# joshua-lintropic/pfs-neural-net

Measured on AMD Instinct MI355X. Metric: training-step edges/sec on 2394×128 bipartite batches; % HBM roofline, higher is better.
Workload: dtype f32 (split-bf16 products: bf16x6 forward, bf16x3 backward); 1 GPU; 16 complete bipartite 2394x128 graphs per GPU, 8 message-passing blocks, Fdim 10; full training step (GNN fwd + train.py loss + bwd + Adam); fibers=2394, classes=128, graphs_per_gpu=16, global_graphs=16, blocks=8, fdim=10, edges_per_gpu_step=4902912, parallelism=dp1

## Files before the change

### include/pfsgnn.h

```cpp
#ifndef PFSGNN_H
#define PFSGNN_H

#include <stddef.h>
#include <stdint.h>

#ifdef __cplusplus
extern "C" {
#endif

const char* pfsgnn_version(void);
const char* pfsgnn_last_error(void);
size_t pfsgnn_workspace_bytes(int G, int NF, int NC, int F);

#define PFSGNN_EDGE_VALU 0
#define PFSGNN_EDGE_MFMA 1
#define PFSGNN_EDGE_MFMA_F32 2
#define PFSGNN_EDGE_BF16Y 3
#define PFSGNN_EDGE_BF16 4
#define PFSGNN_EDGE_BF16_MFMA 5
#define PFSGNN_EDGE_BF16X3 6
#define PFSGNN_EDGE_BF16X6 7
int pfsgnn_set_edge_path(int path);
int pfsgnn_get_edge_path(void);
size_t pfsgnn_sync_bytes(void);
// ... 260 lines not shown
int pfsgnn_sliced_plan(const int* fib_ptr, int G, int NF, int* fib, int* base, int* len,
                       int* slot_of, long long* info, void* ws, size_t ws_bytes, void* stream);
int pfsgnn_sliced_fill(const int* src_p, const int* tgt_p, const int* user_of, const int* fib_ptr,
                       long long E, int NF, int NC, const int* slot_of, const int* base,
                       long long EP, int maxdeg, unsigned char* cls, int* pos_user, float* pco,
                       void* stream);
int pfsgnn_edges_to_slots(const float* src, long long E, long long EP, int F, const int* pos_user,
                          float* dst, void* stream);
int pfsgnn_edges_from_slots(const float* y, const float* sc, const float* sh, long long E,
                            long long EP, int F, const int* pos_user, int rowmajor, float* dst,
                            void* stream);


int pfsgnn_edge_mlp_fwd(int G, int NF, int NC, int F, const float* xe, const float* xsc,
                        const float* xsh, const float* Ps, const float* Pt, const float* W1,
                        const float* W2, const float* b2, float* y, float* mu, float* var,
                        void* ws, size_t ws_bytes, void* stream);
int pfsgnn_edge_mlp_fwd_bn(int G, int NF, int NC, int F, const float* xe, const float* xsc,
                           const float* xsh, const float* Ps, const float* Pt, const float* W1,
                           const float* W2, const float* b2, float* y, float* mu, float* var,
                           const float* gamma, const float* beta, float* rm, float* rv,
                           float momentum, float eps, float* sc, float* sh, float* inv1,
                           float* inv2, void* ws, size_t ws_bytes, void* stream);
int pfsgnn_source_fwd(int G, int NF, int NC, int F, const float* y, const float* sc,
                      const float* sh, const float* Qt, const float* Ws1, const float* Ws2,
                      const float* bs2, float* mom, float* hs, void* ws, size_t ws_bytes,
                      void* stream);
size_t pfsgnn_msg_bytes(int G, int NF, int NC, int F);
int pfsgnn_source_fwd_msg(int G, int NF, int NC, int F, const float* y, const float* sc,
                          const float* sh, const float* Qt, const float* Ws1, const float* Ws2,
                          const float* bs2, float* mom, float* hs, float* msg, void* ws,
                          size_t ws_bytes, void* stream);
int pfsgnn_target_fwd(int G, int NF, int NC, int F, const float* y, const float* sc,
                      const float* sh, const float* Rs, const float* Wt1, float* hsum,
                      const float* Wt2, const float* bt2, float bscale, float* agg,
                      unsigned char* tmask, void* ws, size_t ws_bytes, void* stream);
size_t pfsgnn_tmask_bytes(int G, int NF, int NC, int F);
int pfsgnn_target_bwd(int G, int NF, int NC, int F, const float* y, const float* sc,
                      const float* sh, const float* Rs, const float* Wt1, const float* g_hsum,
                      float* GzT, float* dWt1, float* gxe, float* g_xs,
                      const unsigned char* tmask, void* ws, size_t ws_bytes, void* stream);
int pfsgnn_target_bwd_bn(int G, int NF, int NC, int F, const float* y, const float* sc,
                         const float* sh, const float* Rs, const float* Wt1, const float* g_hsum,
                         float* GzT, float* dWt1, float* gxe, float* g_xs,
                         const unsigned char* tmask, const float* bn_Yp, const float* bn_mu,
                         const float* bn_var, float bn_eps, float* bn_part, void* ws,
                         size_t ws_bytes, void* stream);
int pfsgnn_source_bwd(int G, int NF, int NC, int F, const float* y, const float* sc,
                      const float* sh, const float* Qt, const float* Ws1, const float* Ws2,
                      const float* bs2, const float* mean, const float* coef, const float* Rs,
                      const float* Wt1, const float* g_hsum, const float* g_next,
                      const float* mu1, const float* inv1, float* g_tot, float* GzS,
                      float* dWs1, float* dWs2, float* dbs2, float* Sg, float* Sgx,
                      float* g_xt, const unsigned char* tmask, void* ws, size_t ws_bytes,
                      void* stream);
int pfsgnn_source_bwd_bn(int G, int NF, int NC, int F, const float* y, const float* sc,
                         const float* sh, const float* Qt, const float* Ws1, const float* Ws2,
                         const float* bs2, const float* mean, const float* coef, const float* Rs,
                         const float* Wt1, const float* g_hsum, const float* g_next,
                         const float* mu1, const float* inv1, const float* var1,
                         const float* gamma, long long n, float eps, float* g_tot, float* GzS,
                         float* dWs1, float* dWs2, float* dbs2, float* alpha, float* gam0,
                         float* gam1, float* dgamma, float* dbeta, float* g_xt,
                         const unsigned char* tmask, void* ws, size_t ws_bytes, void* stream);
int pfsgnn_source_bwd_msg(int G, int NF, int NC, int F, const float* y, const float* sc,
                          const float* sh, const float* Qt, const float* Ws1, const float* Ws2,
                          const float* bs2, const float* mean, const float* coef,
                          const float* Rs, const float* Wt1, const float* g_hsum,
                          const float* g_next, const float* mu1, const float* inv1,
                          float* g_tot, float* GzS, float* dWs1, float* dWs2, float* dbs2,
                          float* Sg, float* Sgx, float* g_xt, const unsigned char* tmask,
                          const float* msg, void* ws, size_t ws_bytes, void* stream);
int pfsgnn_source_bwd_bn_msg(int G, int NF, int NC, int F, const float* y, const float* sc,
                             const float* sh, const float* Qt, const float* Ws1,
                             const float* Ws2, const float* bs2, const float* mean,
                             const float* coef, const float* Rs, const float* Wt1,
                             const float* g_hsum, const float* g_next, const float* mu1,
                             const float* inv1, const float* var1, const float* gamma,
                             long long n, float eps, float* g_tot, float* GzS, float* dWs1,
                             float* dWs2, float* dbs2, float* alpha, float* gam0, float* gam1,
                             float* dgamma, float* dbeta, float* g_xt,
                             const unsigned char* tmask, const float* msg, void* ws,
                             size_t ws_bytes, void* stream);
int pfsgnn_edge_bn_grad_sums(int G, int NF, int NC, int F, const float* g, const float* y,
                             const float* mu1, const float* inv1, float* Sg, float* Sgx,
                             void* ws, size_t ws_bytes, void* stream);
int pfsgnn_edge_mlp_bwd(int G, int NF, int NC, int F, const float* g_tot, const float* alpha,
                        const float* gam0, const float* gam1, const float* y, const float* xe,
                        const float* xsc, const float* xsh, const float* Ps, const float* Pt,
                        const float* W1, const float* W2, float* dW1, float* dW2, float* db2,
                        float* gxe, float* GzEs, float* GzEt, float* g_xs, float* g_xt,
                        float* Vu, void* ws, size_t ws_bytes, void* stream);

int pfsgnn_sl_edge_mlp_fwd(const pfsgnn_sliced_t* sl, int G, int NF, int NC, int F,
                           const float* xe, const float* xsc, const float* xsh, const float* Ps,
                           const float* Pt, const float* W1, const float* W2, const float* b2,
                           float* y, float* mu, float* var, void* ws, size_t ws_bytes,
                           void* stream);
int pfsgnn_sl_edge_mlp_fwd_bn(const pfsgnn_sliced_t* sl, int G, int NF, int NC, int F,
                              const float* xe, const float* xsc, const float* xsh,
                              const float* Ps, const float* Pt, const float* W1, const float* W2,
                              const float* b2, float* y, float* mu, float* var,
                              const float* gamma, const float* beta, float* rm, float* rv,
                              float momentum, float eps, float* sc, float* sh, float* inv1,
                              float* inv2, void* ws, size_t ws_bytes, void* stream);
int pfsgnn_sl_source_fwd(const pfsgnn_sliced_t* sl, int G, int NF, int NC, int F, const float* y,
                         const float* sc, const float* sh, const float* Qt, const float* Ws1,
                         const float* Ws2, const float* bs2, float* mom, float* hs, void* ws,
                         size_t ws_bytes, void* stream);
size_t pfsgnn_sl_tmask_bytes(const pfsgnn_sliced_t* sl, int F);
int pfsgnn_sl_target_fwd(const pfsgnn_sliced_t* sl, int G, int NF, int NC, int F, const float* y,
                         const float* sc, const float* sh, const float* Rs, const float* Wt1,
                         float* hsum, const float* Wt2, const float* bt2, float bscale,
                         float* agg, unsigned char* tmask, void* ws, size_t ws_bytes,
                         void* stream);
int pfsgnn_sl_target_bwd(const pfsgnn_sliced_t* sl, int G, int NF, int NC, int F, const float* y,
                         const float* sc, const float* sh, const float* Rs, const float* Wt1,
                         const float* g_hsum, float* GzT, float* dWt1, float* gxe, float* g_xs,
                         const unsigned char* tmask, void* ws, size_t ws_bytes, void* stream);
int pfsgnn_sl_source_bwd(const pfsgnn_sliced_t* sl, int G, int NF, int NC, int F, const float* y,
                         const float* sc, const float* sh, const float* Qt, const float* Ws1,
                         const float* Ws2, const float* bs2, const float* mean,
                         const float* coef, const float* Rs, const float* Wt1,
                         const float* g_hsum, const float* g_next, const float* mu1,
                         const float* inv1, float* g_tot, float* GzS, float* dWs1, float* dWs2,
                         float* dbs2, float* Sg, float* Sgx, float* g_xt,
                         const unsigned char* tmask, void* ws, size_t ws_bytes, void* stream);
int pfsgnn_sl_source_bwd_bn(const pfsgnn_sliced_t* sl, int G, int NF, int NC, int F,
                            const float* y, const float* sc, const float* sh, const float* Qt,
                            const float* Ws1, const float* Ws2, const float* bs2,
                            const float* mean, const float* coef, const float* Rs,
                            const float* Wt1, const float* g_hsum, const float* g_next,
                            const float* mu1, const float* inv1, const float* var1,
                            const float* gamma, long long n, float eps, float* g_tot, float* GzS,
                            float* dWs1, float* dWs2, float* dbs2, float* alpha, float* gam0,
                            float* gam1, float* dgamma, float* dbeta, float* g_xt,
                            const unsigned char* tmask, void* ws, size_t ws_bytes, void* stream);
int pfsgnn_sl_edge_mlp_bwd(const pfsgnn_sliced_t* sl, int G, int NF, int NC, int F,
                           const float* g_tot, const float* alpha, const float* gam0,
                           const float* gam1, const float* y, const float* xe, const float* xsc,
                           const float* xsh, const float* Ps, const float* Pt, const float* W1,
                           const float* W2, float* dW1, float* dW2, float* db2, float* gxe,
                           float* GzEs, float* GzEt, float* g_xs, float* g_xt, float* Vu,
                           void* ws, size_t ws_bytes, void* stream);

int pfsgnn_loss_fwd(int G, int NF, int NC, int F, const float* y, const float* sc,
                    const float* sh, const float* Wd1, const float* bd1, const float* Wd2,
                    const float* bd2, const float* ci, float scale, float sharpness,
                    float noiselevel, unsigned long long seed,
                    const unsigned long long* seed_dev, float* n_prime,
                    float* fiber_time, float* tmean, float* tvar, float* tt,
                    void* ws, size_t ws_bytes, void* stream);
int pfsgnn_loss_finalize(int G, int NF, int NC, const float* n_prime, const float* fiber_time,
                         const float* tvar, const float* ci, float pclass, float pfiber,
                         float total_time, float nfields, float wutils, float wvar,
                         float* loss, float* utils, float* variance, float* Gn, float* Gf,
                         float* Gv, void* stream);
int pfsgnn_loss_bwd(int G, int NF, int NC, int F, const float* y, const float* sc,
                    const float* sh, const float* Wd1, const float* bd1, const float* Wd2,
                    const float* bd2, const float* ci, float scale, float sharpness,
                    float noiselevel, unsigned long long seed,
                    const unsigned long long* seed_dev, const float* Gn,
                    const float* Gf, const float* Gv, const float* tmean, const float* gscale,
                    float* dWd1, float* dbd1, float* dWd2, float* dbd2, float* gxe,
                    void* ws, size_t ws_bytes, void* stream);
int pfsgnn_loss_bn_parts(int G, int NF, int NC);
// ... 28 lines not shown
```

### pfs-neural-net_amd/csrc/pfsgnn_edge.hip

```cpp
#include <cmath>
#include "pfsgnn_common.h"
#include "../../include/pfsgnn.h"
#include "pfsgnn_mfma.h"

#include <algorithm>
#include <map>
#include <mutex>

#define EDGE_PROLOGUE                                                       \
  const int t = threadIdx.x, lane = t & 63;                                 \
  const int wave = __builtin_amdgcn_readfirstlane(t >> 6);                  \
  const int bx = PF_LOGICAL_BLOCK(geo);                                     \
  if (bx >= geo.nblocks) return;                                            \
  const int ks = bx % geo.KS, grp = bx / geo.KS;                            \
  const int fg = grp % geo.NFG, gg = grp / geo.NFG;                         \
  const int f = fg * 64 + lane;                                             \
  const bool fvalid = f < geo.NF;                                           \
  const long long n = (long long)gg * geo.NF + (fvalid ? f : 0);            \
  const long long nbase = (long long)gg * geo.NF + (long long)fg * 64;      \
  const int nvalid = min(64, geo.NF - fg * 64);                             \
  const int c0 = ks * geo.CPS, c1 = min(geo.NC, c0 + geo.CPS);              \
  const long long E = geo.E, NS = geo.NS, NT = geo.NT;                      \
  const uint32_t RB = (uint32_t)geo.E * 4u;       \
  (void)E; (void)NS; (void)NT; (void)n; (void)nbase; (void)nvalid; (void)RB;
// ... 1352 lines not shown
  static const bool on = [] {
    const char* e = getenv("PFSGNN_XCD_ORDER");
    return !(e && atoi(e) == 0);
  }();
  return on;
}
EdgeGeo geo_for(int G, int NF, int NC) {
  if (!use_mfma()) return make_geo(G, NF, NC);
  EdgeGeo g = geo_mfma(G, NF, NC);
  if (xcd_order()) g.xcdper = (g.nblocks + 7) / 8;
  return g;
}
pfm::SlGeo sl_of(const pfsgnn_sliced_t& s) {
  return pfm::SlGeo{s.fib, s.base, s.len, s.cls, s.pco, s.EP, s.E, s.maxdeg};
}
int sliced_max_nc(int F) {
  if (mf_bfy()) return 0;
  static std::mutex mu;
  static std::map<std::pair<int, int>, int> memo;
  std::lock_guard<std::mutex> lk(mu);
  const auto key = std::make_pair(F, g_path);
  auto it = memo.find(key);
  if (it != memo.end()) return it->second;
  const int p0 = mf_prec(0, F), p1 = mf_prec(1, F);
  const int m = std::min(pfm::sl_max_nc(F, p0), p1 == p0 ? pfm::SL_MAX_NC : pfm::sl_max_nc(F, p1));
  memo[key] = m;
  return m;
}
int check_sliced(const char* where, const pfsgnn_sliced_t* sl, int NC, int F) {
  if (!sl) return 0;
  if (sl->EP * F * 4 >= (1ll << 32)) return pf::fail(where, "edge tensor exceeds 4 GiB (split the batch)");
  if (!sl->fib || !sl->base || !sl->len || !sl->cls || !sl->pco || sl->EP <= 0 || sl->E <= 0 ||
      sl->EP < sl->E)
    return pf::fail(where, "bad sliced layout");
  if (mf_bfy()) return pf::fail(where, "sliced layout: bf16 edge-state paths are not supported");
  if (NC > sliced_max_nc(F)) return pf::fail(where, "sliced layout: too many classes per graph for the LDS (pfsgnn_sliced_max_nc)");
  return 0;
}
EdgeGeo geo_of(int G, int NF, int NC, const pfsgnn_sliced_t* sl) {
  return sl ? pfm::sl_geo(G, NF, NC, sl_of(*sl)) : geo_for(G, NF, NC);
}
int col_bpg(const EdgeGeo& geo, const pfsgnn_sliced_t* sl) {
  return sl ? geo.NFG * geo.KS : geo.NFG;
}

}

extern "C" int pfsgnn_set_edge_path(int path) {
  if (path < PFSGNN_EDGE_VALU || path > PFSGNN_EDGE_BF16X6)
    return pf::fail("pfsgnn_set_edge_path",
                    "path must be PFSGNN_EDGE_VALU, _MFMA, _MFMA_F32, _BF16Y, _BF16, _BF16_MFMA, "
                    "_BF16X3 or _BF16X6");
  g_path = path;
  return 0;
}
extern "C" int pfsgnn_get_edge_path(void) { return g_path; }

extern "C" int pfsgnn_sliced_max_nc(int F, int* nc) {
  PF_REQUIRE(nc, "pfsgnn_sliced_max_nc", "null");
  *nc = sliced_max_nc(F);
  return 0;
}

extern "C" int pfsgnn_edge_grid(int G, int NF, int NC, int* info) {
  PF_REQUIRE(G > 0 && NF > 0 && NC > 0 && info, "pfsgnn_edge_grid", "bad arguments");
  const EdgeGeo geo = geo_for(G, NF, NC);
  info[0] = geo.KS;
  info[1] = geo.CPS;
  info[2] = geo.nblocks;
  info[3] = geo.NFG;
  return 0;
}

namespace {
size_t edge_ws_floats(const EdgeGeo& geo, int G, int NC, int F) {
  const size_t nb = geo.nblocks, ks = geo.KS, NS = geo.NS;
  const size_t H = 4 * F, C = 2 * F;
  const size_t colp = (size_t)G * geo.NFG * NC;
  size_t edge = 0;
  edge = std::max(edge, nb * (1 + 2 * F) + 2 * 48 * MOM_MAXG + 256);
  edge = std::max(edge, ks * 4 * C * NS + C * NS + 1024);
  edge = std::max(edge, colp * C + 1024);
  edge = std::max(edge, nb * C * F + ks * C * NS + 1024);
  edge = std::max(edge, nb * (C * (C + 1) + C * F + 2 * F) + colp * C + 4096);
  edge = std::max(edge, nb * (F * (H + 1) + H * F) + colp * H + ks * H * NS + 4096);
  edge = std::max(edge, colp * 4 + ks * NS + nb * (F * (F + 1) + F + 1) + 4096);
  edge += (size_t)geo.NT * (H + 2 * C) + 4 * H * H + 8 * 256;
  return edge;
}
}

extern "C" size_t pfsgnn_workspace_bytes(int G, int NF, int NC, int F) {
  const EdgeGeo geo = make_geo(G, NF, NC);
  pfm::SlGeo sg{};
  sg.maxdeg = 1 << 30;
  EdgeGeo gs = pfm::sl_geo(G, NF, NC, sg);
  gs.NFG *= gs.KS;
  gs.nblocks = G * gs.NFG;
  const size_t edge = std::max(std::max(edge_ws_floats(geo, G, NC, F),
                                        edge_ws_floats(geo_mfma(G, NF, NC), G, NC, F)),
                               edge_ws_floats(gs, G, NC, F));
  size_t node = (size_t)512 * 161 * 161 + 4096;
  size_t lay = (size_t)geo.E + 1024;
  return (std::max(std::max(edge, node), lay) + 64 * 16) * sizeof(float) + 16 * 256;
}

static int edge_mlp_fwd_impl(const pfsgnn_sliced_t* sl, int G, int NF, int NC, int F,
                             const float* xe, const float* xsc, const float* xsh, const float* Ps,
                             const float* Pt, const float* W1, const float* W2, const float* b2,
                             float* y, float* mu, float* var, Bn2Args bn, void* ws,
                             size_t ws_bytes, void* stream) {
  if (int rc = check_dims("pfsgnn_edge_mlp_fwd", G, NF, NC, F)) return rc;
  if (int rc = check_sliced("pfsgnn_edge_mlp_fwd", sl, NC, F)) return rc;
  PF_REQUIRE(xe && Ps && Pt && W1 && W2 && b2 && y && mu && var, "pfsgnn_edge_mlp_fwd", "null");
  const EdgeGeo geo = geo_of(G, NF, NC, sl);
  Ws w{reinterpret_cast<char*>(ws), ws_bytes};
  hipStream_t st = as_stream(stream);
  float* part = w.take((size_t)geo.nblocks * (1 + 2 * F));
  if (sl) {
    PF_REQUIRE(part, "pfsgnn_edge_mlp_fwd", "workspace too small");
    { pf::Timer tm_("edge_mlp_fwd", st);
    float* tabs = w.take((size_t)pfm::sl_tab_floats(geo, F));
    PF_REQUIRE(tabs, "pfsgnn_edge_mlp_fwd", "workspace too small");
    if (int rc = pfm::sl_edge_mlp_fwd(geo, sl_of(*sl), F, xe, xsc, xsh, Ps, Pt, W1, W2, b2, y, part,
                                      tabs, mf_prec(0, F), st))
      return rc;
    tm_.end(); }
    hipLaunchKernelGGL(k_moments_finalize, dim3(F), dim3(256), 0, st, part, geo.nblocks, F, sl->E,
                       mu, var, bn);
    return pf::check_launch("pfsgnn_edge_mlp_fwd");
  }
  if (use_mfma()) {
    PF_REQUIRE(part, "pfsgnn_edge_mlp_fwd", "workspace too small");
    MomFin fin{};
    if (geo.nblocks <= MOM_GROUP * MOM_MAXG && F <= 16) {
      unsigned* cnt = pf::sync_slot(1 + MOM_MAXG);
      double* gp = cnt ? reinterpret_cast<double*>(w.take(2 * 48 * MOM_MAXG)) : nullptr;
      if (gp) fin = MomFin{cnt, gp, mu, var, geo.E, bn};
    }
    { pf::Timer tm_("edge_mlp_fwd", st);
    for (int rep = 0, nrep = 1 + pf::repeats("edge_mlp_fwd"); rep < nrep; ++rep) {
      MomFin fr = fin;
      if (rep + 1 < nrep) fr.bn.rm = fr.bn.rv = nullptr;
      if (int rc = pfm::edge_mlp_fwd(geo, F, xe, xsc, xsh, Ps, Pt, W1, W2, b2, y, part, fr,
                                     mf_prec(0, F), mf_bfy(), st))
        return rc;
    }
    tm_.end(); }
    if (!fin.cnt)
      hipLaunchKernelGGL(k_moments_finalize, dim3(F), dim3(256), 0, st, part, geo.nblocks, F, geo.E,
                         mu, var, bn);
    return pf::check_launch("pfsgnn_edge_mlp_fwd");
  }
  const float* PtT = class_rows(Pt, 4 * F, geo, w, st);
  const float* W2T = transposed(W2, F, 4 * F, w, st);
  PF_REQUIRE(part && PtT && W2T, "pfsgnn_edge_mlp_fwd", "workspace too small");
  { pf::Timer tm_("edge_mlp_fwd", st);
  DISPATCH_F(F, hipLaunchKernelGGL(k_edge_mlp_fwd<FF>, dim3(edge_grid(geo)), dim3(256), 0, st, geo,
                                   xe, xsc, xsh, Ps, PtT, W1, W2T, b2, y, part));
  tm_.end(); }
  hipLaunchKernelGGL(k_moments_finalize, dim3(F), dim3(256), 0, st, part, geo.nblocks, F, geo.E,
                     mu, var, bn);
  return pf::check_launch("pfsgnn_edge_mlp_fwd");
}

extern "C" int pfsgnn_edge_mlp_fwd(int G, int NF, int NC, int F, const float* xe,
                                   const float* xsc, const float* xsh, const float* Ps,
// ... 174 lines not shown
    DISPATCH_F(F, hipLaunchKernelGGL(k_target_fwd<FF>, dim3(edge_grid(geo)), dim3(256), 0, st, geo,
                                     y, sc, sh, Rs, Wt1, part));
  }
  tm_.end();
  return 0;
}

static int target_fwd_impl(const pfsgnn_sliced_t* sl, int G, int NF, int NC, int F,
                           const float* y, const float* sc, const float* sh, const float* Rs,
                           const float* Wt1, float* hsum, const float* Wt2, const float* bt2,
                           float bscale, float* agg, unsigned char* tmask, void* ws,
                           size_t ws_bytes, void* stream) {
  if (int rc = check_dims("pfsgnn_target_fwd", G, NF, NC, F)) return rc;
  if (int rc = check_sliced("pfsgnn_target_fwd", sl, NC, F)) return rc;
  PF_REQUIRE(y && Rs && Wt1 && hsum, "pfsgnn_target_fwd", "null");
  const EdgeGeo geo = geo_of(G, NF, NC, sl);
  Ws w{reinterpret_cast<char*>(ws), ws_bytes};
  float* part = w.take((size_t)G * col_bpg(geo, sl) * NC * 2 * F);
  PF_REQUIRE(part, "pfsgnn_target_fwd", "workspace too small");
  hipStream_t st = as_stream(stream);
  if (int rc = target_fwd_edges(sl, geo, F, y, sc, sh, Rs, Wt1, part, tmask, st)) return rc;
  PF_REQUIRE(!Wt2 || agg, "pfsgnn_target_fwd", "Wt2 needs agg");
  const NodeLin La = Wt2 ? NodeLin{Wt2, 2 * F, 0, 2 * F, 0, bt2, bscale, agg, (long long)G * NC}
                         : no_lin();
  if (int rc = columns_lin(part, G, col_bpg(geo, sl), NC, 2 * F, hsum, La, no_lin(), st)) return rc;
  return pf::check_launch("pfsgnn_target_fwd");
}

extern "C" int pfsgnn_target_fwd(int G, int NF, int NC, int F, const float* y, const float* sc,
                                 const float* sh, const float* Rs, const float* Wt1, float* hsum,
                                 const float* Wt2, const float* bt2, float bscale, float* agg,
                                 unsigned char* tmask, void* ws, size_t ws_bytes, void* stream) {
  return target_fwd_impl(nullptr, G, NF, NC, F, y, sc, sh, Rs, Wt1, hsum, Wt2, bt2, bscale, agg,
                         tmask, ws, ws_bytes, stream);
}

extern "C" size_t pfsgnn_block_tail_bytes(void) { return sizeof(pfsgnn_block_tail); }

extern "C" int pfsgnn_target_block_fwd(const pfsgnn_block_tail* a, void* ws, size_t ws_bytes,
                                       void* stream) {
  const char* where = "pfsgnn_target_block_fwd";
  PF_REQUIRE(a, where, "null");
  const int G = a->G, NF = a->NF, NC = a->NC, F = a->F;
  if (int rc = check_dims(where, G, NF, NC, F)) return rc;
  PF_REQUIRE(a->y && a->Rs && a->Wt1 && a->Wt2 && a->bt2 && a->hsum && a->agg && a->xt && a->u &&
                 a->W1 && a->b1 && a->W2 && a->b2 && a->gamma && a->beta && a->Z && a->Yp &&
                 a->xt_new && a->mu && a->var && a->xs && a->gW1 && a->gb1 && a->gW2 && a->gb2 &&
                 a->means && a->gZ && a->gV && a->unew,
             where, "null");
  PF_REQUIRE(a->gH > 0 && a->gH <= 192, where, "GlobalModel width must be <= 192");
  PF_REQUIRE(!a->gw || (a->y1 && a->r1 && a->r2), where, "RMSNorm needs y1, r1, r2");
  PF_REQUIRE(!a->We || (a->be && a->Ws && a->bs && a->Pt && a->Qt), where,
             "next-block parts need be, Ws, bs, Pt, Qt");
  PF_REQUIRE((long long)G * NC > 1, where, "BatchNorm needs more than one class");
  const EdgeGeo geo = geo_of(G, NF, NC, nullptr);
  Ws w{reinterpret_cast<char*>(ws), ws_bytes};
  float* part = w.take((size_t)G * col_bpg(geo, nullptr) * NC * 2 * F);
  float* scratch = w.take(pf::tail_ws_floats(G, NC, F));
  PF_REQUIRE(part && scratch, where, "workspace too small");
  hipStream_t st = as_stream(stream);
  if (int rc = target_fwd_edges(nullptr, geo, F, a->y, a->sc, a->sh, a->Rs, a->Wt1, part, a->tmask,
                                st))
    return rc;
  if (int rc = pf::class_tail_fwd(*a, part, col_bpg(geo, nullptr), (float)NF, scratch, st)) return rc;
  return pf::check_launch(where);
}

extern "C" int pfsgnn_sl_target_fwd(const pfsgnn_sliced_t* sl, int G, int NF, int NC, int F,
                                    const float* y, const float* sc, const float* sh,
                                    const float* Rs, const float* Wt1, float* hsum,
                                    const float* Wt2, const float* bt2, float bscale, float* agg,
                                    unsigned char* tmask, void* ws, size_t ws_bytes,
                                    void* stream) {
  PF_REQUIRE(sl, "pfsgnn_sl_target_fwd", "null layout");
  return target_fwd_impl(sl, G, NF, NC, F, y, sc, sh, Rs, Wt1, hsum, Wt2, bt2, bscale, agg, tmask,
                         ws, ws_bytes, stream);
}

static int target_bwd_impl(const pfsgnn_sliced_t* sl, int G, int NF, int NC, int F,
                           const float* y, const float* sc, const float* sh, const float* Rs,
                           const float* Wt1, const float* g_hsum, float* GzT, float* dWt1,
                           float* gxe, float* g_xs, const unsigned char* tmask, void* ws,
                           size_t ws_bytes, void* stream,
                           const FiberBnSums& bs = FiberBnSums{}) {
  if (int rc = check_dims("pfsgnn_target_bwd", G, NF, NC, F)) return rc;
  if (int rc = check_sliced("pfsgnn_target_bwd", sl, NC, F)) return rc;
  PF_REQUIRE(y && Rs && Wt1 && g_hsum && GzT && dWt1, "pfsgnn_target_bwd", "null");
  const EdgeGeo geo = geo_of(G, NF, NC, sl);
  const int C = 2 * F;
  Ws w{reinterpret_cast<char*>(ws), ws_bytes};
  hipStream_t st = as_stream(stream);
  float* part = pf::defer_take((size_t)geo.nblocks * C * F);
  const bool defer = part != nullptr;
  if (!defer) part = w.take((size_t)geo.nblocks * C * F);
  float* gz = fiber_dst(geo, C, GzT, w);
  const float* ghT = (sl || use_mfma()) ? g_hsum
                                       : class_rows(g_hsum, C, geo, w, st);
  PF_REQUIRE(part && gz && ghT, "pfsgnn_target_bwd", "workspace too small");
  { pf::Timer tm_("target_bwd", st);
  if (sl) {
    float* tabs = w.take((size_t)pfm::sl_tab_floats(geo, F));
    PF_REQUIRE(tabs, "pfsgnn_target_bwd", "workspace too small");
    if (int rc = pfm::sl_target_bwd(geo, sl_of(*sl), F, y, sc, sh, Rs, Wt1, ghT, gz, gxe, part,
                                    tmask, tabs, mf_prec(1, F), st))
      return rc;
  } else if (use_mfma()) {
    for (int rep = 0, nrep = 1 + pf::repeats("target_bwd"); rep < nrep; ++rep)
      if (int rc = pfm::target_bwd(geo, F, y, sc, sh, Rs, Wt1, ghT, gz, gxe, part, tmask,
                                   mf_prec(1, F), st))
        return rc;
  } else {
  DISPATCH_F(F, hipLaunchKernelGGL(k_target_bwd<FF>, dim3(edge_grid(geo)), dim3(256), 0, st, geo, y,
                                   sc, sh, Rs, Wt1, ghT, gz, gxe, part));
  }
  tm_.end(); }
  if (int rc = fiber_finish_lin(geo, C, gz, GzT, lin_t_add(g_xs ? Wt1 : nullptr, 2 * F, 0, F, g_xs,
                                                           geo.NS),
                                no_lin(), st, bs))
    return rc;
  const RedDesc rd{part, geo.nblocks, (size_t)C * F, F, C, F, dWt1 + F, C, 1, 1.f};
  if (defer) pf::defer_push(&rd, 1);
  else launch_reduce_multi(&rd, 1, st);
  return pf::check_launch("pfsgnn_target_bwd");
}

extern "C" int pfsgnn_target_bwd(int G, int NF, int NC, int F, const float* y, const float* sc,
                                 const float* sh, const float* Rs, const float* Wt1,
                                 const float* g_hsum, float* GzT, float* dWt1, float* gxe,
                                 float* g_xs, const unsigned char* tmask, void* ws,
                                 size_t ws_bytes, void* stream) {
  return target_bwd_impl(nullptr, G, NF, NC, F, y, sc, sh, Rs, Wt1, g_hsum, GzT, dWt1, gxe, g_xs,
                         tmask, ws, ws_bytes, stream);
}

extern "C" int pfsgnn_target_bwd_bn(int G, int NF, int NC, int F, const float* y,
                                    const float* sc, const float* sh, const float* Rs,
                                    const float* Wt1, const float* g_hsum, float* GzT, float* dWt1,
                                    float* gxe, float* g_xs, const unsigned char* tmask,
                                    const float* bn_Yp, const float* bn_mu, const float* bn_var,
                                    float bn_eps, float* bn_part, void* ws, size_t ws_bytes,
                                    void* stream) {
  PF_REQUIRE(g_xs && bn_Yp && bn_mu && bn_var && bn_part, "pfsgnn_target_bwd_bn", "null");
  return target_bwd_impl(nullptr, G, NF, NC, F, y, sc, sh, Rs, Wt1, g_hsum, GzT, dWt1, gxe, g_xs,
                         tmask, ws, ws_bytes, stream,
                         FiberBnSums{bn_Yp, bn_mu, bn_var, bn_eps, bn_part});
}

extern "C" int pfsgnn_sl_target_bwd(const pfsgnn_sliced_t* sl, int G, int NF, int NC, int F,
                                    const float* y, const float* sc, const float* sh,
                                    const float* Rs, const float* Wt1, const float* g_hsum,
                                    float* GzT, float* dWt1, float* gxe, float* g_xs,
                                    const unsigned char* tmask, void* ws, size_t ws_bytes,
                                    void* stream) {
  PF_REQUIRE(sl, "pfsgnn_sl_target_bwd", "null layout");
  return target_bwd_impl(sl, G, NF, NC, F, y, sc, sh, Rs, Wt1, g_hsum, GzT, dWt1, gxe, g_xs, tmask,
                         ws, ws_bytes, stream);
}

struct Bn2Bwd {
  const float* gamma;
  const float* mu1;
  const float* var1;
  long long n;
  float eps;
  float *alpha, *gam0, *gam1, *dgamma, *dbeta;
};

__device__ __forceinline__ void bn2_coef_block(int k, const float* __restrict__ part, int nb, int F,
                                               const Bn2Bwd& bb, float* __restrict__ Sg,
                                               float* __restrict__ Sgx) {
  const int t = threadIdx.x;
  float a0 = 0.f, a1 = 0.f, a2 = 0.f, a3 = 0.f, b0 = 0.f, b1 = 0.f, b2 = 0.f, b3 = 0.f;
  int b = t;
  for (; b + 768 < nb; b += 1024) {
    const float* p = part + (size_t)b * 2 * F + k;
    const size_t st = (size_t)256 * 2 * F;
    a0 += p[0]; b0 += p[F];
    a1 += p[st]; b1 += p[st + F];
    a2 += p[2 * st]; b2 += p[2 * st + F];
    a3 += p[3 * st]; b3 += p[3 * st + F];
  }
  for (; b < nb; b += 256) {
    a0 += part[(size_t)b * 2 * F + k];
    b0 += part[(size_t)b * 2 * F + F + k];
  }
  float v[2] = {(a0 + a1) + (a2 + a3), (b0 + b1) + (b2 + b3)};
  __shared__ float scratch[8];
  block_sum<2>(v, scratch);
  if (t == 0) {
    if (Sg) { Sg[k] = v[0]; Sgx[k] = v[1]; }
    bn2_bwd_coef_one(k, v[0], v[1], bb.mu1, bb.var1, bb.gamma, bb.n, bb.eps, bb.alpha, bb.gam0,
                     bb.gam1, bb.dgamma, bb.dbeta);
  }
}
__global__ __launch_bounds__(256) void k_bn2_coef_part(const float* __restrict__ part, int nb,
                                                       int F, Bn2Bwd bb, float* __restrict__ Sg,
                                                       float* __restrict__ Sgx) {
  bn2_coef_block(blockIdx.x, part, nb, F, bb, Sg, Sgx);
}
extern "C" int pfsgnn_bn2_bwd_coef_part(const float* part, int nparts, int F, const float* gamma,
                                        const float* mu1, const float* var1, long long n,
                                        float eps, float* alpha, float* gam0, float* gam1,
                                        float* dgamma, float* dbeta, void* stream) {
  PF_REQUIRE(part && nparts > 0 && F > 0 && F <= 16 && gamma && mu1 && var1 && alpha && gam0 &&
                 gam1 && dgamma && dbeta,
             "pfsgnn_bn2_bwd_coef_part", "bad arguments");
  const Bn2Bwd bb{gamma, mu1, var1, n, eps, alpha, gam0, gam1, dgamma, dbeta};
  hipLaunchKernelGGL(k_bn2_coef_part, dim3(F), dim3(256), 0, as_stream(stream), part, nparts, F,
                     bb, nullptr, nullptr);
  return pf::check_launch("pfsgnn_bn2_bwd_coef_part");
}
template <int C>
__global__ __launch_bounds__(256) void k_bn2_coef_columns_lin(const float* __restrict__ part,
                                                              int nb, int F, Bn2Bwd bb,
                                                              float* __restrict__ Sg,
                                                              float* __restrict__ Sgx, ColRed cr) {
  __shared__ ColLinLds<C> S;
  const int bx = blockIdx.x;
  if (bx < F)
    bn2_coef_block(bx, part, nb, F, bb, Sg, Sgx);
  else
    reduce_columns_lin_block<C>(S, bx - F, cr.part, cr.G, cr.BPG, cr.NC, cr.out, cr.L0, cr.L1);
}

static int source_bwd_impl(const pfsgnn_sliced_t* sl, int G, int NF, int NC, int F,
                           const float* y, const float* sc, const float* sh, const float* Qt,
                           const float* Ws1, const float* Ws2, const float* bs2, const float* mean,
                           const float* coef, const float* Rs, const float* Wt1,
                           const float* g_hsum, const float* g_next, const float* mu1,
                           const float* inv1, float* g_tot, float* GzS, float* dWs1, float* dWs2,
                           float* dbs2, float* Sg, float* Sgx, const Bn2Bwd* bb, float* g_xt,
                           const unsigned char* tmask, void* ws, size_t ws_bytes, void* stream,
                           const float* msg = nullptr);

extern "C" int pfsgnn_source_bwd(int G, int NF, int NC, int F, const float* y, const float* sc,
                                 const float* sh, const float* Qt, const float* Ws1,
                                 const float* Ws2, const float* bs2, const float* mean,
                                 const float* coef, const float* Rs, const float* Wt1,
                                 const float* g_hsum, const float* g_next, const float* mu1,
                                 const float* inv1, float* g_tot, float* GzS, float* dWs1,
                                 float* dWs2, float* dbs2, float* Sg, float* Sgx, float* g_xt,
                                 const unsigned char* tmask, void* ws, size_t ws_bytes,
                                 void* stream) {
  return source_bwd_impl(nullptr, G, NF, NC, F, y, sc, sh, Qt, Ws1, Ws2, bs2, mean, coef, Rs, Wt1,
                         g_hsum, g_next, mu1, inv1, g_tot, GzS, dWs1, dWs2, dbs2, Sg, Sgx, nullptr,
                         g_xt, tmask, ws, ws_bytes, stream);
}

extern "C" int pfsgnn_source_bwd_bn(int G, int NF, int NC, int F, const float* y, const float* sc,
                                    const float* sh, const float* Qt, const float* Ws1,
                                    const float* Ws2, const float* bs2, const float* mean,
                                    const float* coef, const float* Rs, const float* Wt1,
                                    const float* g_hsum, const float* g_next, const float* mu1,
                                    const float* inv1, const float* var1, const float* gamma,
                                    long long n, float eps, float* g_tot, float* GzS, float* dWs1,
                                    float* dWs2, float* dbs2, float* alpha, float* gam0,
                                    float* gam1, float* dgamma, float* dbeta, float* g_xt,
                                    const unsigned char* tmask, void* ws, size_t ws_bytes,
                                    void* stream) {
  PF_REQUIRE(mu1 && inv1 && var1 && gamma && n > 0 && alpha && gam0 && gam1 && dgamma && dbeta,
             "pfsgnn_source_bwd_bn", "null");
  const Bn2Bwd bb{gamma, mu1, var1, n, eps, alpha, gam0, gam1, dgamma, dbeta};
  return source_bwd_impl(nullptr, G, NF, NC, F, y, sc, sh, Qt, Ws1, Ws2, bs2, mean, coef, Rs, Wt1,
                         g_hsum, g_next, mu1, inv1, g_tot, GzS, dWs1, dWs2, dbs2, nullptr, nullptr,
                         &bb, g_xt, tmask, ws, ws_bytes, stream);
}

extern "C" int pfsgnn_source_bwd_msg(int G, int NF, int NC, int F, const float* y,
                                     const float* sc, const float* sh, const float* Qt,
                                     const float* Ws1, const float* Ws2, const float* bs2,
                                     const float* mean, const float* coef, const float* Rs,
                                     const float* Wt1, const float* g_hsum, const float* g_next,
                                     const float* mu1, const float* inv1, float* g_tot, float* GzS,
                                     float* dWs1, float* dWs2, float* dbs2, float* Sg, float* Sgx,
                                     float* g_xt, const unsigned char* tmask, const float* msg,
                                     void* ws, size_t ws_bytes, void* stream) {
  PF_REQUIRE(msg, "pfsgnn_source_bwd_msg", "null message cache");
  return source_bwd_impl(nullptr, G, NF, NC, F, y, sc, sh, Qt, Ws1, Ws2, bs2, mean, coef, Rs, Wt1,
                         g_hsum, g_next, mu1, inv1, g_tot, GzS, dWs1, dWs2, dbs2, Sg, Sgx, nullptr,
                         g_xt, tmask, ws, ws_bytes, stream, msg);
}

extern "C" int pfsgnn_source_bwd_bn_msg(
    int G, int NF, int NC, int F, const float* y, const float* sc, const float* sh,
    const float* Qt, const float* Ws1, const float* Ws2, const float* bs2, const float* mean,
    const float* coef, const float* Rs, const float* Wt1, const float* g_hsum,
    const float* g_next, const float* mu1, const float* inv1, const float* var1,
    const float* gamma, long long n, float eps, float* g_tot, float* GzS, float* dWs1,
    float* dWs2, float* dbs2, float* alpha, float* gam0, float* gam1, float* dgamma,
    float* dbeta, float* g_xt, const unsigned char* tmask, const float* msg, void* ws,
    size_t ws_bytes, void* stream) {
  PF_REQUIRE(msg && mu1 && inv1 && var1 && gamma && n > 0 && alpha && gam0 && gam1 && dgamma &&
                 dbeta,
             "pfsgnn_source_bwd_bn_msg", "null");
  const Bn2Bwd bb{gamma, mu1, var1, n, eps, alpha, gam0, gam1, dgamma, dbeta};
  return source_bwd_impl(nullptr, G, NF, NC, F, y, sc, sh, Qt, Ws1, Ws2, bs2, mean, coef, Rs, Wt1,
                         g_hsum, g_next, mu1, inv1, g_tot, GzS, dWs1, dWs2, dbs2, nullptr, nullptr,
                         &bb, g_xt, tmask, ws, ws_bytes, stream, msg);
}

extern "C" int pfsgnn_sl_source_bwd(const pfsgnn_sliced_t* sl, int G, int NF, int NC, int F,
                                    const float* y, const float* sc, const float* sh,
                                    const float* Qt, const float* Ws1, const float* Ws2,
                                    const float* bs2, const float* mean, const float* coef,
                                    const float* Rs, const float* Wt1, const float* g_hsum,
                                    const float* g_next, const float* mu1, const float* inv1,
                                    float* g_tot, float* GzS, float* dWs1, float* dWs2,
                                    float* dbs2, float* Sg, float* Sgx, float* g_xt,
                                    const unsigned char* tmask, void* ws, size_t ws_bytes,
                                    void* stream) {
  PF_REQUIRE(sl, "pfsgnn_sl_source_bwd", "null layout");
  return source_bwd_impl(sl, G, NF, NC, F, y, sc, sh, Qt, Ws1, Ws2, bs2, mean, coef, Rs, Wt1,
                         g_hsum, g_next, mu1, inv1, g_tot, GzS, dWs1, dWs2, dbs2, Sg, Sgx, nullptr,
                         g_xt, tmask, ws, ws_bytes, stream);
}

extern "C" int pfsgnn_sl_source_bwd_bn(
    const pfsgnn_sliced_t* sl, int G, int NF, int NC, int F, const float* y, const float* sc,
    const float* sh, const float* Qt, const float* Ws1, const float* Ws2, const float* bs2,
    const float* mean, const float* coef, const float* Rs, const float* Wt1, const float* g_hsum,
    const float* g_next, const float* mu1, const float* inv1, const float* var1,
    const float* gamma, long long n, float eps, float* g_tot, float* GzS, float* dWs1,
    float* dWs2, float* dbs2, float* alpha, float* gam0, float* gam1, float* dgamma, float* dbeta,
    float* g_xt, const unsigned char* tmask, void* ws, size_t ws_bytes, void* stream) {
  PF_REQUIRE(sl && mu1 && inv1 && var1 && gamma && n > 0 && alpha && gam0 && gam1 && dgamma &&
                 dbeta,
             "pfsgnn_sl_source_bwd_bn", "null");
  const Bn2Bwd bb{gamma, mu1, var1, n, eps, alpha, gam0, gam1, dgamma, dbeta};
  return source_bwd_impl(sl, G, NF, NC, F, y, sc, sh, Qt, Ws1, Ws2, bs2, mean, coef, Rs, Wt1,
                         g_hsum, g_next, mu1, inv1, g_tot, GzS, dWs1, dWs2, dbs2, nullptr, nullptr,
                         &bb, g_xt, tmask, ws, ws_bytes, stream);
}

static int source_bwd_impl(const pfsgnn_sliced_t* sl, int G, int NF, int NC, int F,
                           const float* y, const float* sc, const float* sh, const float* Qt,
                           const float* Ws1, const float* Ws2, const float* bs2, const float* mean,
                           const float* coef, const float* Rs, const float* Wt1,
                           const float* g_hsum, const float* g_next, const float* mu1,
                           const float* inv1, float* g_tot, float* GzS, float* dWs1, float* dWs2,
                           float* dbs2, float* Sg, float* Sgx, const Bn2Bwd* bb, float* g_xt,
                           const unsigned char* tmask, void* ws, size_t ws_bytes, void* stream,
                           const float* msg) {
  if (int rc = check_dims("pfsgnn_source_bwd", G, NF, NC, F)) return rc;
  PF_REQUIRE(!msg || (!sl && msg_bytes(G, NF, NC, F) > 0), "pfsgnn_source_bwd_msg",
             "the message cache is not kept on this path (pfsgnn_msg_bytes is 0)");
  if (int rc = check_sliced("pfsgnn_source_bwd", sl, NC, F)) return rc;
  PF_REQUIRE(y && Qt && Ws1 && Ws2 && bs2 && mean && coef && g_tot && GzS && dWs1 && dWs2 && dbs2,
             "pfsgnn_source_bwd", "null");
  PF_REQUIRE((Rs == nullptr) == (Wt1 == nullptr) && (Rs == nullptr) == (g_hsum == nullptr),
             "pfsgnn_source_bwd", "Rs, Wt1, g_hsum must be given together");
  PF_REQUIRE(!mu1 || (inv1 && ((Sg && Sgx) || bb)), "pfsgnn_source_bwd",
             "mu1 needs inv1, Sg, Sgx");
  const EdgeGeo geo = geo_of(G, NF, NC, sl);
  const int C = 2 * F;
  const size_t nb = geo.nblocks;
  Ws w{reinterpret_cast<char*>(ws), ws_bytes};
  float* pW2 = pf::defer_take(nb * C * (C + 1) + nb * C * F);
  const bool defer = pW2 != nullptr;
  if (!defer) pW2 = w.take(nb * C * (C + 1) + nb * C * F);
  float* pW1 = pW2 ? pW2 + nb * C * (C + 1) : nullptr;
  float* pCol = w.take((size_t)G * col_bpg(geo, sl) * NC * C);
  float* pBN = w.take(nb * 2 * F);
  hipStream_t st = as_stream(stream);
  const bool mfma = sl || use_mfma();
  const float* QtT = mfma ? Qt : class_rows(Qt, C, geo, w, st);
  const float* ghT = mfma ? g_hsum : class_rows(g_hsum, C, geo, w, st);
  PF_REQUIRE(pW2 && pW1 && pCol && pBN && QtT && (ghT || !g_hsum), "pfsgnn_source_bwd",
             "workspace too small");
  { pf::Timer tm_("source_bwd", st);
  if (sl) {
    float* tabs = w.take((size_t)pfm::sl_tab_floats(geo, F));
    PF_REQUIRE(tabs, "pfsgnn_source_bwd", "workspace too small");
    if (int rc = pfm::sl_source_bwd(geo, sl_of(*sl), F, y, sc, sh, QtT, Ws1, Ws2, bs2, mean, coef,
                                    Rs, Wt1, ghT, g_next, mu1, inv1, g_tot, pW2, pW1, pCol, pBN,
                                    tmask, tabs, mf_prec(1, F), st))
      return rc;
  } else if (mfma) {
    for (int rep = 0, nrep = 1 + pf::repeats("source_bwd"); rep < nrep; ++rep)
      if (int rc = pfm::source_bwd(geo, F, msg, y, sc, sh, QtT, Ws1, Ws2, bs2, mean, coef, Rs, Wt1,
                                   ghT, g_next, mu1, inv1, g_tot, pW2, pW1, pCol, pBN, tmask,
                                   mf_prec(1, F), st))
        return rc;
  } else {
  DISPATCH_F(F, hipLaunchKernelGGL(k_source_bwd<FF>, dim3(edge_grid(geo)), dim3(256), 0, st, geo, y,
                                   sc, sh, QtT, Ws1, Ws2, bs2, mean, coef, Rs, Wt1, ghT, g_next,
                                   mu1, inv1, g_tot, pW2, pW1, pCol, pBN));
  }
  tm_.end(); }
  {
    RedDesc rd[5] = {{pBN, (int)nb, (size_t)2 * F, F, 1, F, Sg, F, 0, 1.f},
                     {pBN + F, (int)nb, (size_t)2 * F, F, 1, F, Sgx, F, 0, 1.f},
                     {pW2, (int)nb, (size_t)C * (C + 1), C + 1, C, C, dWs2, C, 1, 1.f},
                     {pW2 + C, (int)nb, (size_t)C * (C + 1), C + 1, C, 1, dbs2, 1, 1, 1.f},
                     {pW1, (int)nb, (size_t)C * F, F, C, F, dWs1 + F, C, 1, 1.f}};
    const bool sums = mu1 && !bb;
    const RedDesc* now = sums ? rd : rd + 2;
    int nnow = sums ? 5 : 3;
    if (defer) {
      pf::defer_push(rd + 2, 3);
      nnow -= 3;
    }
    if (nnow) launch_reduce_multi(now, nnow, st);
  }
  const NodeLin Lx = lin_t_add(g_xt ? Ws1 : nullptr, 2 * F, 0, F, g_xt, geo.NT);
  if (bb && Lx.W) {
    const ColRed cr{pCol, G, col_bpg(geo, sl), NC, GzS, Lx, no_lin()};
    const int nbc = (int)(((long long)G * NC + 3) / 4);
    DISPATCH_C(C, hipLaunchKernelGGL(k_bn2_coef_columns_lin<CC>, dim3(F + nbc), dim3(256), 0, st,
                                     pBN, (int)nb, F, *bb, Sg, Sgx, cr));
  } else {
    if (bb)
      hipLaunchKernelGGL(k_bn2_coef_part, dim3(F), dim3(256), 0, st, pBN, (int)nb, F, *bb, Sg,
                         Sgx);
    if (int rc = columns_lin(pCol, G, col_bpg(geo, sl), NC, C, GzS, Lx, no_lin(), st)) return rc;
  }
  return pf::check_launch("pfsgnn_source_bwd");
}

extern "C" int pfsgnn_edge_bn_grad_sums(int G, int NF, int NC, int F, const float* g,
                                        const float* y, const float* mu1, const float* inv1,
                                        float* Sg, float* Sgx, void* ws, size_t ws_bytes,
                                        void* stream) {
  if (int rc = check_dims("pfsgnn_edge_bn_grad_sums", G, NF, NC, F)) return rc;
  PF_REQUIRE(g && y && mu1 && inv1 && Sg && Sgx, "pfsgnn_edge_bn_grad_sums", "null");
  const EdgeGeo geo = make_geo(G, NF, NC);
  Ws w{reinterpret_cast<char*>(ws), ws_bytes};
  float* pBN = w.take((size_t)geo.nblocks * 2 * F);
  PF_REQUIRE(pBN, "pfsgnn_edge_bn_grad_sums", "workspace too small");
  hipStream_t st = as_stream(stream);
  { pf::Timer tm_("edge_bn_sums", st);
  DISPATCH_F(F, hipLaunchKernelGGL(k_edge_bn_sums<FF>, dim3(edge_grid(geo)), dim3(256), 0, st, geo, g,
                                   y, mu1, inv1, pBN));
  tm_.end(); }
  {
    RedDesc rd[2] = {{pBN, geo.nblocks, (size_t)2 * F, F, 1, F, Sg, F, 0, 1.f},
                     {pBN + F, geo.nblocks, (size_t)2 * F, F, 1, F, Sgx, F, 0, 1.f}};
    launch_reduce_multi(rd, 2, st);
  }
  return pf::check_launch("pfsgnn_edge_bn_grad_sums");
}

static int edge_mlp_bwd_impl(const pfsgnn_sliced_t* sl, int G, int NF, int NC, int F,
                             const float* g_tot, const float* alpha, const float* gam0,
                             const float* gam1, const float* y, const float* xe, const float* xsc,
                             const float* xsh, const float* Ps, const float* Pt, const float* W1,
                             const float* W2, float* dW1, float* dW2, float* db2, float* gxe,
                             float* GzEs, float* GzEt, float* g_xs, float* g_xt, float* Vu,
                             void* ws, size_t ws_bytes, void* stream) {
  if (int rc = check_dims("pfsgnn_edge_mlp_bwd", G, NF, NC, F)) return rc;
  if (int rc = check_sliced("pfsgnn_edge_mlp_bwd", sl, NC, F)) return rc;
  PF_REQUIRE(g_tot && alpha && gam0 && gam1 && y && xe && Ps && Pt && W1 && W2 && dW1 && dW2 &&
                 db2 && GzEs && GzEt,
             "pfsgnn_edge_mlp_bwd", "null");
  const EdgeGeo geo = geo_of(G, NF, NC, sl);
  const int H = 4 * F;
  const size_t nb = geo.nblocks;
  Ws w{reinterpret_cast<char*>(ws), ws_bytes};
  float* pW2 = pf::defer_take(nb * F * (H + 1) + nb * H * F);
  const bool defer = pW2 != nullptr;
  if (!defer) pW2 = w.take(nb * F * (H + 1) + nb * H * F);
  float* pW1 = pW2 ? pW2 + nb * F * (H + 1) : nullptr;
  float* pCol = w.take((size_t)G * col_bpg(geo, sl) * NC * H);
  float* gs = fiber_dst(geo, H, GzEs, w);
  hipStream_t st = as_stream(stream);
  if (sl) {
    PF_REQUIRE(pW2 && pW1 && pCol && gs, "pfsgnn_edge_mlp_bwd", "workspace too small");
    pf::Timer tm_("edge_mlp_bwd", st);
    float* tabs = w.take((size_t)pfm::sl_tab_floats(geo, F));
    PF_REQUIRE(tabs, "pfsgnn_edge_mlp_bwd", "workspace too small");
    if (int rc = pfm::sl_edge_mlp_bwd(geo, sl_of(*sl), F, g_tot, alpha, gam0, gam1, y, xe, xsc,
                                      xsh, Ps, Pt, W1, W2, gxe, gs, pW2, pW1, pCol, tabs,
                                      mf_prec(0, F), st))
      return rc;
    tm_.end();
  } else if (use_mfma()) {
    PF_REQUIRE(pW2 && pW1 && pCol && gs, "pfsgnn_edge_mlp_bwd", "workspace too small");
    pf::Timer tm_("edge_mlp_bwd", st);
    for (int rep = 0, nrep = 1 + pf::repeats("edge_mlp_bwd"); rep < nrep; ++rep)
      if (int rc = pfm::edge_mlp_bwd(geo, F, g_tot, alpha, gam0, gam1, y, xe, xsc, xsh, Ps, Pt,
                                     W1, W2, gxe, gs, pW2, pW1, pCol, mf_prec(0, F), st))
        return rc;
    tm_.end();
  } else {
// ... 53 lines not shown
```

### pfs-neural-net_amd/csrc/pfsgnn_mfma.h

```cpp
#pragma once
#include "pfsgnn_common.h"

namespace pfm {

static constexpr int TARGET_BLOCKS = 2048;
static constexpr int MAX_CPS = 64;

int edge_mlp_fwd(const EdgeGeo& geo, int F, const float* xe, const float* xsc, const float* xsh,
                 const float* Ps, const float* PtS, const float* W1, const float* W2,
                 const float* b2, float* y, float* part, const MomFin& fin, int prec, int bfy,
                 hipStream_t st);
int source_fwd(const EdgeGeo& geo, int F, const float* y, const float* sc, const float* sh,
               const float* QtS, const float* Ws1, const float* Ws2, const float* bs2,
               float* partS, int prec, hipStream_t st);
int source_fwd_tiles(const EdgeGeo& geo, int F, const float* y, const float* sc,
                     const float* sh, const float* QtS, const float* Ws1, const float* Ws2,
                     const float* bs2, float* mom, float* hs, float* msg, int prec, int wave_nc,
                     hipStream_t st);
int target_fwd(const EdgeGeo& geo, int F, const float* y, const float* sc, const float* sh,
               const float* Rs, const float* Wt1, float* part, uint8_t* tmask, int prec,
               hipStream_t st);
int target_bwd(const EdgeGeo& geo, int F, const float* y, const float* sc, const float* sh,
               const float* Rs, const float* Wt1, const float* ghS, float* gz, float* gxe,
               float* part, const uint8_t* tmask, int prec, hipStream_t st);
int source_bwd(const EdgeGeo& geo, int F, const float* msg, const float* y, const float* sc,
               const float* sh, const float* QtS, const float* Ws1, const float* Ws2,
               const float* bs2, const float* mean, const float* coef, const float* Rs,
               const float* Wt1, const float* ghS, const float* g_next, const float* mu1,
               const float* inv1, float* g_tot, float* pW2, float* pW1, float* pCol, float* pBN,
               const uint8_t* tmask, int prec, hipStream_t st);
int edge_mlp_bwd(const EdgeGeo& geo, int F, const float* g_tot, const float* alpha,
                 const float* gam0, const float* gam1, const float* y, const float* xe,
                 const float* xsc, const float* xsh, const float* Ps, const float* PtS,
                 const float* W1, const float* W2, float* gxe, float* gs, float* pW2, float* pW1,
                 float* pCol, int prec, hipStream_t st);

struct SlGeo {
  const int* fib;
  const int* base;
  const int* len;
  const uint8_t* cls;
  const float* pco;
  long long EP, E;
  int maxdeg;
};
static constexpr int SL_MAX_NC = 128;
int sl_max_nc(int F, int prec);
EdgeGeo sl_geo(int G, int NF, int NC, const SlGeo& sl);
int sl_edge_mlp_fwd(const EdgeGeo& geo, const SlGeo& sl, int F, const float* xe, const float* xsc,
                    const float* xsh, const float* Ps, const float* PtS, const float* W1,
                    const float* W2, const float* b2, float* y, float* part, float* tabs,
                    int prec, hipStream_t st);
int sl_source_fwd(const EdgeGeo& geo, const SlGeo& sl, int F, const float* y, const float* sc,
                  const float* sh, const float* QtS, const float* Ws1, const float* Ws2,
                  const float* bs2, float* mom, float* hs, float* tabs, int prec,
                  hipStream_t st);
int sl_target_fwd(const EdgeGeo& geo, const SlGeo& sl, int F, const float* y, const float* sc,
                  const float* sh, const float* Rs, const float* Wt1, float* part, uint8_t* tmask,
                  int prec, hipStream_t st);
int sl_target_bwd(const EdgeGeo& geo, const SlGeo& sl, int F, const float* y, const float* sc,
                  const float* sh, const float* Rs, const float* Wt1, const float* ghS, float* gz,
                  float* gxe, float* part, const uint8_t* tmask, float* tabs, int prec,
                  hipStream_t st);
int sl_source_bwd(const EdgeGeo& geo, const SlGeo& sl, int F, const float* y, const float* sc,
                  const float* sh, const float* QtS, const float* Ws1, const float* Ws2,
                  const float* bs2, const float* mean, const float* coef, const float* Rs,
                  const float* Wt1, const float* ghS, const float* g_next, const float* mu1,
                  const float* inv1, float* g_tot, float* pW2, float* pW1, float* pCol,
                  float* pBN, const uint8_t* tmask, float* tabs, int prec, hipStream_t st);
static inline long long sl_tab_floats(const EdgeGeo& geo, int F) {
  const long long c = 16 * ((((2 * F + 3) / 4) + 3) / 4), h = 16 * ((((4 * F + 3) / 4) + 3) / 4);
  return geo.NT * (2 * c > h ? 2 * c : h);
}
int sl_edge_mlp_bwd(const EdgeGeo& geo, const SlGeo& sl, int F, const float* g_tot,
                    const float* alpha, const float* gam0, const float* gam1, const float* y,
                    const float* xe, const float* xsc, const float* xsh, const float* Ps,
                    const float* PtS, const float* W1, const float* W2, float* gxe, float* gs,
                    float* pW2, float* pW1, float* pCol, float* tabs, int prec, hipStream_t st);

}
```

### pfs-neural-net_amd/csrc/pfsgnn_mfma.hip

```cpp
#include "pfsgnn_mfma_core.h"

#ifndef MF_WG_EARLY_READS
#define MF_WG_EARLY_READS 1
#endif
#ifndef MF_FWD_PAIRS
#define MF_FWD_PAIRS 0
#endif
#ifndef MF_SB_PACK
#define MF_SB_PACK 1
#endif
#ifndef MF_SB_LDSW
#define MF_SB_LDSW 0
#endif
#ifndef MF_WG4
#define MF_WG4 1
#endif

namespace {

#ifndef MF_EFWD_MINB
#define MF_EFWD_MINB 6
#endif
#ifndef MF_EFWD_B6S
#define MF_EFWD_B6S 1
// ... 489 lines not shown
                            p[((1 * NT + tt) * 4 + r) * 64], p[((2 * NT + tt) * 4 + r) * 64],
                            p[((3 * NT + tt) * 4 + r) * 64]);
        na += nb;
      }
      emit(o, mean, M2, M3, M4);
    }
}

template <int F, int PREC>
__global__ __launch_bounds__(256) void km_target_fwd(EdgeGeo geo, const float* __restrict__ y,
                                                     const float* __restrict__ sc,
                                                     const float* __restrict__ sh,
                                                     const float* __restrict__ Rs,
                                                     const float* __restrict__ Wt1,
                                                     float* __restrict__ part,
                                                     uint8_t* __restrict__ tmask) {
  constexpr int C = 2 * F, NT = GM<C>::NT;
  MF_GEO
  __shared__ __attribute__((aligned(16))) float colbuf[COL_CH * 4 * C];
  FwdLayer<PREC, C, F> L1;
  L1.load([&](int h, int k) { return Wt1[h * 2 * F + F + k]; }, lane);
  floatx4 rs[NT];
#pragma unroll
  for (int tt = 0; tt < NT; ++tt) rs[tt] = ld_node<C>(Rs, tt, g4, NS, n, fvalid);
  const floatx4 scv = ld_fconst<F>(sc, g4, 1.f), shv = ld_fconst<F>(sh, g4, 0.f);
  MF_FMASK(F)
  const Rsrc ry = rsrc(y, EB * F);

  int cbase = c0;
  auto load = [&](int c) {
    Rows<1> r;
    r.v[0] = ld_frows<F>(ry, (uint32_t)c * eoc, ro);
    return r;
  };
  auto pre = [&](const Rows<1>& rows, floatx4 (&z)[NT]) {
    const floatx4 x[1] = {edge_in<F>(rows.v[0], fm, sc, scv, shv)};
#pragma unroll
    for (int tt = 0; tt < NT; ++tt) z[tt] = rs[tt];
    L1.apply(x, z);
  };
  auto post = [&](const floatx4 (&z)[NT], int c) {
    if (tmask && fvalid)
      (tmask + (uint32_t)c * eoc)[opaque(eo0 + g4)] = (uint8_t)mask_bits<C>(z);
    const int cl = c - cbase;
#pragma unroll
    for (int tt = 0; tt < NT; ++tt)
#pragma unroll
      for (int r = 0; r < GM<C>::nreg(tt); ++r) {
        const float s = row_sum16(fvalid ? lrelu(z[tt][r]) : 0.f);
        const int h = GM<C>::row(g4, 4 * tt + r);
        if (j16 == 15 && h >= 0) colbuf[(cl * 4 + wave) * C + h] = s;
      }
    if (cl == COL_CH - 1 || c == c1 - 1) {
      __syncthreads();
      col_flush<C>(colbuf, cl + 1, cbase, part, colbase);
      __syncthreads();
      cbase = c + 1;
    }
  };
#if MF_FWD_PAIRS
  class_stream_pairs<MF_DEPTH_FWD>(
      c0, c1, load,
      [&](const Rows<1>& rows, int c) {
        floatx4 z[NT];
        pre(rows, z);
        post(z, c);
      },
      [&](const Rows<1>& ra, int ca, const Rows<1>& rb, int cb) {
        floatx4 za[NT], zb[NT];
        pre(ra, za);
        pre(rb, zb);
        post(za, ca);
        post(zb, cb);
      });
#else
  class_stream<MF_DEPTH_FWD>(c0, c1, load, [&](const Rows<1>& rows, int c) {
    floatx4 z[NT];
    pre(rows, z);
    post(z, c);
  });
#endif
}

template <int F, int PREC, bool TM>
__global__ __launch_bounds__(256) void km_target_bwd(EdgeGeo geo, const float* __restrict__ y,
                                                     const float* __restrict__ sc,
                                                     const float* __restrict__ sh,
                                                     const float* __restrict__ Rs,
                                                     const float* __restrict__ Wt1,
                                                     const float* __restrict__ ghS,
                                                     float* __restrict__ GzT,
                                                     float* __restrict__ gxe,
                                                     float* __restrict__ partW,
                                                     const uint8_t* __restrict__ tmask) {
  constexpr int C = 2 * F, NT = GM<C>::NT;
  constexpr int NIMG = NT + 1;
  using WI = WgImg<PREC>;
  MF_GEO
  __shared__ __attribute__((aligned(16))) short imgs[4 * NIMG * WI::U];
  __shared__ float scratch[4 * C * F];
  __shared__ __attribute__((aligned(16))) float ghl[MF_MAX_CPS * ClassRows<C>::CP];
  ClassRows<C>::stage(ghl, ghS, geo.NT, (long long)gg * geo.NC + c0, c1 - c0);
  short* img = imgs + wave * NIMG * WI::U;
  FwdLayer<FP(PREC), C, F> L1;
  if constexpr (!TM) L1.load([&](int h, int k) { return Wt1[h * 2 * F + F + k]; }, lane);
  GradLayer<PREC, F, C> LT;
  LT.load([&](int k, int h) { return gxe ? Wt1[h * 2 * F + F + k] : 0.f; }, lane);
  floatx4 rs[NT], accF[NT], accW[NT];
#pragma unroll
  for (int tt = 0; tt < NT; ++tt) {
    if constexpr (!TM) rs[tt] = ld_node<C>(Rs, tt, g4, NS, n, fvalid);
    accF[tt] = zero4();
    accW[tt] = zero4();
  }
  const floatx4 scv = ld_fconst<F>(sc, g4, 1.f), shv = ld_fconst<F>(sh, g4, 0.f);
  MF_FMASK(F)
  const Rsrc ry = rsrc(y, EB * F), rtm = rsrc(tmask, EB);
  __syncthreads();

  auto load = [&](int c) {
    Rows<1> r;
    const uint32_t co = (uint32_t)c * eoc;
    r.v[0] = ld_frows<F>(ry, co, ro);
    if constexpr (TM) r.m = __builtin_amdgcn_raw_buffer_load_b8(rtm, eo0 + g4, co, 0);
    return r;
  };
  class_stream<MF_DEPTH_BWD>(c0, c1, load, [&](const Rows<1>& rows, int c) {
    const floatx4 x[1] = {edge_in<F>(rows.v[0], fm, sc, scv, shv)};
    floatx4 z[NT], gz[NT];
    if constexpr (!TM) {
#pragma unroll
      for (int tt = 0; tt < NT; ++tt) z[tt] = rs[tt];
      L1.apply(x, z);
    }
#pragma unroll
    for (int tt = 0; tt < NT; ++tt) {
      const floatx4 gh = ClassRows<C>::get(ghl, c - c0, tt, g4);
      gz[tt] = zero4();
#pragma unroll
      for (int r = 0; r < GM<C>::nreg(tt); ++r) {
        const float sl = TM ? mask_slope(rows.m, 4 * tt + r) : dlrelu(z[tt][r]);
        gz[tt][r] = fvalid ? gh[r] * sl : 0.f;
      }
      accF[tt] += gz[tt];
    }
    Fr sgz[NT];
#pragma unroll
    for (int tt = 0; tt < NT; ++tt) sgz[tt] = split(gz[tt]);
    if (gxe) {
      floatx4 gx[1] = {zero4()};
      if constexpr (PREC >= 1) LT.apply(sgz, gx); else LT.apply(gz, gx);
      st_frows<F>(gxe, EB * F, (uint32_t)c * eoc, ro, g4, fvalid, gx[0]);
    }
    lds_order();
#pragma unroll
    for (int tt = 0; tt < NT; ++tt) WI::put(img + tt * WI::U, lane, gz[tt], sgz[tt]);
    WI::put(img + NT * WI::U, lane, x[0], split(x[0]));
    lds_order();
    const typename WI::TB tx = WI::B(img + NT * WI::U, lane);
#pragma unroll
    for (int tt = 0; tt < NT; ++tt)
      accW[tt] = WI::mma(WI::A(img + tt * WI::U, lane), tx, accW[tt]);
  });
  if (fvalid) {
#pragma unroll
    for (int tt = 0; tt < NT; ++tt)
#pragma unroll
      for (int r = 0; r < GM<C>::nreg(tt); ++r) {
        const int h = GM<C>::row(g4, 4 * tt + r);
        if (h >= 0) GzT[(size_t)ks * C * NS + (size_t)h * NS + n] = accF[tt][r];
      }
  }
  block_partial(accW, scratch, C * F, [&](int a, int s, int jj) {
    const int h = GM<C>::mrow(a, s), k = GM<F>::mrow(0, jj);
    return (h >= 0 && k >= 0) ? h * F + k : -1;
  }, partW + (size_t)bx * C * F);
}

template <int F, int PREC, bool TM, bool MSG = false>
__global__ __launch_bounds__(256, 2) void km_source_bwd(
    EdgeGeo geo, const float* __restrict__ msg, const float* __restrict__ y, const float* __restrict__ sc,
    const float* __restrict__ sh, const float* __restrict__ QtS, const float* __restrict__ Ws1,
    const float* __restrict__ Ws2, const float* __restrict__ bs2, const float* __restrict__ mean,
    const float* __restrict__ coef, const float* __restrict__ Rs, const float* __restrict__ Wt1,
    const float* __restrict__ ghS, const float* __restrict__ g_next,
    const float* __restrict__ mu1, const float* __restrict__ inv1, float* __restrict__ g_tot,
    float* __restrict__ partW2, float* __restrict__ partW1, float* __restrict__ partCol,
    float* __restrict__ partBN, const uint8_t* __restrict__ tmask) {
  constexpr int C = 2 * F, NT = GM<C>::NT;
  constexpr bool PACK = MF_SB_PACK && NT == 2 && GM<C>::nreg(1) == 1 && GM<F>::NT == 1 && GM<F>::RPG == 3;
  constexpr int NIMG = PACK ? 5 : 3 * NT + 1;
  constexpr int SCR = C * (C + 1) > C * F ? C * (C + 1) : C * F;
  using WI = WgImg<PREC>;
  MF_GEO
  __shared__ __attribute__((aligned(16))) short imgs[4 * NIMG * WI::U];
  __shared__ __attribute__((aligned(16))) float colbuf[COL_CH * 4 * C];
  __shared__ float scratch[4 * SCR];
  __shared__ __attribute__((aligned(16))) float qtl[MF_MAX_CPS * ClassRows<C>::CP];
  __shared__ __attribute__((aligned(16))) float ghl[MF_MAX_CPS * ClassRows<C>::CP];
  ClassRows<C>::stage(qtl, QtS, geo.NT, (long long)gg * geo.NC + c0, c1 - c0);
  if (ghS) ClassRows<C>::stage(ghl, ghS, geo.NT, (long long)gg * geo.NC + c0, c1 - c0);
  short* img = imgs + wave * NIMG * WI::U;
  short* im_gm = img;
  short* im_a = img + NT * WI::U;
  short* im_gz = im_a + NT * WI::U;
  short* im_x = im_gz + NT * WI::U;
  short* im_r1 = img;
  short* im_r2 = img + WI::U;
  short* im_r3 = img + 2 * WI::U;
  short* im_c1 = img + 3 * WI::U;
  short* im_c2 = img + 4 * WI::U;
  (void)im_r1; (void)im_r2; (void)im_r3; (void)im_c1; (void)im_c2;
  const long long CNS = (long long)C * NS;
  const bool tpart = Rs != nullptr;

  RecLayer<PREC, C, F> L1s, L1t;
  RecLayer<PREC, C, C> L2;
  constexpr int R1 = RecLds<RecLayer<PREC, C, F>>::n, R2 = RecLds<RecLayer<PREC, C, C>>::n;
  __shared__ s16x8 recw[(R1 * (TM ? 1 : 2) + R2) > 0 ? R1 * (TM ? 1 : 2) + R2 : 1];
  rec_bind(L1s, recw);
  rec_bind(L2, recw + R1);
  rec_bind(L1t, recw + R1 + R2);
  L1s.load([&](int h, int k) { return Ws1[h * 2 * F + F + k]; }, lane);
  if constexpr (!TM) L1t.load([&](int h, int k) { return tpart ? Wt1[h * 2 * F + F + k] : 0.f; }, lane);
  if constexpr (!MSG) L2.load([&](int o, int h) { return Ws2[o * C + h]; }, lane);
  constexpr bool LW = MF_SB_LDSW && std::is_same_v<GradLayer<PREC, C, C>, LayerB3<C, C>>;
  using GL2 = std::conditional_t<LW, LayerB3S<C, C>, GradLayer<PREC, C, C>>;
  using GL1 = std::conditional_t<LW, LayerB3S<F, C>, GradLayer<PREC, F, C>>;
  GL2 L2T;
  GL1 L1sT, L1tT;
  if constexpr (LW) {
    __shared__ s16x8 gw[(LayerB3S<C, C>::NOP + 2 * LayerB3S<F, C>::NOP) * 64];
    L2T.bind(gw);
    L1sT.bind(gw + LayerB3S<C, C>::NOP * 64);
    L1tT.bind(gw + (LayerB3S<C, C>::NOP + LayerB3S<F, C>::NOP) * 64);
  }
  L2T.load([&](int h, int o) { return Ws2[o * C + h]; }, lane);
  L1sT.load([&](int k, int h) { return Ws1[h * 2 * F + F + k]; }, lane);
  L1tT.load([&](int k, int h) { return tpart ? Wt1[h * 2 * F + F + k] : 0.f; }, lane);
  floatx4 rs[NT], bias[NT], mn[NT], q0[NT], q1[NT], q2[NT], q3[NT];
#pragma unroll
  for (int tt = 0; tt < NT; ++tt) {
    if constexpr (!TM) rs[tt] = ld_node<C>(Rs, tt, g4, NS, n, fvalid);
    bias[tt] = ld_vec<C>(bs2, tt, g4);
    mn[tt] = ld_node<C>(mean, tt, g4, NS, n, fvalid);
    q0[tt] = ld_node<C>(coef, tt, g4, NS, n, fvalid);
    q1[tt] = ld_node<C>(coef + CNS, tt, g4, NS, n, fvalid);
    q2[tt] = ld_node<C>(coef + 2 * CNS, tt, g4, NS, n, fvalid);
    q3[tt] = ld_node<C>(coef + 3 * CNS, tt, g4, NS, n, fvalid);
  }
  const floatx4 scv = ld_fconst<F>(sc, g4, 1.f), shv = ld_fconst<F>(sh, g4, 0.f);
  const floatx4 m1v = ld_fconst<F>(mu1, g4, 0.f), i1v = ld_fconst<F>(inv1, g4, 0.f);
  MF_FMASK(F)
  const Rsrc ry = rsrc(y, EB * F), rgn = rsrc(g_next, EB * F), rtm = rsrc(tmask, EB);
  [[maybe_unused]] const Rsrc rms = rsrc(msg, EB * C);
  [[maybe_unused]] const RowOff<C> roC(eo0, RB, g4);

  floatx4 accW2[NT * NT], accW1[NT], accB[NT];
  floatx4 accP[5];
#pragma unroll
  for (int tt = 0; tt < NT; ++tt) {
    accW1[tt] = zero4();
    accB[tt] = zero4();
#pragma unroll
    for (int nb = 0; nb < NT; ++nb) accW2[tt * NT + nb] = zero4();
  }
#pragma unroll
  for (int i = 0; i < 5; ++i) accP[i] = zero4();
  floatx4 sg = zero4(), sgx = zero4();
  const s16x8 ones = ones_reg();
  __syncthreads();

  int cbase = c0;
  using RowsT = Rows<MSG ? 2 + NT : 2>;
  auto load = [&](int c) {
    RowsT r;
    const uint32_t co = (uint32_t)c * eoc;
    r.v[0] = ld_frows<F>(ry, co, ro);
    r.v[1] = g_next ? ld_frows<F>(rgn, co, ro) : zero4();
    if constexpr (TM) r.m = tpart ? __builtin_amdgcn_raw_buffer_load_b8(rtm, eo0 + g4, co, 0) : 0u;
    if constexpr (MSG) {
      floatx4 mv[NT];
      ld_rows_nt<C>(rms, co, roC, mv);
#pragma unroll
      for (int tt = 0; tt < NT; ++tt) r.v[2 + tt] = mv[tt];
    }
    return r;
  };
  class_stream<MF_DEPTH_BWD>(c0, c1, load, [&](const RowsT& rows, int c) {
    const floatx4 yr = rows.v[0], gnr = rows.v[1];
    const floatx4 x[1] = {edge_in<F>(yr, fm, sc, scv, shv)};
    floatx4 zs[NT], as[NT], m[NT];
#pragma unroll
    for (int tt = 0; tt < NT; ++tt) zs[tt] = ClassRows<C>::get(qtl, c - c0, tt, g4);
    L1s.apply(x, zs);
    lrelu_act<C>(zs, as);
    if constexpr (MSG) {
#pragma unroll
      for (int tt = 0; tt < NT; ++tt) m[tt] = rows.v[2 + tt];
    } else {
#pragma unroll
      for (int tt = 0; tt < NT; ++tt) m[tt] = bias[tt];
      L2.apply(as, m);
    }
    floatx4 gm[NT];
#pragma unroll
    for (int tt = 0; tt < NT; ++tt) {
      gm[tt] = zero4();
#pragma unroll
      for (int r = 0; r < GM<C>::nreg(tt); ++r) {
        const float d = m[tt][r] - mn[tt][r];
        gm[tt][r] = fvalid ? fmaf(d, fmaf(d, fmaf(d, q3[tt][r], q2[tt][r]), q1[tt][r]), q0[tt][r]) : 0.f;
      }
      accB[tt] += gm[tt];
    }
    Fr sgm[NT], sgz[NT];
#pragma unroll
    for (int tt = 0; tt < NT; ++tt) sgm[tt] = split(gm[tt]);
    floatx4 gz[NT];
#pragma unroll
    for (int tt = 0; tt < NT; ++tt) gz[tt] = zero4();
    if constexpr (PREC >= 1) L2T.apply(sgm, gz); else L2T.apply(gm, gz);
#pragma unroll
    for (int tt = 0; tt < NT; ++tt) {
#pragma unroll
      for (int r = 0; r < GM<C>::nreg(tt); ++r) gz[tt][r] *= dlrelu(zs[tt][r]);
      sgz[tt] = split(gz[tt]);
    }
    lds_order();
    [[maybe_unused]] floatx4 r3v, c2v;
    if constexpr (PACK) {
      r3v = floatx4{gm[1][0], gz[1][0], 0.f, 0.f};
      c2v = floatx4{as[1][0], x[0][0], x[0][1], x[0][2]};
      const Fr sr3 = {s16x4{sgm[1].h[0], sgz[1].h[0], 0, 0}, s16x4{sgm[1].l[0], sgz[1].l[0], 0, 0}};
      WI::put(im_r1, lane, gm[0], sgm[0]);
      WI::put(im_r2, lane, gz[0], sgz[0]);
      WI::put(im_r3, lane, r3v, sr3);
      WI::put(im_c1, lane, as[0], split(as[0]));
      WI::put(im_c2, lane, c2v, split(c2v));
    } else {
#pragma unroll
      for (int tt = 0; tt < NT; ++tt) {
        WI::put(im_gm + tt * WI::U, lane, gm[tt], sgm[tt]);
        WI::put(im_a + tt * WI::U, lane, as[tt], split(as[tt]));
        WI::put(im_gz + tt * WI::U, lane, gz[tt], sgz[tt]);
      }
      WI::put(im_x, lane, x[0], split(x[0]));
    }
    lds_order();
#if MF_WG_EARLY_READS
    typename WI::R rx, ra[NT], rgm[NT], rgz[NT], rp[5], rq[2];
    if constexpr (PACK) {
#pragma unroll
      for (int i = 0; i < 5; ++i) rp[i] = WI::rd(img + i * WI::U, lane);
#if MF_WG4
      lds_order();
      rq[0] = WI::rd(im_c1, lane);
      rq[1] = WI::rd(im_c2, lane);
#endif
    } else {
      rx = WI::rd(im_x, lane);
#pragma unroll
      for (int tt = 0; tt < NT; ++tt) {
        ra[tt] = WI::rd(im_a + tt * WI::U, lane);
        rgm[tt] = WI::rd(im_gm + tt * WI::U, lane);
        rgz[tt] = WI::rd(im_gz + tt * WI::U, lane);
      }
    }
    lds_order();
#endif
    floatx4 g[1] = {zero4()};
    if constexpr (PREC >= 1) L1sT.apply(sgz, g); else L1sT.apply(gz, g);
    if (tpart) {
      floatx4 zt[NT];
      if constexpr (!TM) {
#pragma unroll
        for (int tt = 0; tt < NT; ++tt) zt[tt] = rs[tt];
        L1t.apply(x, zt);
      }
#pragma unroll
      for (int tt = 0; tt < NT; ++tt) {
        const floatx4 gh = ClassRows<C>::get(ghl, c - c0, tt, g4);
#pragma unroll
        for (int r = 0; r < 4; ++r) {
          const float sl = TM ? mask_slope(rows.m, 4 * tt + r) : dlrelu(zt[tt][r]);
          zt[tt][r] = (fvalid && r < GM<C>::nreg(tt)) ? gh[r] * sl : 0.f;
        }
      }
      if constexpr (PREC >= 1) {
        Fr szt[NT];
#pragma unroll
        for (int tt = 0; tt < NT; ++tt) szt[tt] = split(zt[tt]);
        L1tT.apply(szt, g);
      } else {
        L1tT.apply(zt, g);
      }
    }
#pragma unroll
    for (int r = 0; r < 4; ++r) g[0][r] = fm[r] ? g[0][r] + (g_next ? gnr[r] : 0.f) : 0.f;
    st_frows<F>(g_tot, EB * F, (uint32_t)c * eoc, ro, g4, fvalid, g[0]);
    if (mu1) {
#pragma unroll
      for (int r = 0; r < GM<F>::RPG; ++r) {
        sg[r] += g[0][r];
        sgx[r] = fmaf(g[0][r], (yr[r] - m1v[r]) * i1v[r], sgx[r]);
      }
    }
    lds_order();
    const int cl = c - cbase;
    if constexpr (PACK) {
#if !MF_WG_EARLY_READS
#error "source_bwd's packed tiles read their images early (MF_WG_EARLY_READS)"
#endif
      const typename WI::TA t1 = WI::A(rp[0]), t2 = WI::A(rp[1]), t3 = WI::A(rp[2]);
#if MF_WG4
      const typename WI::TB4 tc1 = WI::B4(rp[3], rq[0]), tc2 = WI::B4(rp[4], rq[1]);
      accP[0] = WI::mma4(t1, tc1, accP[0]);
      accP[1] = WI::mma4(t1, tc2, accP[1]);
      accP[2] = WI::mma4(t2, tc2, accP[2]);
      accP[3] = WI::mma4(t3, tc1, accP[3]);
      accP[4] = WI::mma4(t3, tc2, accP[4]);
#else
      const typename WI::TB tc1 = WI::B(rp[3]), tc2 = WI::B(rp[4]);
      accP[0] = WI::mma(t1, tc1, accP[0]);
      accP[1] = WI::mma(t1, tc2, accP[1]);
      accP[2] = WI::mma(t2, tc2, accP[2]);
      accP[3] = WI::mma(t3, tc1, accP[3]);
      accP[4] = WI::mma(t3, tc2, accP[4]);
#endif
      const floatx4 cs2 = WI::colsum(t2, gz[0], ones), cs3 = WI::colsum(t3, r3v, ones);
      if (j16 == WI::CS_LANE) {
#pragma unroll
        for (int r = 0; r < 4; ++r) {
          const int h = GM<C>::mrow(0, 4 * g4 + r);
          if (h >= 0) colbuf[(cl * 4 + wave) * C + h] = cs2[r];
        }
        const int h1 = GM<C>::row(g4, 4);
        if (h1 >= 0) colbuf[(cl * 4 + wave) * C + h1] = cs3[1];
      }
    } else {
#if MF_WG_EARLY_READS
    const typename WI::TB tx = WI::B(rx);
    typename WI::TB ta[NT];
#pragma unroll
    for (int nb = 0; nb < NT; ++nb) ta[nb] = WI::B(ra[nb]);
#else
    const typename WI::TB tx = WI::B(im_x, lane);
    typename WI::TB ta[NT];
#pragma unroll
    for (int nb = 0; nb < NT; ++nb) ta[nb] = WI::B(im_a + nb * WI::U, lane);
#endif
#pragma unroll
    for (int tt = 0; tt < NT; ++tt) {
#if MF_WG_EARLY_READS
      const typename WI::TA tgm = WI::A(rgm[tt]);
#pragma unroll
      for (int nb = 0; nb < NT; ++nb) accW2[tt * NT + nb] = WI::mma(tgm, ta[nb], accW2[tt * NT + nb]);
      const typename WI::TA tgz = WI::A(rgz[tt]);
#else
      const typename WI::TA tgm = WI::A(im_gm + tt * WI::U, lane);
#pragma unroll
      for (int nb = 0; nb < NT; ++nb) accW2[tt * NT + nb] = WI::mma(tgm, ta[nb], accW2[tt * NT + nb]);
      const typename WI::TA tgz = WI::A(im_gz + tt * WI::U, lane);
#endif
      accW1[tt] = WI::mma(tgz, tx, accW1[tt]);
      const floatx4 cs = WI::colsum(tgz, gz[tt]);
      if (j16 == WI::CS_LANE) {
#pragma unroll
        for (int r = 0; r < 4; ++r) {
          const int h = GM<C>::mrow(tt, 4 * g4 + r);
          if (h >= 0) colbuf[(cl * 4 + wave) * C + h] = cs[r];
        }
      }
    }
    }
    if (cl == COL_CH - 1 || c == c1 - 1) {
      __syncthreads();
      col_flush<C>(colbuf, cl + 1, cbase, partCol, colbase);
      __syncthreads();
      cbase = c + 1;
    }
  });
  if constexpr (PACK) {
    block_partial(accP, scratch, C * (C + 1), [&](int a, int s, int jj) {
      int o = -1, h = -1;
      if (a == 0) { o = GM<C>::mrow(0, s); h = GM<C>::mrow(0, jj); }
      if (a == 1 && (jj & 3) == 0) { o = GM<C>::mrow(0, s); h = GM<C>::row(jj >> 2, 4); }
      if (a == 3 && (s & 3) == 0) { o = GM<C>::row(s >> 2, 4); h = GM<C>::mrow(0, jj); }
      if (a == 4 && (s & 3) == 0 && (jj & 3) == 0) { o = GM<C>::row(s >> 2, 4); h = GM<C>::row(jj >> 2, 4); }
      return (o >= 0 && h >= 0) ? o * (C + 1) + h : -1;
    }, partW2 + (size_t)bx * C * (C + 1));
  } else {
    block_partial(accW2, scratch, C * (C + 1), [&](int a, int s, int jj) {
      const int o = GM<C>::mrow(a / NT, s), h = GM<C>::mrow(a % NT, jj);
      return (o >= 0 && h >= 0) ? o * (C + 1) + h : -1;
    }, partW2 + (size_t)bx * C * (C + 1));
  }
  {
    __syncthreads();
#pragma unroll
    for (int tt = 0; tt < NT; ++tt)
#pragma unroll
      for (int r = 0; r < GM<C>::nreg(tt); ++r) {
        const float v = group_sum16(accB[tt][r]);
        const int o = GM<C>::row(g4, 4 * tt + r);
        if (j16 == 0 && o >= 0) scratch[wave * C + o] = v;
      }
    __syncthreads();
    if (t < C)
      partW2[(size_t)bx * C * (C + 1) + t * (C + 1) + C] =
          ((scratch[t] + scratch[C + t]) + scratch[2 * C + t]) + scratch[3 * C + t];
  }
  if constexpr (PACK) {
    block_partial(accP, scratch, C * F, [&](int a, int s, int jj) {
      int h = -1, k = -1;
      if ((jj & 3) != 0) k = GM<F>::row(jj >> 2, (jj & 3) - 1);
      if (a == 2) h = GM<C>::mrow(0, s);
      if (a == 4 && (s & 3) == 1) h = GM<C>::row(s >> 2, 4);
      return (h >= 0 && k >= 0) ? h * F + k : -1;
    }, partW1 + (size_t)bx * C * F);
  } else {
    block_partial(accW1, scratch, C * F, [&](int a, int s, int jj) {
      const int h = GM<C>::mrow(a, s), k = GM<F>::mrow(0, jj);
      return (h >= 0 && k >= 0) ? h * F + k : -1;
    }, partW1 + (size_t)bx * C * F);
  }
  if (mu1) {
    __syncthreads();
#pragma unroll
    for (int r = 0; r < GM<F>::RPG; ++r) {
      const float a = group_sum16(sg[r]), b = group_sum16(sgx[r]);
      const int k = GM<F>::row(g4, r);
      if (j16 == 0 && k >= 0) { scratch[wave * 2 * F + k] = a; scratch[wave * 2 * F + F + k] = b; }
    }
    __syncthreads();
    if (t < 2 * F)
      partBN[(size_t)bx * 2 * F + t] =
          ((scratch[t] + scratch[2 * F + t]) + scratch[4 * F + t]) + scratch[6 * F + t];
  }
}

#ifndef MF_BWD_PIPE6
#define MF_BWD_PIPE6 0
#endif
template <int F, int PREC>
__global__ __launch_bounds__(256, 2) void km_edge_mlp_bwd(
    EdgeGeo geo, const float* __restrict__ g_tot, const float* __restrict__ alpha,
    const float* __restrict__ gam0, const float* __restrict__ gam1, const float* __restrict__ y,
    const float* __restrict__ xe, const float* __restrict__ xsc, const float* __restrict__ xsh,
    const float* __restrict__ Ps, const float* __restrict__ PtS, const float* __restrict__ W1,
    const float* __restrict__ W2, float* __restrict__ gxe, float* __restrict__ GzEs,
    float* __restrict__ partW2, float* __restrict__ partW1, float* __restrict__ partCol) {
  constexpr int H = 4 * F, NT = GM<H>::NT;
  constexpr int NIMG = 1 + NT + NT + 1;
  constexpr int SCR = F * (H + 1) > H * F ? F * (H + 1) : H * F;
  using WI = WgImg<PREC>;
  MF_GEO
  __shared__ __attribute__((aligned(16))) short imgs[4 * NIMG * WI::U];
  __shared__ __attribute__((aligned(16))) float colbuf[COL_CH * 4 * H];
  __shared__ float scratch[4 * SCR];
  __shared__ __attribute__((aligned(16))) float ptl[MF_MAX_CPS * ClassRows<H>::CP];
  ClassRows<H>::stage(ptl, PtS, geo.NT, (long long)gg * geo.NC + c0, c1 - c0);
  short* img = imgs + wave * NIMG * WI::U;
  short* im_gy = img;
  short* im_a = img + WI::U;
  short* im_gz = im_a + NT * WI::U;
  short* im_x = im_gz + NT * WI::U;

#ifdef MF_EMB_REC_B6
  std::conditional_t<PREC == 1, LayerB6<H, F>, FwdLayer<FP(PREC), H, F>> L1;
#else
  FwdLayer<FP(PREC), H, F> L1;
#endif
  L1.load([&](int h, int k) { return W1[h * 4 * F + 2 * F + k]; }, lane);
  GradLayer<PREC, H, F> L2T;
  L2T.load([&](int h, int o) { return W2[o * H + h]; }, lane);
  GradLayer<PREC, F, H> L1T;
  L1T.load([&](int k, int h) { return gxe ? W1[h * 4 * F + 2 * F + k] : 0.f; }, lane);
  floatx4 ps[NT], accF[NT], accW1[NT], accW2[NT];
#pragma unroll
  for (int tt = 0; tt < NT; ++tt) {
    ps[tt] = ld_node<H>(Ps, tt, g4, NS, n, fvalid);
    accF[tt] = zero4();
    accW1[tt] = zero4();
    accW2[tt] = zero4();
  }
  floatx4 accB = zero4();
  const floatx4 alv = ld_fconst<F>(alpha, g4, 0.f), g0v = ld_fconst<F>(gam0, g4, 0.f),
                g1v = ld_fconst<F>(gam1, g4, 0.f);
  const floatx4 scv = ld_fconst<F>(xsc, g4, 1.f), shv = ld_fconst<F>(xsh, g4, 0.f);
  MF_FMASK(F)
  const Rsrc rgt = rsrc(g_tot, EB * F), ry = rsrc(y, EB * F), rxe = rsrc(xe, EB * F);
  const s16x8 ones = ones_reg();
  __syncthreads();

  int cbase = c0;
  auto load = [&](int c) {
    Rows<3> r;
    const uint32_t co = (uint32_t)c * eoc;
    r.v[0] = ld_frows<F>(rgt, co, ro);
    r.v[1] = ld_frows<F>(ry, co, ro);
    r.v[2] = ld_frows<F>(rxe, co, ro);
    return r;
  };
  struct Head {
    floatx4 gy, x, z[NT];
  };
  auto head = [&](const Rows<3>& rows, int c) {
// ... 161 lines not shown
    MF_CASE(16, 0, K, __VA_ARGS__) MF_CASE(16, 1, K, __VA_ARGS__)                \
    default: return pf::fail("pfsgnn mfma", "unsupported Fdim for this edge path"); \
  }

#define MF_CASE3(FF, PP, TT, K, ...)                                              \
  case FF * 8 + PP: {                                                             \
    hipLaunchKernelGGL((K<FF, PP, TT>), dim3(edge_grid(geo)), dim3(256), 0, st, geo, \
                       __VA_ARGS__);                                              \
  } break;
#define MF_LAUNCH3(F, P, TT, K, ...)                                              \
  switch ((F) * 8 + (P)) {                                                        \
    MF_CASE3(8, 0, TT, K, __VA_ARGS__) MF_CASE3(8, 1, TT, K, __VA_ARGS__)        \
    MF_CASE3(10, 0, TT, K, __VA_ARGS__) MF_CASE3(10, 1, TT, K, __VA_ARGS__)      \
    MF_CASE3(10, 2, TT, K, __VA_ARGS__) MF_CASE3(10, 3, TT, K, __VA_ARGS__)      \
    MF_CASE3(10, 4, TT, K, __VA_ARGS__)                                           \
    MF_CASE3(16, 0, TT, K, __VA_ARGS__) MF_CASE3(16, 1, TT, K, __VA_ARGS__)      \
    default: return pf::fail("pfsgnn mfma", "unsupported Fdim for this edge path"); \
  }

#ifndef MF_PART
#define MF_PART 0
#endif
namespace pfm {
#if MF_PART != 2

static inline int fwd_prec(int prec) { return FP(prec); }

int edge_mlp_fwd(const EdgeGeo& geo, int F, const float* xe, const float* xsc, const float* xsh,
                 const float* Ps, const float* PtS, const float* W1, const float* W2,
                 const float* b2, float* y, float* part, const MomFin& fin, int prec, int bfy,
                 hipStream_t st) {
  if (fin.cnt && (geo.nblocks > MOM_GROUP * MOM_MAXG || F > 16))
    return pf::fail("pfsgnn mfma", "edge_mlp_fwd: in-launch finalize needs <= 4096 blocks");
  MF_LAUNCH(F, fwd_prec(prec), km_edge_mlp_fwd, xe, xsc, xsh, Ps, PtS, W1, W2, b2, y, part, bfy,
            fin)
  return 0;
}

int source_fwd(const EdgeGeo& geo, int F, const float* y, const float* sc, const float* sh,
               const float* QtS, const float* Ws1, const float* Ws2, const float* bs2,
               float* partS, int prec, hipStream_t st) {
  MF_LAUNCH(F, fwd_prec(prec), km_source_fwd, y, sc, sh, QtS, Ws1, Ws2, bs2, partS)
  return 0;
}

int source_fwd_tiles(const EdgeGeo& geo, int F, const float* y, const float* sc,
                     const float* sh, const float* QtS, const float* Ws1, const float* Ws2,
                     const float* bs2, float* mom, float* hs, float* msg, int prec, int wave_nc,
                     hipStream_t st) {
  if (geo.NC > MF_SFT_MAXNC) return pf::fail("pfsgnn mfma", "source_fwd_tiles: NC > 256");
  const bool wf = geo.NC <= std::min(wave_nc, MF_SFT_WAVE_MAXNC);
  const int TF = wf ? 64 : 16;
  const int ntiles = geo.G * ((geo.NF + TF - 1) / TF);
  const int nb = 8 * ((ntiles + 7) / 8);
  const size_t lds = sft_lds_floats(geo.NC, F) * sizeof(float);
#define MF_SFT(FF, PP)                                                                     \
  case FF * 8 + PP:                                                                        \
    if (wf)                                                                                \
      hipLaunchKernelGGL((km_source_fwd_ft<FF, PP, true>), dim3(nb), dim3(256), lds, st, geo, \
                         ntiles, y, sc, sh, QtS, Ws1, Ws2, bs2, mom, hs, msg);             \
    else                                                                                   \
      hipLaunchKernelGGL((km_source_fwd_ft<FF, PP, false>), dim3(nb), dim3(256), lds, st, geo, \
                         ntiles, y, sc, sh, QtS, Ws1, Ws2, bs2, mom, hs, msg);             \
    break;
  switch (F * 8 + fwd_prec(prec)) {
    MF_SFT(8, 0) MF_SFT(8, 1) MF_SFT(10, 0) MF_SFT(10, 1) MF_SFT(10, 2) MF_SFT(10, 3)
    MF_SFT(10, 4) MF_SFT(16, 0) MF_SFT(16, 1)
    default: return pf::fail("pfsgnn mfma", "unsupported Fdim for this edge path");
  }
#undef MF_SFT
  return 0;
}

int target_fwd(const EdgeGeo& geo, int F, const float* y, const float* sc, const float* sh,
               const float* Rs, const float* Wt1, float* part, uint8_t* tmask, int prec,
               hipStream_t st) {
  MF_LAUNCH(F, fwd_prec(prec), km_target_fwd, y, sc, sh, Rs, Wt1, part, tmask)
  return 0;
}

int target_bwd(const EdgeGeo& geo, int F, const float* y, const float* sc, const float* sh,
               const float* Rs, const float* Wt1, const float* ghS, float* gz, float* gxe,
               float* part, const uint8_t* tmask, int prec, hipStream_t st) {
  if (tmask) {
    MF_LAUNCH3(F, prec, true, km_target_bwd, y, sc, sh, Rs, Wt1, ghS, gz, gxe, part, tmask)
  } else {
    MF_LAUNCH3(F, prec, false, km_target_bwd, y, sc, sh, Rs, Wt1, ghS, gz, gxe, part, tmask)
  }
  return 0;
}

int source_bwd(const EdgeGeo& geo, int F, const float* msg, const float* y, const float* sc,
               const float* sh, const float* QtS, const float* Ws1, const float* Ws2,
               const float* bs2, const float* mean, const float* coef, const float* Rs,
               const float* Wt1, const float* ghS, const float* g_next, const float* mu1,
               const float* inv1, float* g_tot, float* pW2, float* pW1, float* pCol, float* pBN,
               const uint8_t* tmask, int prec, hipStream_t st) {
  if (msg) {
    if (prec != 0 && prec != 1) return pf::fail("pfsgnn mfma", "message cache: mfma paths only");
#define MF_CASE_MSG(FF, PP, TT)                                                                  \
  case FF * 8 + PP:                                                                             \
    hipLaunchKernelGGL((km_source_bwd<FF, PP, TT, true>), dim3(edge_grid(geo)), dim3(256), 0, st, \
                       geo, msg, y, sc, sh, QtS, Ws1, Ws2, bs2, mean, coef, Rs, Wt1, ghS, g_next, \
                       mu1, inv1, g_tot, pW2, pW1, pCol, pBN, tmask);                           \
    break;
    if (tmask && Rs) {
      switch (F * 8 + prec) {
        MF_CASE_MSG(8, 0, true) MF_CASE_MSG(8, 1, true) MF_CASE_MSG(10, 0, true)
        MF_CASE_MSG(10, 1, true) MF_CASE_MSG(16, 0, true) MF_CASE_MSG(16, 1, true)
        default: return pf::fail("pfsgnn mfma", "unsupported Fdim for this edge path");
      }
    } else {
      switch (F * 8 + prec) {
        MF_CASE_MSG(8, 0, false) MF_CASE_MSG(8, 1, false) MF_CASE_MSG(10, 0, false)
        MF_CASE_MSG(10, 1, false) MF_CASE_MSG(16, 0, false) MF_CASE_MSG(16, 1, false)
        default: return pf::fail("pfsgnn mfma", "unsupported Fdim for this edge path");
      }
    }
#undef MF_CASE_MSG
    return 0;
  }
  if (tmask && Rs) {
    MF_LAUNCH3(F, prec, true, km_source_bwd, nullptr, y, sc, sh, QtS, Ws1, Ws2, bs2, mean, coef, Rs, Wt1,
               ghS, g_next, mu1, inv1, g_tot, pW2, pW1, pCol, pBN, tmask)
  } else {
    MF_LAUNCH3(F, prec, false, km_source_bwd, nullptr, y, sc, sh, QtS, Ws1, Ws2, bs2, mean, coef, Rs, Wt1,
               ghS, g_next, mu1, inv1, g_tot, pW2, pW1, pCol, pBN, tmask)
  }
  return 0;
}

#endif
#if MF_PART != 1
int edge_mlp_bwd(const EdgeGeo& geo, int F, const float* g_tot, const float* alpha,
                 const float* gam0, const float* gam1, const float* y, const float* xe,
                 const float* xsc, const float* xsh, const float* Ps, const float* PtS,
                 const float* W1, const float* W2, float* gxe, float* gs, float* pW2, float* pW1,
                 float* pCol, int prec, hipStream_t st) {
  MF_LAUNCH(F, prec, km_edge_mlp_bwd, g_tot, alpha, gam0, gam1, y, xe, xsc, xsh, Ps, PtS, W1, W2,
            gxe, gs, pW2, pW1, pCol)
  return 0;
}
#endif

}
```

### pfs-neural-net_amd/pfsgnn/engine.py

```python
import os

import torch


class Dims:

    def __init__(self, G, NF, NC, F, sp=None):
        self.G, self.NF, self.NC, self.F = int(G), int(NF), int(NC), int(F)
        self.sp = sp
        self.E = self.G * self.NF * self.NC if sp is None else sp.E
        self.EP = self.E if sp is None else sp.EP
        self.NS = self.G * self.NF
        self.NT = self.G * self.NC

    def __repr__(self):
        kind = "" if self.sp is None else ", general"
        return f"Dims(G={self.G}, NF={self.NF}, NC={self.NC}, F={self.F}, E={self.E}{kind})"


def param_names(B, normed=True):
    names = []

    def mlp(pre):
        names.extend([pre + ".0.weight", pre + ".0.bias", pre + ".2.weight", pre + ".2.bias"])
# ... 233 lines not shown
                                                Gr[key + "weight"], Gr[key + "bias"])
            z = self.be.zeros(scale.shape[0])
            return scale, z, z
        return self.be.bn2_bwd_coef(Sg, Sgx, st["mu1"], st["var1"], P[key + "weight"], d.E,
                                    self.bn_eps, Gr[key + "weight"], Gr[key + "bias"])

    def edge_bnstat(self, P, pre, st):
        if "rm" in st:
            key = pre + "norm."
            inv, _ = self.be.bn_eval_bwd_coef(P[key + "weight"], P[key + "bias"], st["rm"],
                                              st["rv"], self.bn_eps, 2)
            return st["rm"], inv
        return st["mu1"], st["inv1"]

    def edge_bwd(self, P, Gr, d, pre, st, g_tot, bnc, want_gxe, g_xs, g_xt, g_u):
        be, F, G = self.be, self.F, d.G
        if self.normed:
            alpha, gam0, gam1 = bnc
        else:
            alpha, gam0, gam1 = be.ones(F), be.zeros(F), be.zeros(F)
        W1, W2 = P[pre + "0.weight"], P[pre + "2.weight"]
        xe, xsc, xsh = st["xe3"]
        dW1 = Gr[pre + "0.weight"]
        g_xe, GzEs, GzEt, Vu = be.edge_mlp_bwd(d, g_tot, alpha, gam0, gam1, st["y"], xe, xsc, xsh,
                                               st["Ps"], st["Pt"], W1, W2, dW1,
                                               Gr[pre + "2.weight"], Gr[pre + "2.bias"],
                                               want_gxe=want_gxe, nodes=(g_xs, g_xt))
        be.wgrad(GzEs, st["xs"], dW1, col0=0)
        be.wgrad_cat(GzEt, [(st["xt"], F, False), (st["u"], 3 * F, True)], dW1,
                     db=Gr[pre + "0.bias"])
        self._gu_add(Vu, G, g_u)
        return g_xe

    def source_fwd(self, P, BN, d, pre, xs, xt, xe3, u, Qt=None, epi=None):
        be, F = self.be, self.F
        Ws1, bs1 = P[pre + "node_mlp_1.0.weight"], P[pre + "node_mlp_1.0.bias"]
        Ws2, bs2 = P[pre + "node_mlp_1.2.weight"], P[pre + "node_mlp_1.2.bias"]
        if Qt is None:
            Qt = be.lin(Ws1, 0, F, xt, b=bs1)
        hmom = be.empty(8 * F, d.NS)
        msg = be.msg_cache(d) if (self.training or self.want_grad) and \
            hasattr(be, "msg_cache") else None
        if msg is not None:
            mom = be.source_fwd(d, xe3[0], xe3[1], xe3[2], Qt, Ws1, Ws2, bs2, hmom, msg=msg)
        else:
            mom = be.source_fwd(d, xe3[0], xe3[1], xe3[2], Qt, Ws1, Ws2, bs2, hmom)
        hS = [(xs, 0, False), (hmom, F, False), (u, 9 * F, True)]
        st = dict(xs=xs, xt=xt, xe3=xe3, u=u, Qt=Qt, mom=mom, msg=msg)
        if epi:
            names = list(epi)
            xs_new, sS, outs = self.mlp_fwd(P, pre + "node_mlp_2.", hS, pre + "norm.", BN,
                                            epi=[epi[k] for k in names])
            st.update(zip(names, outs))
        else:
            xs_new, sS = self.mlp_fwd(P, pre + "node_mlp_2.", hS, pre + "norm.", BN)
        st.update(sS=sS, xs_new=xs_new)
        return st

    def _mom_epi_ok(self, d, st):
        sS = st.get("sS")
        return (d.sp is None and getattr(self.be, "fiber_bn_sums", False)
                and self.F in (8, 10) and sS is not None and sS[0] != "ops"
                and os.environ.get("PFSGNN_MOM_EPI", "1") != "0"
                and os.environ.get("PFSGNN_MLP_BWD_RS", "1") != "0")

    def source_node_bwd(self, P, Gr, d, pre, st, g_xs_new, g_xs, g_u, bn_part=None):
        be, F, G = self.be, self.F, d.G
        gu = be.empty(F, d.NS)
        if self._mom_epi_ok(d, st):
            coef = be.empty(4, 2 * F, d.NS)
            self.mlp_bwd(P, Gr, pre + "node_mlp_2.", g_xs_new, st["sS"],
                         outs=[(g_xs, F, True), (None, 8 * F, False), (gu, F, False)],
                         bn_part=bn_part, mom_coef=(st["mom"], coef, F, d.NC))
            self._gu_add(gu, G, g_u)
            return coef
        gst = be.empty(8 * F, d.NS)
        self.mlp_bwd(P, Gr, pre + "node_mlp_2.", g_xs_new, st["sS"],
                     outs=[(g_xs, F, True), (gst, 8 * F, False), (gu, F, False)],
                     bn_part=bn_part)
        self._gu_add(gu, G, g_u)
        return be.moment_coef(st["mom"], gst, d.NC if d.sp is None else d.sp.fib_ptr)

    def source_edge_bwd(self, P, Gr, d, pre, st, coef, tpart, g_next, bnstat, g_xt, se=None,
                        epre=None, tmask=None):
        be, F = self.be, self.F
        Ws1, Ws2 = P[pre + "node_mlp_1.0.weight"], P[pre + "node_mlp_1.2.weight"]
        y, sc, sh = st["xe3"]
        bn2 = None
        if se is not None and bnstat is not None:
            key = epre + "norm."
            bn2 = (P[key + "weight"], se["var1"], d.E, self.bn_eps, Gr[key + "weight"],
                   Gr[key + "bias"])
        out = be.source_bwd(
            d, y, sc, sh, st["Qt"], Ws1, Ws2, P[pre + "node_mlp_1.2.bias"], st["mom"][0], coef,
            tpart, g_next, bnstat, Gr[pre + "node_mlp_1.0.weight"], Gr[pre + "node_mlp_1.2.weight"],
            Gr[pre + "node_mlp_1.2.bias"], bn2=bn2, g_xt=g_xt,
            **({"tmask": tmask} if tmask is not None and tpart is not None else {}),
            **({"msg": st["msg"]} if st.get("msg") is not None else {}))
        g_tot, GzS = out[0], out[1]
        be.wgrad(GzS, st["xt"], Gr[pre + "node_mlp_1.0.weight"], col0=0,
                 db=Gr[pre + "node_mlp_1.0.bias"])
        if bn2 is not None:
            return g_tot, out[4]
        return g_tot, out[2], out[3]

    def target_fwd(self, P, BN, d, pre, xs, xt, xe3, u, Rs=None, glob=None):
        be, F = self.be, self.F
        Wt1, bt1 = P[pre + "node_mlp_1.0.weight"], P[pre + "node_mlp_1.0.bias"]
        Wt2, bt2 = P[pre + "node_mlp_1.2.weight"], P[pre + "node_mlp_1.2.bias"]
        if Rs is None:
            Rs = be.lin(Wt1, 0, F, xs, b=bt1)
        tmask = be.tmask(d) if self.training and hasattr(be, "tmask") else None
        if glob is not None and d.sp is None and hasattr(be, "target_block_fwd") and \
                d.G * -(-d.NC // 32) <= 512 and d.NC <= 2048 and \
                os.environ.get("PFSGNN_CLASS_TAIL", "1") != "0":
            return self._target_block_fwd(P, BN, d, pre, xs, xt, xe3, u, Rs, tmask, glob)
        if d.sp is None:
            hsum, agg = be.target_fwd(d, xe3[0], xe3[1], xe3[2], Rs, Wt1,
                                      agg=(Wt2, bt2, float(d.NF)),
                                      **({"tmask": tmask} if tmask is not None else {}))
        else:
            hsum = be.target_fwd(d, xe3[0], xe3[1], xe3[2], Rs, Wt1,
                                 **({"tmask": tmask} if tmask is not None else {}))
            agg = be.lin(Wt2, 0, 2 * F, hsum)
            be.lin(bt2.view(-1, 1), 0, 1, d.sp.deg_t, out=agg, add=True)
        hT = [(xt, 0, False), (agg, F, False), (u, 3 * F, True)]
        st = dict(xs=xs, xt=xt, xe3=xe3, u=u, Rs=Rs, hsum=hsum, tmask=tmask)
        if glob is None:
            xt_new, sT = self.mlp_fwd(P, pre + "node_mlp_2.", hT, pre + "norm.", BN)
            st.update(sT=sT, xt_new=xt_new)
            return st
        pg, pnext = glob
        m2 = pre + "node_mlp_2."
        w = P[pg + "norm.weight"]
        nxt = None
        if pnext is not None:
            pe, ps = pnext + "edge_model.", pnext + "s_model."
            nxt = (P[pe + "0.weight"], P[pe + "0.bias"], P[ps + "node_mlp_1.0.weight"],
                   P[ps + "node_mlp_1.0.bias"])
        r = be.target_global_fwd(hT, d.G, d.NC, P[m2 + "0.weight"], P[m2 + "0.bias"],
                                 P[m2 + "2.weight"], P[m2 + "2.bias"],
                                 self._bn_args(P, BN, pre + "norm."), xs, d.NF, u,
                                 P[pg + "0.weight"], P[pg + "0.bias"], P[pg + "2.weight"],
                                 P[pg + "2.bias"], w, self._rms_eps(u), nxt)
        st.update(sT=(hT, r["Z"], (r["Yp"], r["mu"], r["var"], pre + "norm.")), xt_new=r["xt"])
        st["su"] = dict(sU=([(u, 0, False), (r["means"], F, False)], r["gZ"], None), v=r["gV"],
                        rms=r["rms"], u_new=r["u"], fused=True)
        st["parts_t"] = (r["Pt"], r["Qt"])
        return st

    def _target_block_fwd(self, P, BN, d, pre, xs, xt, xe3, u, Rs, tmask, glob):
        be, F = self.be, self.F
        pg, pnext = glob
        m2 = pre + "node_mlp_2."
        nxt = None
        if pnext is not None:
            pe, ps = pnext + "edge_model.", pnext + "s_model."
            nxt = (P[pe + "0.weight"], P[pe + "0.bias"], P[ps + "node_mlp_1.0.weight"],
                   P[ps + "node_mlp_1.0.bias"])
        r = be.target_block_fwd(d, xe3[0], xe3[1], xe3[2], Rs, P[pre + "node_mlp_1.0.weight"],
                                P[pre + "node_mlp_1.2.weight"], P[pre + "node_mlp_1.2.bias"],
                                tmask, xt, u, P[m2 + "0.weight"], P[m2 + "0.bias"],
                                P[m2 + "2.weight"], P[m2 + "2.bias"],
                                self._bn_args(P, BN, pre + "norm."), xs, P[pg + "0.weight"],
                                P[pg + "0.bias"], P[pg + "2.weight"], P[pg + "2.bias"],
                                P[pg + "norm.weight"], self._rms_eps(u), nxt)
        hT = [(xt, 0, False), (r["agg"], F, False), (u, 3 * F, True)]
        st = dict(xs=xs, xt=xt, xe3=xe3, u=u, Rs=Rs, hsum=r["hsum"], tmask=tmask)
        st.update(sT=(hT, r["Z"], (r["Yp"], r["mu"], r["var"], pre + "norm.")), xt_new=r["xt"])
        st["su"] = dict(sU=([(u, 0, False), (r["means"], F, False)], r["gZ"], None), v=r["gV"],
                        rms=r["rms"], u_new=r["u"], fused=True)
        st["parts_t"] = (r["Pt"], r["Qt"])
        return st

    def _class_bwd_ok(self, d, su, stt):
        sT = stt.get("sT")
        return (d.sp is None and self.normed and self.F in (8, 10, 16) and d.NC <= 1024
                and hasattr(self.be, "target_class_bwd") and su.get("fused")
                and sT is not None and sT[2] is not None and sT[2][0] != "eval"
                and os.environ.get("PFSGNN_CLASS_BWD", "1") != "0")

    def _class_bwd(self, P, Gr, d, p, su, stt, pend, g_u, g_xs_new, g_xt_new, g_xt_in, g_u_in):
        be, F, G = self.be, self.F, d.G
        pg, pt = p + "global_model.", p + "t_model."
        m2 = pt + "node_mlp_2."
        segsU, Zg, _ = su["sU"]
        hT, ZT, (Yp, mu, var, key) = stt["sT"]
        w = P[pg + "norm.weight"]
        gH = P[pg + "0.weight"].shape[0]
        gV, gdZ, dwp = be.empty(F, G), be.empty(gH, G), be.empty(F, G)
        r = be.target_class_bwd(d, pend, g_u, su["v"], w, su["rms"], Zg, P[pg + "0.weight"],
                                P[pg + "2.weight"], gV, gdZ, dwp, g_u_in, g_xs_new, g_xt_new, Yp,
                                mu, var, P[key + "weight"], self.bn_eps, Gr[key + "weight"],
                                Gr[key + "bias"], ZT, P[m2 + "0.weight"], P[m2 + "2.weight"],
                                P[pt + "node_mlp_1.2.weight"], g_xt_in)
        be.wgrad(gV, Zg, Gr[pg + "2.weight"], db=Gr[pg + "2.bias"], act_in=True)
        be.wgrad_cat(gdZ, segsU, Gr[pg + "0.weight"], db=Gr[pg + "0.bias"])
        be.wgrad(dwp, be._ones_row(G), Gr[pg + "norm.weight"].view(F, 1))
        be.wgrad(r["dYp"], ZT, Gr[m2 + "2.weight"], db=Gr[m2 + "2.bias"], act_in=True)
        be.wgrad_cat(r["dZ"], hT, Gr[m2 + "0.weight"], db=Gr[m2 + "0.bias"])
        self._gu_add(r["gu_t"], G, g_u_in)
        be.wgrad(r["g_agg"], stt["hsum"], Gr[pt + "node_mlp_1.2.weight"],
                 db=Gr[pt + "node_mlp_1.2.bias"], dbscale=float(d.NF))
        return r["g_hsum"]

    def target_node_bwd(self, P, Gr, d, pre, st, g_xt_new, g_xt, g_u):
        be, F, G = self.be, self.F, d.G
        g_agg = be.empty(2 * F, d.NT)
        gu = be.empty(F, d.NT)
        self.mlp_bwd(P, Gr, pre + "node_mlp_2.", g_xt_new, st["sT"],
                     outs=[(g_xt, F, True), (g_agg, 2 * F, False), (gu, F, False)])
        self._gu_add(gu, G, g_u)
        Wt2 = P[pre + "node_mlp_1.2.weight"]
        if d.sp is None:
            be.wgrad(g_agg, st["hsum"], Gr[pre + "node_mlp_1.2.weight"],
                     db=Gr[pre + "node_mlp_1.2.bias"], dbscale=float(d.NF))
        else:
            be.wgrad(g_agg, st["hsum"], Gr[pre + "node_mlp_1.2.weight"])
            be.wgrad(g_agg, d.sp.deg_t, Gr[pre + "node_mlp_1.2.bias"].view(-1, 1))
        return be.lin_t(Wt2, 0, 2 * F, g_agg)

    def target_edge_bwd(self, P, Gr, d, pre, st, g_hsum, want_gxe, g_xs, bn_sums=None):
        be, F = self.be, self.F
        Wt1 = P[pre + "node_mlp_1.0.weight"]
        y, sc, sh = st["xe3"]
        kw = {"tmask": st["tmask"]} if st.get("tmask") is not None else {}
        if bn_sums is not None:
            kw["bn_sums"] = bn_sums
        out = be.target_bwd(d, y, sc, sh, st["Rs"], Wt1, g_hsum,
                            Gr[pre + "node_mlp_1.0.weight"], want_gxe=want_gxe,
                            g_xs=g_xs, **kw)
        GzT, gxe = out[0], out[1]
        be.wgrad(GzT, st["xs"], Gr[pre + "node_mlp_1.0.weight"], col0=0,
                 db=Gr[pre + "node_mlp_1.0.bias"])
        return (gxe, out[2]) if bn_sums is not None else gxe

    def global_fwd(self, P, d, pre, xs, xt, u):
        be, F, G = self.be, self.F, d.G
        W1 = P[pre + "0.weight"]
        if 3 * F <= 192 and W1.shape[0] <= 192:
            w = P[pre + "norm.weight"] if self.normed else None
            u_new, means, Z, v, rms = be.global_fwd(
                xs, xt, u, W1, P[pre + "0.bias"], P[pre + "2.weight"], P[pre + "2.bias"], w,
                self._rms_eps(u) if w is not None else 0.0, G)
            sU = ([(u, 0, False), (means, F, False)], Z, None)
            return dict(sU=sU, v=v, rms=rms, u_new=u_new, fused=True)
        hU = [(u, 0, False), (be.graph_mean2(xs, xt, G), F, False)]
        v, sU = self.mlp_fwd(P, pre, hU)
        if self.normed:
            u_new, rms = be.rms2_fwd(v, P[pre + "norm.weight"], self._rms_eps(v))
        else:
            u_new, rms = v, None
        return dict(sU=sU, v=v, rms=rms, u_new=u_new)

    def global_bwd(self, P, Gr, d, pre, st, g_u_new, g_xs, g_xt, g_u):
        be, F = self.be, self.F
        if st.get("fused"):
            pre_w = pre + "norm.weight"
            segs, Z, _ = st["sU"]
            W1, W2 = P[pre + "0.weight"], P[pre + "2.weight"]
            g_v, dZ = be.global_bwd(g_u_new, st["v"], P[pre_w] if self.normed else None, st["rms"],
                                    self._rms_eps(st["v"]), Gr[pre_w] if self.normed else None,
                                    Z, W1, W2, g_u, g_xs, 1.0 / d.NF, g_xt, 1.0 / d.NC)
            be.wgrad(g_v, Z, Gr[pre + "2.weight"], db=Gr[pre + "2.bias"], act_in=True)
            be.wgrad_cat(dZ, segs, Gr[pre + "0.weight"], db=Gr[pre + "0.bias"])
            return
        if self.normed:
            g_v = be.rms2_bwd(g_u_new, st["v"], P[pre + "norm.weight"], st["rms"],
                              self._rms_eps(st["v"]), Gr[pre + "norm.weight"])
        else:
            g_v = g_u_new
        g_m = be.empty(2 * F, d.G)
        self.mlp_bwd(P, Gr, pre, g_v, st["sU"], outs=[(g_u, F, True), (g_m, 2 * F, False)])
        be.graph_bcast_add2(g_xs, 1.0 / d.NF, g_xt, 1.0 / d.NC, g_m)

    def forward(self, P, BN, d, xs_in, xt_in, xe_in, u_in, training=True, want_grad=False):
        self.training = training
        self.want_grad = want_grad
        xs, s_enc = self.mlp_fwd(P, "encoder_s.", xs_in)
        xt, t_enc = self.mlp_fwd(P, "encoder_t.", xt_in)
        ctx = {"d": d, "enc": (s_enc, t_enc), "blocks": [], "training": training,
               "want_grad": want_grad}
        xe3 = (xe_in, None, None)
        u = u_in
        parts = None
        for b in range(self.B):
            p = f"mpb.{b}."
            pn = f"mpb.{b + 1}." if b + 1 < self.B else None
            if parts is None:
                parts = self.node_parts(P, d, p + "edge_model.", p + "s_model.", xs, xt, u)
            se = self.edge_fwd(P, BN, d, p + "edge_model.", xs, xt, xe3, u,
                               parts=None if parts is None else parts[:2])
            xe3n = (se["y"], se["sc"], se["sh"])
            fused = self._fused_tail_ok(P, d, p + "s_model.", p + "t_model.", p + "global_model.")
            epi = None
            if fused:
                F = self.F
                pt1 = p + "t_model.node_mlp_1.0."
                epi = {"Rs": (P[pt1 + "weight"], 0, 2 * F, P[pt1 + "bias"])}
                if pn is not None:
                    epi["Ps_next"] = (P[pn + "edge_model.0.weight"], 0, 4 * F, None)
            ss = self.source_fwd(P, BN, d, p + "s_model.", xs, xt, xe3n, u,
                                 Qt=None if parts is None else parts[2], epi=epi)
            stt = self.target_fwd(P, BN, d, p + "t_model.", ss["xs_new"], xt, xe3n, u,
                                  Rs=ss.get("Rs"),
                                  glob=(p + "global_model.", pn) if fused else None)
            if fused:
                su = stt.pop("su")
                pt = stt.pop("parts_t")
                parts = (ss["Ps_next"],) + tuple(pt) if pn is not None else None
            else:
                su = self.global_fwd(P, d, p + "global_model.", ss["xs_new"], stt["xt_new"], u)
                parts = None
            ctx["blocks"].append((se, ss, stt, su))
            xs, xt, xe3, u = ss["xs_new"], stt["xt_new"], xe3n, su["u_new"]
        ctx["out"] = (xs, xt, xe3, u)
        return ctx

    def backward(self, P, Gr, ctx, g_xe_out=None, g_xs_out=None, g_xt_out=None, g_u_out=None):
        d, be, F = ctx["d"], self.be, self.F
        if not ctx.get("training", True) and not ctx.get("want_grad", False):
            raise NotImplementedError("this eval-mode forward ran for inference only (forward "
                                      "with want_grad=True to differentiate through it)")
        be.defer_begin()
        g_bn_part = ctx.pop("g_xe_bn_part", None)
        try:
            self._backward(P, Gr, ctx, d, g_xs_out, g_xt_out, g_xe_out, g_u_out, g_bn_part)
        finally:
            self._gu_pend = None
            be.defer_flush()

    def _backward(self, P, Gr, ctx, d, g_xs_out, g_xt_out, g_xe_out, g_u_out, g_bn_part=None):
        be, F = self.be, self.F
        g_xs, g_xt, g_xe, g_u = g_xs_out, g_xt_out, g_xe_out, g_u_out
        self._gu_pend = []
        prev_pend = []
        stride = (F * (d.NS + d.NT + d.G) + 63) // 64 * 64
        acc_all = be.zeros(self.B * stride)
        for b in reversed(range(self.B)):
            se, ss, stt, su = ctx["blocks"][b]
            p = f"mpb.{b}."
            acc = acc_all[b * stride:b * stride + F * (d.NS + d.NT + d.G)]
            g_xs_in = acc[:F * d.NS].view(F, d.NS)
            g_xt_in = acc[F * d.NS:F * (d.NS + d.NT)].view(F, d.NT)
            g_u_in = acc[F * (d.NS + d.NT):].view(F, d.G)
            live_t = g_u is not None or g_xt is not None
            live_s = live_t or g_xs is not None
            bnstat = self.edge_bnstat(P, p + "edge_model.", se) if self.normed else None
            ev = "rm" in se
            if live_s:
                own = b < self.B - 1
                g_xs_new = be.zeros(F, d.NS) if g_xs is None else (g_xs if own else g_xs.clone())
                g_xt_new = be.zeros(F, d.NT) if g_xt is None else (g_xt if own else g_xt.clone())
                tpart = None
                if (g_u is not None and live_t and len(prev_pend) <= 4
                        and all(tg is g_u for _, tg in prev_pend)
                        and self._class_bwd_ok(d, su, stt)):
                    g_hsum = self._class_bwd(P, Gr, d, p, su, stt, [X for X, _ in prev_pend],
                                             g_u, g_xs_new, g_xt_new, g_xt_in, g_u_in)
                    prev_pend = []
                else:
                    self._gu_flush_list(prev_pend, d.G)
                    prev_pend = []
                    if g_u is not None:
                        self.global_bwd(P, Gr, d, p + "global_model.", su, g_u, g_xs_new,
                                        g_xt_new, g_u_in)
                    if live_t:
                        g_hsum = self.target_node_bwd(P, Gr, d, p + "t_model.", stt, g_xt_new,
                                                      g_xt_in, g_u_in)
                bn_part = None
                if live_t:
                    bn_sums = self._fiber_bn_sums(d, ss)
                    r = self.target_edge_bwd(P, Gr, d, p + "t_model.", stt, g_hsum, False,
                                             g_xs_new, bn_sums=bn_sums)
                    if bn_sums is not None:
                        bn_part = r[1]
                    tpart = (stt["Rs"], P[p + "t_model.node_mlp_1.0.weight"], g_hsum)
                coef = self.source_node_bwd(P, Gr, d, p + "s_model.", ss, g_xs_new, g_xs_in, g_u_in,
                                            bn_part=bn_part)
                g_tot, *bnc = self.source_edge_bwd(P, Gr, d, p + "s_model.", ss, coef, tpart,
                                                   g_xe, bnstat, g_xt_in,
                                                   se=None if ev else se,
                                                   epre=p + "edge_model.",
                                                   tmask=stt.get("tmask") if live_t else None)
                if not self.normed:
                    bnc = None
                elif ev:
                    bnc = self.edge_bn_coef(P, Gr, d, p + "edge_model.", se, *bnc)
                else:
                    bnc = bnc[0]
            else:
                g_tot = be.zeros(F, d.EP) if g_xe is None else g_xe
                bnc = None
                if self.normed and b == self.B - 1 and g_xe is not None and g_bn_part is not None:
                    key = p + "edge_model.norm."
                    bnc = be.bn2_bwd_coef_part(g_bn_part, se["mu1"], se["var1"], P[key + "weight"],
                                               d.E, self.bn_eps, Gr[key + "weight"],
                                               Gr[key + "bias"])
                elif self.normed:
                    Sg, Sgx = be.edge_bn_grad_sums(d, g_tot, se["y"], *bnstat)
                    bnc = self.edge_bn_coef(P, Gr, d, p + "edge_model.", se, Sg, Sgx)
            g_xe = self.edge_bwd(P, Gr, d, p + "edge_model.", se, g_tot, bnc, b > 0,
                                 g_xs_in, g_xt_in, g_u_in)
            self._gu_flush_list(prev_pend, d.G)
            prev_pend, self._gu_pend = self._gu_pend, []
            g_xs, g_xt, g_u = g_xs_in, g_xt_in, g_u_in
        self._gu_flush_list(prev_pend, d.G)
        s_enc, t_enc = ctx["enc"]
        self.mlp_bwd(P, Gr, "encoder_s.", g_xs, s_enc)
        self.mlp_bwd(P, Gr, "encoder_t.", g_xt, t_enc)

    def loss_forward(self, P, d, xe3, ci, sharpness, seed, pclass=0.1, pfiber=0.1, total_time=42.0,
                     nfields=10, wutils=2000.0, wvar=1.0, noiselevel=0.3, want_time=False):
        be = self.be
        y, sc, sh = xe3
        scale = total_time / d.NC
        dec = [P["decoder_e.0.weight"], P["decoder_e.0.bias"], P["decoder_e.2.weight"], P["decoder_e.2.bias"]]
        n_prime, fiber_time, tmean, tvar, tt = be.loss_fwd(d, y, sc, sh, *dec, ci, scale, sharpness,
                                                          noiselevel, seed, want_time)
        loss, utils, variance, Gn, Gf, Gv = be.loss_finalize(d, n_prime, fiber_time, tvar, ci, pclass,
                                                             pfiber, total_time, nfields, wutils, wvar)
        lctx = dict(d=d, xe3=xe3, ci=ci, scale=scale, sharpness=sharpness, noiselevel=noiselevel,
                    seed=seed, tmean=tmean, Gn=Gn, Gf=Gf, Gv=Gv)
        diag = dict(loss=loss, utils=utils, variance=variance, n_prime=n_prime,
                    fiber_time=fiber_time, time=tt)
        return loss.sum(), diag, lctx

    def loss_bnstat(self, ectx):
        blocks = ectx.get("blocks") if ectx is not None else None
        if (not blocks or not self.normed or not ectx.get("training", True)
                or not getattr(self.be, "loss_bn_part", False)
                or os.environ.get("PFSGNN_LOSS_BN_SUMS", "1") == "0"):
            return None
        se = blocks[-1][0]
        if "rm" in se or se.get("inv1") is None:
            return None
        return se["mu1"], se["inv1"]

    def loss_backward(self, P, Gr, lctx, gscale=1.0, bnstat=None):
        be, d = self.be, lctx["d"]
        y, sc, sh = lctx["xe3"]
        dec = [P["decoder_e.0.weight"], P["decoder_e.0.bias"], P["decoder_e.2.weight"], P["decoder_e.2.bias"]]
        kw = {"bn": bnstat} if bnstat is not None else {}
        return be.loss_bwd(d, y, sc, sh, *dec, lctx["ci"], lctx["scale"], lctx["sharpness"],
                           lctx["noiselevel"], lctx["seed"], lctx["Gn"], lctx["Gf"], lctx["Gv"],
                           lctx["tmean"], gscale,
                           Gr["decoder_e.0.weight"], Gr["decoder_e.0.bias"],
                           Gr["decoder_e.2.weight"], Gr["decoder_e.2.bias"], **kw)
```

### pfs-neural-net_amd/pfsgnn/native.py

```python
import ctypes
import os

import torch

from .sparse import SparseEdgeOps, SparseGeo

_LIB_PATH = os.path.join(os.path.dirname(os.path.abspath(__file__)), "libpfsgnn.so")
if os.environ.get("PFSGNN_LIB_VARIANT"):
    _LIB_PATH = os.path.join(os.path.dirname(_LIB_PATH),
                             "libpfsgnn_" + os.environ["PFSGNN_LIB_VARIANT"] + ".so")
if os.environ.get("PFSGNN_LIB_PATH"):
    _LIB_PATH = os.environ["PFSGNN_LIB_PATH"]


class NativeUnavailable(RuntimeError):
    pass


_lib = None

P = ctypes.c_void_p
I = ctypes.c_int
LL = ctypes.c_longlong
FL = ctypes.c_float
# ... 89 lines not shown
                        "We", "be", "Ws", "bs", "Pt", "Qt"))

_SIGS = {
    "pfsgnn_version": ([], ctypes.c_char_p),
    "pfsgnn_last_error": ([], ctypes.c_char_p),
    "pfsgnn_workspace_bytes": ([I, I, I, I], SZ),
    "pfsgnn_set_edge_path": ([I], I),
    "pfsgnn_sync_bytes": ([], SZ),
    "pfsgnn_set_sync_buffer": ([P, SZ], I),
    "pfsgnn_get_edge_path": ([], I),
    "pfsgnn_edge_grid": ([I, I, I, ctypes.POINTER(ctypes.c_int)], I),
    "pfsgnn_timing_enable": ([I], I),
    "pfsgnn_timing_reset": ([], I),
    "pfsgnn_timing_repeat": ([ctypes.c_char_p, I], I),
    "pfsgnn_timing_query": ([ctypes.c_char_p, ctypes.POINTER(ctypes.c_double),
                             ctypes.POINTER(ctypes.c_longlong)], I),
    "pfsgnn_lin": ([P, I, I, I, P, I, P, FL, I, P, I, P], I),
    "pfsgnn_lin_t": ([P, I, I, I, P, I, P, P, I, P], I),
    "pfsgnn_lin_gather": ([P, I, I, I, P, I, P, FL, I, P, I, P, P, I, P, P, I, P], I),
    "pfsgnn_wgrad": ([P, I, P, I, I, I, P, I, P, FL, P, SZ, P], I),
    "pfsgnn_lin_cat": ([P, I, I, SEGP, I, I, P, FL, I, P, I, P], I),
    "pfsgnn_wgrad_cat": ([P, I, SEGP, I, I, I, P, I, P, FL, P, SZ, P], I),
    "pfsgnn_wgrad_part_bytes": ([I, I, I, I], SZ),
    "pfsgnn_wgrad_cat_part": ([P, I, SEGP, I, I, I, P, I, P, FL, P, SZ, REDP,
                               ctypes.POINTER(ctypes.c_int), P], I),
    "pfsgnn_reduce_batch": ([REDP, I, P], I),
    "pfsgnn_wgrad_multi_bytes": ([WGJP, I], SZ),
    "pfsgnn_gemm_multi": ([GMJP, I, P], I),
    "pfsgnn_wgrad_multi": ([WGJP, I, P, SZ, P], I),
    "pfsgnn_defer_begin": ([P, SZ], I),
    "pfsgnn_defer_end": ([P], I),
    "pfsgnn_defer_end_multi": ([WGJP, I, P, SZ, P], I),
    "pfsgnn_defer_need": ([], SZ),
    "pfsgnn_bn_fwd": ([P, I, I, P, P, P, P, FL, FL, P, P, P, P, SZ, P], I),
    "pfsgnn_bn_bwd": ([P, P, P, P, P, FL, I, I, P, P, P, P, SZ, P], I),
    "pfsgnn_mlp_ws_bytes": ([I], SZ),
    "pfsgnn_mlp_fwd": ([SEGP, I, I, P, I, I, P, P, I, P, P, P, P, P, P, P, FL, FL, P, P, P, P,
                        SZ, P], I),
    "pfsgnn_mlp_fwd_epi": ([SEGP, I, I, P, I, I, P, P, I, P, P, P, P, P, P, P, FL, FL, P, P, P,
                            LINMP, I, P, SZ, P], I),
    "pfsgnn_target_global_fwd": ([SEGP, I, I, I, P, I, I, P, P, I, P, P, P, P, P, P, P, FL, FL,
                                  P, P, P, P, I, P, P, I, P, P, P, P, FL] + [P] * 7
                                 + [P] * 6 + [P, SZ, P], I),
    "pfsgnn_mlp_bwd": ([P, I, P, P, P, P, FL, P, P, P, P, I, I, I, P, I, P, P, OSEGP, I, P, SZ,
                        P], I),
    "pfsgnn_mlp_bwd_pre": ([P, I, P, P, P, P, FL, P, P, P, P, I, I, I, P, I, P, P, OSEGP, I, P, I,
                            P, P, I, I, I, P, SZ, P], I),
    "pfsgnn_build_complete": ([I, I, I, I, P, P], I),
    "pfsgnn_graph_reduce": ([P, I, I, I, I, P, P], I),
    "pfsgnn_graph_reduce_add": ([P, I, I, I, I, P, P], I),
    "pfsgnn_graph_bcast_add": ([P, I, I, I, P, FL, P], I),
    "pfsgnn_graph_reduce_multi": ([P, P, I, I, I, P, P], I),
    "pfsgnn_graph_mean2": ([P, I, P, I, I, I, P, P], I),
    "pfsgnn_graph_bcast_add2": ([P, I, FL, P, I, FL, I, I, P, P], I),
    "pfsgnn_rms2_fwd": ([P, I, I, P, FL, P, P, P, P, P], I),
    "pfsgnn_rms2_bwd": ([P, P, P, P, P, P, I, I, FL, P, P, P, SZ, P], I),
    "pfsgnn_global_fwd": ([P, I, P, I, P, I, I, P, I, P, P, P, P, FL] + [P] * 7 + [P], I),
    "pfsgnn_global_bwd": ([P, P, P, P, P, P, I, I, P, I, P, P, P, P, P, P, P, P, I, FL, P, I,
                           FL, P], I),
    "pfsgnn_bn2_finalize": ([P, P, P, P, P, P, I, LL, FL, FL, P, P, P, P, P], I),
    "pfsgnn_bn_eval_coef": ([P, P, P, P, I, FL, I, P, P, P], I),
    "pfsgnn_affine_rows": ([P, I, I, P, P, P, P], I),
    "pfsgnn_bn2_bwd_coef": ([P, P, P, P, P, I, LL, FL, P, P, P, P, P, P], I),
    "pfsgnn_bn2_bwd_coef_part": ([P, I, I, P, P, P, LL, FL, P, P, P, P, P, P], I),
    "pfsgnn_moment_coef": ([P, P, I, I, I, P, P], I),
    "pfsgnn_moment_coef_seg": ([P, P, I, I, P, P, P], I),
    "pfsgnn_sparse_layout_ws_bytes": ([LL], SZ),
    "pfsgnn_sparse_layout": ([P, LL, I, I, I, P, P, P, P, P, P, P, P, SZ, P], I),
    "pfsgnn_gather_cols": ([P, I, I, P, LL, P, I, P, P], I),
    "pfsgnn_segment_sum": ([P, I, LL, P, P, I, I, P, I, P], I),
    "pfsgnn_segment_moments": ([P, I, LL, P, I, P, P, P], I),
    "pfsgnn_segment_moment_grad": ([P, I, LL, P, P, P, I, P, P], I),
    "pfsgnn_rows_ws_bytes": ([I, LL], SZ),
    "pfsgnn_rows_stats": ([P, I, LL, P, P, P, SZ, P], I),
    "pfsgnn_rows_bn_sums": ([P, P, I, LL, P, P, P, P, P, SZ, P], I),
    "pfsgnn_rows_axpby": ([P, P, I, LL, P, P, P, P, P], I),
    "pfsgnn_edge_mlp_fwd": ([I, I, I, I, P, P, P, P, P, P, P, P, P, P, P, P, SZ, P], I),
    "pfsgnn_edge_mlp_fwd_bn": ([I, I, I, I] + [P] * 15 + [FL, FL, P, P, P, P, P, SZ, P], I),
    "pfsgnn_source_fwd": ([I, I, I, I, P, P, P, P, P, P, P, P, P, P, SZ, P], I),
    "pfsgnn_target_fwd": ([I, I, I, I, P, P, P, P, P, P, P, P, FL, P, P, P, SZ, P], I),
    "pfsgnn_tmask_bytes": ([I, I, I, I], SZ),
    "pfsgnn_target_bwd": ([I, I, I, I, P, P, P, P, P, P, P, P, P, P, P, P, SZ, P], I),
    "pfsgnn_target_bwd_bn": ([I, I, I, I] + [P] * 14 + [FL, P, P, SZ, P], I),
    "pfsgnn_source_bwd": ([I, I, I, I] + [P] * 24 + [P, SZ, P], I),
    "pfsgnn_source_bwd_bn": ([I, I, I, I] + [P] * 17 + [LL, FL] + [P] * 12 + [P, SZ, P], I),
    "pfsgnn_msg_bytes": ([I, I, I, I], SZ),
    "pfsgnn_source_fwd_msg": ([I, I, I, I, P, P, P, P, P, P, P, P, P, P, P, SZ, P], I),
    "pfsgnn_source_bwd_msg": ([I, I, I, I] + [P] * 25 + [P, SZ, P], I),
    "pfsgnn_source_bwd_bn_msg": ([I, I, I, I] + [P] * 17 + [LL, FL] + [P] * 13 + [P, SZ, P], I),
    "pfsgnn_edge_bn_grad_sums": ([I, I, I, I, P, P, P, P, P, P, P, SZ, P], I),
    "pfsgnn_edge_mlp_bwd": ([I, I, I, I] + [P] * 21 + [P, SZ, P], I),
    "pfsgnn_loss_fwd": ([I, I, I, I, P, P, P, P, P, P, P, P, FL, FL, FL, ULL, P, P, P, P, P, P, P, SZ, P], I),
    "pfsgnn_loss_finalize": ([I, I, I, P, P, P, P, FL, FL, FL, FL, FL, FL, P, P, P, P, P, P, P], I),
    "pfsgnn_loss_bwd": ([I, I, I, I, P, P, P, P, P, P, P, P, FL, FL, FL, ULL, P, P, P, P, P, P,
                         P, P, P, P, P, P, SZ, P], I),
    "pfsgnn_loss_bn_parts": ([I, I, I], I),
    "pfsgnn_loss_bwd_bn": ([I, I, I, I, P, P, P, P, P, P, P, P, FL, FL, FL, ULL, P, P, P, P, P,
                            P, P, P, P, P, P, P, P, P, P, SZ, P], I),
    "pfsgnn_layout_analyze": ([P, LL, I, I, I, P, P, P, SZ, P], I),
    "pfsgnn_edges_to_canonical": ([P, I, I, I, I, I, P, P, P], I),
    "pfsgnn_edges_from_canonical": ([P, P, P, I, I, I, I, I, P, I, P, P], I),
    "pfsgnn_adam": ([P, P, P, P, LL, I, P, ctypes.c_double, ctypes.c_double, ctypes.c_double,
                     ctypes.c_double, ctypes.c_double, P, P], I),
    "pfsgnn_sliced_max_nc": ([I, ctypes.POINTER(ctypes.c_int)], I),
    "pfsgnn_target_block_fwd": ([ctypes.POINTER(BlockTail), P, SZ, P], I),
    "pfsgnn_sync_faults": ([ctypes.POINTER(ctypes.c_uint)], I),
    "pfsgnn_set_grid_sync_fenced": ([I], I),
    "pfsgnn_block_tail_bytes": ([], SZ),
    "pfsgnn_target_class_bwd": ([ctypes.POINTER(ClassBwd), P, SZ, P], I),
    "pfsgnn_class_bwd_bytes": ([], SZ),
    "pfsgnn_bn_eval_bwd_coef": ([P, P, P, P, I, FL, I, P, P, P, P, P, P, P], I),
    "pfsgnn_sliced_plan_ws_bytes": ([I, I], SZ),
    "pfsgnn_sliced_plan": ([P, I, I, P, P, P, P, P, P, SZ, P], I),
    "pfsgnn_sliced_fill": ([P, P, P, P, LL, I, I, P, P, LL, I, P, P, P, P], I),
    "pfsgnn_edges_to_slots": ([P, LL, LL, I, P, P, P], I),
    "pfsgnn_edges_from_slots": ([P, P, P, LL, LL, I, P, I, P, P], I),
    "pfsgnn_sl_tmask_bytes": ([SLP, I], SZ),
}
for _op in ("edge_mlp_fwd", "edge_mlp_fwd_bn", "source_fwd", "target_fwd", "target_bwd",
            "source_bwd", "source_bwd_bn", "edge_mlp_bwd"):
    _SIGS["pfsgnn_sl_" + _op] = ([SLP] + _SIGS["pfsgnn_" + _op][0], I)


def lib():
    global _lib
    if _lib is None:
        if not os.path.exists(_LIB_PATH):
            raise NativeUnavailable(
                f"{_LIB_PATH} not found: build it with `make -C pfs-neural-net_amd` "
                "(or __graft_entry__.build()); there is no non-HIP fallback")
        L = ctypes.CDLL(_LIB_PATH)
        for name, (args, ret) in _SIGS.items():
            fn = getattr(L, name)
            fn.argtypes = args
            fn.restype = ret
        _lib = L
        path = os.environ.get("PFSGNN_EDGE_PATH")
        if path:
            set_edge_path(path)
    return _lib


EDGE_PATHS = {"valu": 0, "mfma": 1, "mfma32": 2, "bf16y": 3, "bf16": 4, "bf16m": 5, "bf16x3": 6,
              "bf16x6": 7}


def set_edge_path(path):
    if path not in EDGE_PATHS:
        raise ValueError(f"edge path must be one of {sorted(EDGE_PATHS)}, got {path!r}")
    _check(lib().pfsgnn_set_edge_path(EDGE_PATHS[path]), "pfsgnn_set_edge_path")


def get_edge_path():
    code = lib().pfsgnn_get_edge_path()
    return {v: k for k, v in EDGE_PATHS.items()}[code]


def edge_grid(G, NF, NC):
    info = (ctypes.c_int * 4)()
    _check(lib().pfsgnn_edge_grid(int(G), int(NF), int(NC), info), "pfsgnn_edge_grid")
    return dict(KS=info[0], CPS=info[1], nblocks=info[2], NFG=info[3])


def exported_symbols():
    return list(_SIGS.keys())

# ... 690 lines not shown
            _call("pfsgnn_sl_" + op, sl.ref, *args)

    def edge_mlp_fwd(self, d, xe, xsc, xsh, Ps, Pt, W1, W2, b2):
        if self._composed(d):
            return self._sp.edge_mlp_fwd(d, xe, xsc, xsh, Ps, Pt, W1, W2, b2)
        self._set_dims(d)
        y, mu, var = self.empty(d.F, d.EP), self.empty(d.F), self.empty(d.F)
        self._chk(xe, Ps, Pt, W1, W2, b2)
        ws, wsb = self._wsargs(d)
        self._ecall("edge_mlp_fwd", d, d.G, d.NF, d.NC, d.F, xe.data_ptr(), _ptr(xsc), _ptr(xsh),
              Ps.data_ptr(), Pt.data_ptr(), W1.data_ptr(), W2.data_ptr(), b2.data_ptr(),
              y.data_ptr(), mu.data_ptr(), var.data_ptr(), ws, wsb, _stream())
        return y, mu, var

    def edge_mlp_fwd_bn(self, d, xe, xsc, xsh, Ps, Pt, W1, W2, b2, bn):
        gamma, beta, rm, rv, momentum, eps = bn
        if self._composed(d):
            y, mu, var = self._sp.edge_mlp_fwd(d, xe, xsc, xsh, Ps, Pt, W1, W2, b2)
            sc, sh, inv1, _ = self.bn2_finalize(mu, var, gamma, beta, rm, rv, d.E, momentum, eps)
            return y, mu, var, sc, sh, inv1
        self._set_dims(d)
        F = d.F
        y, mu, var = self.empty(F, d.EP), self.empty(F), self.empty(F)
        sc, sh, inv1, inv2 = self.empty(F), self.empty(F), self.empty(F), self.empty(F)
        self._chk(xe, Ps, Pt, W1, W2, b2, gamma, beta, rm, rv)
        ws, wsb = self._wsargs(d)
        self._ecall("edge_mlp_fwd_bn", d, d.G, d.NF, d.NC, F, xe.data_ptr(), _ptr(xsc), _ptr(xsh),
              Ps.data_ptr(), Pt.data_ptr(), W1.data_ptr(), W2.data_ptr(), b2.data_ptr(),
              y.data_ptr(), mu.data_ptr(), var.data_ptr(), gamma.data_ptr(), beta.data_ptr(),
              _ptr(rm), _ptr(rv), float(momentum), float(eps), sc.data_ptr(), sh.data_ptr(),
              inv1.data_ptr(), inv2.data_ptr(), ws, wsb, _stream())
        return y, mu, var, sc, sh, inv1

    def source_fwd(self, d, y, sc, sh, Qt, Ws1, Ws2, bs2, hs_out, msg=None):
        if self._composed(d):
            return self._sp.source_fwd(d, y, sc, sh, Qt, Ws1, Ws2, bs2, hs_out)
        mom = self.empty(4, 2 * d.F, d.NS)
        self._chk(y, Qt, Ws1, Ws2, bs2, hs_out)
        ws, wsb = self._wsargs(d)
        args = (d.G, d.NF, d.NC, d.F, y.data_ptr(), _ptr(sc), _ptr(sh), Qt.data_ptr(),
                Ws1.data_ptr(), Ws2.data_ptr(), bs2.data_ptr(), mom.data_ptr(), hs_out.data_ptr())
        if msg is not None:
            _call("pfsgnn_source_fwd_msg", *args, msg.data_ptr(), ws, wsb, _stream())
        else:
            self._ecall("source_fwd", d, *args, ws, wsb, _stream())
        return mom

    def msg_cache(self, d):
        if self._composed(d) or d.sp is not None:
            return None
        n = lib().pfsgnn_msg_bytes(d.G, d.NF, d.NC, d.F)
        return torch.empty(n // 4, dtype=torch.float32, device=self.device) if n else None

    def tmask(self, d):
        if self._composed(d):
            return None
        if d.sp is not None:
            n = lib().pfsgnn_sl_tmask_bytes(d.sp.sl.ref, d.F)
            return torch.empty(n, dtype=torch.uint8, device=self.device) if n else None
        n = lib().pfsgnn_tmask_bytes(d.G, d.NF, d.NC, d.F)
        return torch.empty(n, dtype=torch.uint8, device=self.device) if n else None

    def target_fwd(self, d, y, sc, sh, Rs, Wt1, agg=None, tmask=None):
        if self._composed(d):
            hsum = self._sp.target_fwd(d, y, sc, sh, Rs, Wt1)
            if agg is None:
                return hsum
            Wt2, bt2, bscale = agg
            return hsum, self.lin(Wt2, 0, Wt2.shape[1], hsum, b=bt2, bscale=bscale)
        hsum = self.empty(2 * d.F, d.NT)
        Wt2 = bt2 = A = None
        bscale = 1.0
        if agg is not None:
            Wt2, bt2, bscale = agg
            self._chk(Wt2, bt2)
            assert Wt2.shape == (2 * d.F, 2 * d.F)
            A = self.empty(2 * d.F, d.NT)
        ws, wsb = self._wsargs(d)
        self._ecall("target_fwd", d, d.G, d.NF, d.NC, d.F, y.data_ptr(), _ptr(sc), _ptr(sh),
              Rs.data_ptr(), Wt1.data_ptr(), hsum.data_ptr(), _ptr(Wt2), _ptr(bt2),
              float(bscale), _ptr(A), _ptr(tmask), ws, wsb, _stream())
        return hsum if agg is None else (hsum, A)

    def target_bwd(self, d, y, sc, sh, Rs, Wt1, g_hsum, dWt1, want_gxe=False, g_xs=None,
                   tmask=None, bn_sums=None):
        if bn_sums is not None:
            assert g_xs is not None and not self._composed(d) and d.sp is None
            Yp, mu, var, eps = bn_sums
            self._chk(g_xs, Yp, mu, var)
            GzT = self.empty(2 * d.F, d.NS)
            gxe = self.empty(d.F, d.EP) if want_gxe else None
            part = self.empty((d.NS + 63) // 64, 32)
            g_hsum = g_hsum.contiguous()
            ws, wsb = self._wsargs(d)
            _call("pfsgnn_target_bwd_bn", d.G, d.NF, d.NC, d.F, y.data_ptr(), _ptr(sc), _ptr(sh),
                  Rs.data_ptr(), Wt1.data_ptr(), g_hsum.data_ptr(), GzT.data_ptr(),
                  dWt1.data_ptr(), _ptr(gxe), g_xs.data_ptr(), _ptr(tmask), Yp.data_ptr(),
                  mu.data_ptr(), var.data_ptr(), float(eps), part.data_ptr(), ws, wsb, _stream())
            return GzT, gxe, part
        if self._composed(d):
            out = self._sp.target_bwd(d, y, sc, sh, Rs, Wt1, g_hsum, dWt1, want_gxe=want_gxe)
            if g_xs is not None:
                self.lin_t(Wt1, 0, d.F, out[0], out=g_xs, add=True)
            return out
        self._chk(g_xs)
        GzT = self.empty(2 * d.F, d.NS)
        gxe = self.empty(d.F, d.EP) if want_gxe else None
        g_hsum = g_hsum.contiguous()
        ws, wsb = self._wsargs(d)
        self._ecall("target_bwd", d, d.G, d.NF, d.NC, d.F, y.data_ptr(), _ptr(sc), _ptr(sh),
              Rs.data_ptr(), Wt1.data_ptr(), g_hsum.data_ptr(), GzT.data_ptr(), dWt1.data_ptr(),
              _ptr(gxe), _ptr(g_xs), _ptr(tmask), ws, wsb, _stream())
        return GzT, gxe

    def source_bwd(self, d, y, sc, sh, Qt, Ws1, Ws2, bs2, mean, coef, tpart, g_next, bnstat,
                   dWs1, dWs2, dbs2, bn2=None, g_xt=None, tmask=None, msg=None):
        if self._composed(d):
            out = self._sp.source_bwd(d, y, sc, sh, Qt, Ws1, Ws2, bs2, mean, coef, tpart, g_next,
                                      bnstat, dWs1, dWs2, dbs2)
            if g_xt is not None:
                self.lin_t(Ws1, 0, d.F, out[1], out=g_xt, add=True)
            if bn2 is None:
                return out
            gamma, var1, n, eps, dg, db = bn2
            cf = self.bn2_bwd_coef(out[2], out[3], bnstat[0], var1, gamma, n, eps, dg, db)
            return out[0], out[1], None, None, cf
        g_tot = self.empty(d.F, d.EP)
        GzS = self.empty(2 * d.F, d.NT)
        Rs = Wt1 = g_hsum = None
        if tpart is not None:
            Rs, Wt1, g_hsum = tpart
            g_hsum = g_hsum.contiguous()
        mu1 = inv1 = Sg = Sgx = None
        if bnstat is not None:
            mu1, inv1 = bnstat
            if bn2 is None:
                Sg, Sgx = self.empty(d.F), self.empty(d.F)
        mean = mean.contiguous()
        if g_next is not None:
            g_next = g_next.contiguous()
        ws, wsb = self._wsargs(d)
        head = (d.G, d.NF, d.NC, d.F, y.data_ptr(), _ptr(sc), _ptr(sh), Qt.data_ptr(),
                Ws1.data_ptr(), Ws2.data_ptr(), bs2.data_ptr(), mean.data_ptr(), coef.data_ptr(),
                _ptr(Rs), _ptr(Wt1), _ptr(g_hsum), _ptr(g_next), _ptr(mu1), _ptr(inv1))
        if bn2 is not None:
            assert bnstat is not None
            gamma, var1, n, eps, dg, db = bn2
            a, g0, g1 = self.empty(d.F), self.empty(d.F), self.empty(d.F)
            tail = (var1.data_ptr(), gamma.data_ptr(), int(n), float(eps), g_tot.data_ptr(),
                    GzS.data_ptr(), dWs1.data_ptr(), dWs2.data_ptr(), dbs2.data_ptr(),
                    a.data_ptr(), g0.data_ptr(), g1.data_ptr(), dg.data_ptr(), db.data_ptr(),
                    _ptr(g_xt), _ptr(tmask))
            if msg is not None:
                _call("pfsgnn_source_bwd_bn_msg", *head, *tail, msg.data_ptr(), ws, wsb, _stream())
            else:
                self._ecall("source_bwd_bn", d, *head, *tail, ws, wsb, _stream())
            return g_tot, GzS, None, None, (a, g0, g1)
        tail = (g_tot.data_ptr(), GzS.data_ptr(), dWs1.data_ptr(), dWs2.data_ptr(),
                dbs2.data_ptr(), _ptr(Sg), _ptr(Sgx), _ptr(g_xt), _ptr(tmask))
        if msg is not None:
            _call("pfsgnn_source_bwd_msg", *head, *tail, msg.data_ptr(), ws, wsb, _stream())
        else:
            self._ecall("source_bwd", d, *head, *tail, ws, wsb, _stream())
        return g_tot, GzS, Sg, Sgx

    def edge_bn_grad_sums(self, d, g, y, mu1, inv1):
        if d.sp is not None:
            return self._sp.edge_bn_grad_sums(d, g, y, mu1, inv1)
        Sg, Sgx = self.empty(d.F), self.empty(d.F)
        ws, wsb = self._wsargs(d)
        _call("pfsgnn_edge_bn_grad_sums", d.G, d.NF, d.NC, d.F, g.data_ptr(), y.data_ptr(),
              mu1.data_ptr(), inv1.data_ptr(), Sg.data_ptr(), Sgx.data_ptr(), ws, wsb, _stream())
        return Sg, Sgx

    def edge_mlp_bwd(self, d, g_tot, alpha, gam0, gam1, y, xe, xsc, xsh, Ps, Pt, W1, W2,
                     dW1, dW2, db2, want_gxe=True, nodes=None):
        if self._composed(d):
            out = self._sp.edge_mlp_bwd(d, g_tot, alpha, gam0, gam1, y, xe, xsc, xsh, Ps, Pt, W1,
                                        W2, dW1, dW2, db2, want_gxe=want_gxe)
            if nodes is None:
                return out
            F = d.F
            self.lin_t(W1, 0, F, out[1], out=nodes[0], add=True)
            self.lin_t(W1, F, F, out[2], out=nodes[1], add=True)
            return out + (self.lin_t(W1, 3 * F, F, out[2]),)
        gxe = self.empty(d.F, d.EP) if want_gxe else None
        GzEs, GzEt = self.empty(4 * d.F, d.NS), self.empty(4 * d.F, d.NT)
        g_xs = g_xt = Vu = None
        if nodes is not None:
            g_xs, g_xt = nodes
            self._chk(g_xs, g_xt)
            Vu = self.empty(d.F, d.NT)
        ws, wsb = self._wsargs(d)
        self._ecall("edge_mlp_bwd", d, d.G, d.NF, d.NC, d.F, g_tot.data_ptr(), alpha.data_ptr(),
              gam0.data_ptr(), gam1.data_ptr(), y.data_ptr(), xe.data_ptr(), _ptr(xsc), _ptr(xsh),
              Ps.data_ptr(), Pt.data_ptr(), W1.data_ptr(), W2.data_ptr(), dW1.data_ptr(),
              dW2.data_ptr(), db2.data_ptr(), _ptr(gxe), GzEs.data_ptr(), GzEt.data_ptr(),
              _ptr(g_xs), _ptr(g_xt), _ptr(Vu), ws, wsb, _stream())
        return (gxe, GzEs, GzEt) if nodes is None else (gxe, GzEs, GzEt, Vu)

    def edge_apply(self, d, y, sc, sh):
        if d.sp is not None:
            return self._sp.edge_apply(d, y, sc, sh)
        out = self.empty(d.F, d.E)
        _call("pfsgnn_edges_from_canonical", y.data_ptr(), _ptr(sc), _ptr(sh), d.G, d.NF, d.NC,
              d.F, 2, None, 0, out.data_ptr(), _stream())
        return out

    def _seed_args(self, seed):
        if isinstance(seed, torch.Tensor):
            if not seed.is_cuda or seed.dtype != torch.int64 or seed.numel() != 1:
                raise ValueError("a tensor seed must be one int64 on the device")
            return 0, seed.data_ptr()
        return int(seed) & ((1 << 64) - 1), None

    def loss_fwd(self, d, y, sc, sh, Wd1, bd1, Wd2, bd2, ci, scale, sharpness, noiselevel, seed,
                 want_time=False):
        n_prime, fiber_time = self.empty(d.NT), self.empty(d.NS)
        tmean, tvar = self.empty(d.NT), self.empty(d.NT)
        tt = self.empty(d.E) if want_time else None
        ci = ci.contiguous()
        ws, wsb = self._wsargs(d)
        _call("pfsgnn_loss_fwd", d.G, d.NF, d.NC, d.F, y.data_ptr(), _ptr(sc), _ptr(sh),
              Wd1.data_ptr(), bd1.data_ptr(), Wd2.data_ptr(), bd2.data_ptr(), ci.data_ptr(),
              float(scale), float(sharpness), float(noiselevel), *self._seed_args(seed),
              n_prime.data_ptr(), fiber_time.data_ptr(), tmean.data_ptr(), tvar.data_ptr(),
              _ptr(tt), ws, wsb, _stream())
# ... 221 lines not shown
```

Baseline: 509.5 million edges/s.

## Fold target-model weight-gradient accumulation into the source backward kernel

```diff
diff --git a/include/pfsgnn.h b/include/pfsgnn.h
--- a/include/pfsgnn.h
+++ b/include/pfsgnn.h
@@ -366,6 +366,24 @@
                              float* dgamma, float* dbeta, float* g_xt,
                              const unsigned char* tmask, const float* msg, void* ws,
                              size_t ws_bytes, void* stream);
+int pfsgnn_tbwd_fold(int F);
+int pfsgnn_target_bwd_fold(int G, int NF, int NC, int F, const float* y, const float* sc,
+                           const float* sh, const float* Rs, const float* Wt1,
+                           const float* g_hsum, float* GzT, float* dWt1, float* gxe, float* g_xs,
+                           const unsigned char* tmask, const float* bn_Yp, const float* bn_mu,
+                           const float* bn_var, float bn_eps, float* bn_part, void* ws,
+                           size_t ws_bytes, void* stream);
+int pfsgnn_source_bwd_fold(int G, int NF, int NC, int F, const float* y, const float* sc,
+                           const float* sh, const float* Qt, const float* Ws1, const float* Ws2,
+                           const float* bs2, const float* mean, const float* coef,
+                           const float* Rs, const float* Wt1, const float* g_hsum,
+                           const float* g_next, const float* mu1, const float* inv1,
+                           const float* var1, const float* gamma, long long n, float eps,
+                           float* g_tot, float* GzS, float* dWs1, float* dWs2, float* dbs2,
+                           float* Sg, float* Sgx, float* alpha, float* gam0, float* gam1,
+                           float* dgamma, float* dbeta, float* g_xt, const unsigned char* tmask,
+                           const float* msg, float* dWt1, void* ws, size_t ws_bytes,
+                           void* stream);
 int pfsgnn_edge_bn_grad_sums(int G, int NF, int NC, int F, const float* g, const float* y,
                              const float* mu1, const float* inv1, float* Sg, float* Sgx,
                              void* ws, size_t ws_bytes, void* stream);
diff --git a/pfs-neural-net_amd/csrc/pfsgnn_edge.hip b/pfs-neural-net_amd/csrc/pfsgnn_edge.hip
--- a/pfs-neural-net_amd/csrc/pfsgnn_edge.hip
+++ b/pfs-neural-net_amd/csrc/pfsgnn_edge.hip
@@ -1458,7 +1458,7 @@
   edge = std::max(edge, ks * 4 * C * NS + C * NS + 1024);
   edge = std::max(edge, colp * C + 1024);
   edge = std::max(edge, nb * C * F + ks * C * NS + 1024);
-  edge = std::max(edge, nb * (C * (C + 1) + C * F + 2 * F) + colp * C + 4096);
+  edge = std::max(edge, nb * (C * (C + 1) + 2 * C * F + 2 * F) + colp * C + 4096);
   edge = std::max(edge, nb * (F * (H + 1) + H * F) + colp * H + ks * H * NS + 4096);
   edge = std::max(edge, colp * 4 + ks * NS + nb * (F * (F + 1) + F + 1) + 4096);
   edge += (size_t)geo.NT * (H + 2 * C) + 4 * H * H + 8 * 256;
@@ -1799,7 +1799,7 @@
                            const float* Wt1, const float* g_hsum, float* GzT, float* dWt1,
                            float* gxe, float* g_xs, const unsigned char* tmask, void* ws,
                            size_t ws_bytes, void* stream,
-                           const FiberBnSums& bs = FiberBnSums{}) {
+                           const FiberBnSums& bs = FiberBnSums{}, bool fold = false) {
   if (int rc = check_dims("pfsgnn_target_bwd", G, NF, NC, F)) return rc;
   if (int rc = check_sliced("pfsgnn_target_bwd", sl, NC, F)) return rc;
   PF_REQUIRE(y && Rs && Wt1 && g_hsum && GzT && dWt1, "pfsgnn_target_bwd", "null");
@@ -1807,13 +1807,13 @@
   const int C = 2 * F;
   Ws w{reinterpret_cast<char*>(ws), ws_bytes};
   hipStream_t st = as_stream(stream);
-  float* part = pf::defer_take((size_t)geo.nblocks * C * F);
+  float* part = fold ? nullptr : pf::defer_take((size_t)geo.nblocks * C * F);
   const bool defer = part != nullptr;
-  if (!defer) part = w.take((size_t)geo.nblocks * C * F);
+  if (!defer && !fold) part = w.take((size_t)geo.nblocks * C * F);
   float* gz = fiber_dst(geo, C, GzT, w);
   const float* ghT = (sl || use_mfma()) ? g_hsum
                                        : class_rows(g_hsum, C, geo, w, st);
-  PF_REQUIRE(part && gz && ghT, "pfsgnn_target_bwd", "workspace too small");
+  PF_REQUIRE((part || fold) && gz && ghT, "pfsgnn_target_bwd", "workspace too small");
   { pf::Timer tm_("target_bwd", st);
   if (sl) {
     float* tabs = w.take((size_t)pfm::sl_tab_floats(geo, F));
@@ -1835,9 +1835,11 @@
                                                            geo.NS),
                                 no_lin(), st, bs))
     return rc;
-  const RedDesc rd{part, geo.nblocks, (size_t)C * F, F, C, F, dWt1 + F, C, 1, 1.f};
-  if (defer) pf::defer_push(&rd, 1);
-  else launch_reduce_multi(&rd, 1, st);
+  if (!fold) {
+    const RedDesc rd{part, geo.nblocks, (size_t)C * F, F, C, F, dWt1 + F, C, 1, 1.f};
+    if (defer) pf::defer_push(&rd, 1);
+    else launch_reduce_multi(&rd, 1, st);
+  }
   return pf::check_launch("pfsgnn_target_bwd");
 }
 
@@ -1861,6 +1863,24 @@
   return target_bwd_impl(nullptr, G, NF, NC, F, y, sc, sh, Rs, Wt1, g_hsum, GzT, dWt1, gxe, g_xs,
                          tmask, ws, ws_bytes, stream,
                          FiberBnSums{bn_Yp, bn_mu, bn_var, bn_eps, bn_part});
+}
+
+static bool tbwd_folds(int F) { return use_mfma() && pfm::source_bwd_folds(F, mf_prec(1, F)); }
+
+extern "C" int pfsgnn_tbwd_fold(int F) { return tbwd_folds(F) ? 1 : 0; }
+
+extern "C" int pfsgnn_target_bwd_fold(int G, int NF, int NC, int F, const float* y,
+                                      const float* sc, const float* sh, const float* Rs,
+                                      const float* Wt1, const float* g_hsum, float* GzT,
+                                      float* dWt1, float* gxe, float* g_xs,
+                                      const unsigned char* tmask, const float* bn_Yp,
+                                      const float* bn_mu, const float* bn_var, float bn_eps,
+                                      float* bn_part, void* ws, size_t ws_bytes, void* stream) {
+  PF_REQUIRE(!bn_part || (g_xs && bn_Yp && bn_mu && bn_var), "pfsgnn_target_bwd_fold",
+             "BatchNorm sums need g_xs, Yp, mu, var");
+  const FiberBnSums bs = bn_part ? FiberBnSums{bn_Yp, bn_mu, bn_var, bn_eps, bn_part} : FiberBnSums{};
+  return target_bwd_impl(nullptr, G, NF, NC, F, y, sc, sh, Rs, Wt1, g_hsum, GzT, dWt1, gxe, g_xs,
+                         tmask, ws, ws_bytes, stream, bs, tmask && !gxe && tbwd_folds(F));
 }
 
 extern "C" int pfsgnn_sl_target_bwd(const pfsgnn_sliced_t* sl, int G, int NF, int NC, int F,
@@ -1948,7 +1968,7 @@
                            const float* inv1, float* g_tot, float* GzS, float* dWs1, float* dWs2,
                            float* dbs2, float* Sg, float* Sgx, const Bn2Bwd* bb, float* g_xt,
                            const unsigned char* tmask, void* ws, size_t ws_bytes, void* stream,
-                           const float* msg = nullptr);
+                           const float* msg = nullptr, float* dWt1f = nullptr);
 
 extern "C" int pfsgnn_source_bwd(int G, int NF, int NC, int F, const float* y, const float* sc,
                                  const float* sh, const float* Qt, const float* Ws1,
@@ -2016,6 +2036,29 @@
                          &bb, g_xt, tmask, ws, ws_bytes, stream, msg);
 }
 
+extern "C" int pfsgnn_source_bwd_fold(
+    int G, int NF, int NC, int F, const float* y, const float* sc, const float* sh,
+    const float* Qt, const float* Ws1, const float* Ws2, const float* bs2, const float* mean,
+    const float* coef, const float* Rs, const float* Wt1, const float* g_hsum,
+    const float* g_next, const float* mu1, const float* inv1, const float* var1,
+    const float* gamma, long long n, float eps, float* g_tot, float* GzS, float* dWs1,
+    float* dWs2, float* dbs2, float* Sg, float* Sgx, float* alpha, float* gam0, float* gam1,
+    float* dgamma, float* dbeta, float* g_xt, const unsigned char* tmask, const float* msg,
+    float* dWt1, void* ws, size_t ws_bytes, void* stream) {
+  const char* where = "pfsgnn_source_bwd_fold";
+  PF_REQUIRE(dWt1 && tmask && Rs, where, "the folded pair needs dWt1, tmask and TModel's part");
+  if (!gamma)
+    return source_bwd_impl(nullptr, G, NF, NC, F, y, sc, sh, Qt, Ws1, Ws2, bs2, mean, coef, Rs,
+                           Wt1, g_hsum, g_next, mu1, inv1, g_tot, GzS, dWs1, dWs2, dbs2, Sg, Sgx,
+                           nullptr, g_xt, tmask, ws, ws_bytes, stream, msg, dWt1);
+  PF_REQUIRE(mu1 && inv1 && var1 && n > 0 && alpha && gam0 && gam1 && dgamma && dbeta, where,
+             "null");
+  const Bn2Bwd bb{gamma, mu1, var1, n, eps, alpha, gam0, gam1, dgamma, dbeta};
+  return source_bwd_impl(nullptr, G, NF, NC, F, y, sc, sh, Qt, Ws1, Ws2, bs2, mean, coef, Rs, Wt1,
+                         g_hsum, g_next, mu1, inv1, g_tot, GzS, dWs1, dWs2, dbs2, nullptr, nullptr,
+                         &bb, g_xt, tmask, ws, ws_bytes, stream, msg, dWt1);
+}
+
 extern "C" int pfsgnn_sl_source_bwd(const pfsgnn_sliced_t* sl, int G, int NF, int NC, int F,
                                     const float* y, const float* sc, const float* sh,
                                     const float* Qt, const float* Ws1, const float* Ws2,
@@ -2057,7 +2100,7 @@
                            const float* inv1, float* g_tot, float* GzS, float* dWs1, float* dWs2,
                            float* dbs2, float* Sg, float* Sgx, const Bn2Bwd* bb, float* g_xt,
                            const unsigned char* tmask, void* ws, size_t ws_bytes, void* stream,
-                           const float* msg) {
+                           const float* msg, float* dWt1f) {
   if (int rc = check_dims("pfsgnn_source_bwd", G, NF, NC, F)) return rc;
   PF_REQUIRE(!msg || (!sl && msg_bytes(G, NF, NC, F) > 0), "pfsgnn_source_bwd_msg",
              "the message cache is not kept on this path (pfsgnn_msg_bytes is 0)");
@@ -2072,10 +2115,13 @@
   const int C = 2 * F;
   const size_t nb = geo.nblocks;
   Ws w{reinterpret_cast<char*>(ws), ws_bytes};
-  float* pW2 = pf::defer_take(nb * C * (C + 1) + nb * C * F);
+  const bool fold = dWt1f && tmask && Rs && !sl && tbwd_folds(F);
+  const size_t nW = nb * C * (C + 1) + nb * C * F * (fold ? 2 : 1);
+  float* pW2 = pf::defer_take(nW);
   const bool defer = pW2 != nullptr;
-  if (!defer) pW2 = w.take(nb * C * (C + 1) + nb * C * F);
+  if (!defer) pW2 = w.take(nW);
   float* pW1 = pW2 ? pW2 + nb * C * (C + 1) : nullptr;
+  float* pWt = fold && pW1 ? pW1 + nb * C * F : nullptr;
   float* pCol = w.take((size_t)G * col_bpg(geo, sl) * NC * C);
   float* pBN = w.take(nb * 2 * F);
   hipStream_t st = as_stream(stream);
@@ -2096,7 +2142,7 @@
     for (int rep = 0, nrep = 1 + pf::repeats("source_bwd"); rep < nrep; ++rep)
       if (int rc = pfm::source_bwd(geo, F, msg, y, sc, sh, QtT, Ws1, Ws2, bs2, mean, coef, Rs, Wt1,
                                    ghT, g_next, mu1, inv1, g_tot, pW2, pW1, pCol, pBN, tmask,
-                                   mf_prec(1, F), st))
+                                   mf_prec(1, F), st, pWt))
         return rc;
   } else {
   DISPATCH_F(F, hipLaunchKernelGGL(k_source_bwd<FF>, dim3(edge_grid(geo)), dim3(256), 0, st, geo, y,
@@ -2105,17 +2151,19 @@
   }
   tm_.end(); }
   {
-    RedDesc rd[5] = {{pBN, (int)nb, (size_t)2 * F, F, 1, F, Sg, F, 0, 1.f},
+    RedDesc rd[6] = {{pBN, (int)nb, (size_t)2 * F, F, 1, F, Sg, F, 0, 1.f},
                      {pBN + F, (int)nb, (size_t)2 * F, F, 1, F, Sgx, F, 0, 1.f},
                      {pW2, (int)nb, (size_t)C * (C + 1), C + 1, C, C, dWs2, C, 1, 1.f},
                      {pW2 + C, (int)nb, (size_t)C * (C + 1), C + 1, C, 1, dbs2, 1, 1, 1.f},
-                     {pW1, (int)nb, (size_t)C * F, F, C, F, dWs1 + F, C, 1, 1.f}};
+                     {pW1, (int)nb, (size_t)C * F, F, C, F, dWs1 + F, C, 1, 1.f},
+                     {pWt, (int)nb, (size_t)C * F, F, C, F, fold ? dWt1f + F : nullptr, C, 1, 1.f}};
+    const int nw = fold ? 4 : 3;
     const bool sums = mu1 && !bb;
     const RedDesc* now = sums ? rd : rd + 2;
-    int nnow = sums ? 5 : 3;
+    int nnow = (sums ? 2 : 0) + nw;
     if (defer) {
-      pf::defer_push(rd + 2, 3);
-      nnow -= 3;
+      pf::defer_push(rd + 2, nw);
+      nnow -= nw;
     }
     if (nnow) launch_reduce_multi(now, nnow, st);
   }
diff --git a/pfs-neural-net_amd/csrc/pfsgnn_mfma.h b/pfs-neural-net_amd/csrc/pfsgnn_mfma.h
--- a/pfs-neural-net_amd/csrc/pfsgnn_mfma.h
+++ b/pfs-neural-net_amd/csrc/pfsgnn_mfma.h
@@ -28,7 +28,8 @@
                const float* bs2, const float* mean, const float* coef, const float* Rs,
                const float* Wt1, const float* ghS, const float* g_next, const float* mu1,
                const float* inv1, float* g_tot, float* pW2, float* pW1, float* pCol, float* pBN,
-               const uint8_t* tmask, int prec, hipStream_t st);
+               const uint8_t* tmask, int prec, hipStream_t st, float* pWt = nullptr);
+bool source_bwd_folds(int F, int prec);
 int edge_mlp_bwd(const EdgeGeo& geo, int F, const float* g_tot, const float* alpha,
                  const float* gam0, const float* gam1, const float* y, const float* xe,
                  const float* xsc, const float* xsh, const float* Ps, const float* PtS,
diff --git a/pfs-neural-net_amd/csrc/pfsgnn_mfma.hip b/pfs-neural-net_amd/csrc/pfsgnn_mfma.hip
--- a/pfs-neural-net_amd/csrc/pfsgnn_mfma.hip
+++ b/pfs-neural-net_amd/csrc/pfsgnn_mfma.hip
@@ -595,7 +595,7 @@
 #endif
 }
 
-template <int F, int PREC, bool TM>
+template <int F, int PREC, bool TM, bool NW = false>
 __global__ __launch_bounds__(256) void km_target_bwd(EdgeGeo geo, const float* __restrict__ y,
                                                      const float* __restrict__ sc,
                                                      const float* __restrict__ sh,
@@ -607,18 +607,19 @@
                                                      float* __restrict__ partW,
                                                      const uint8_t* __restrict__ tmask) {
   constexpr int C = 2 * F, NT = GM<C>::NT;
+  static_assert(!NW || TM, "the mask-only form reads the mask");
   constexpr int NIMG = NT + 1;
   using WI = WgImg<PREC>;
   MF_GEO
-  __shared__ __attribute__((aligned(16))) short imgs[4 * NIMG * WI::U];
-  __shared__ float scratch[4 * C * F];
+  __shared__ __attribute__((aligned(16))) short imgs[NW ? 4 : 4 * NIMG * WI::U];
+  __shared__ float scratch[NW ? 1 : 4 * C * F];
   __shared__ __attribute__((aligned(16))) float ghl[MF_MAX_CPS * ClassRows<C>::CP];
   ClassRows<C>::stage(ghl, ghS, geo.NT, (long long)gg * geo.NC + c0, c1 - c0);
   short* img = imgs + wave * NIMG * WI::U;
   FwdLayer<FP(PREC), C, F> L1;
   if constexpr (!TM) L1.load([&](int h, int k) { return Wt1[h * 2 * F + F + k]; }, lane);
   GradLayer<PREC, F, C> LT;
-  LT.load([&](int k, int h) { return gxe ? Wt1[h * 2 * F + F + k] : 0.f; }, lane);
+  if constexpr (!NW) LT.load([&](int k, int h) { return gxe ? Wt1[h * 2 * F + F + k] : 0.f; }, lane);
   floatx4 rs[NT], accF[NT], accW[NT];
 #pragma unroll
   for (int tt = 0; tt < NT; ++tt) {
@@ -634,12 +635,12 @@
   auto load = [&](int c) {
     Rows<1> r;
     const uint32_t co = (uint32_t)c * eoc;
-    r.v[0] = ld_frows<F>(ry, co, ro);
+    if constexpr (NW) r.v[0] = zero4(); else r.v[0] = ld_frows<F>(ry, co, ro);
     if constexpr (TM) r.m = __builtin_amdgcn_raw_buffer_load_b8(rtm, eo0 + g4, co, 0);
     return r;
   };
-  class_stream<MF_DEPTH_BWD>(c0, c1, load, [&](const Rows<1>& rows, int c) {
-    const floatx4 x[1] = {edge_in<F>(rows.v[0], fm, sc, scv, shv)};
+  class_stream<NW ? 2 * MF_DEPTH_BWD : MF_DEPTH_BWD>(c0, c1, load, [&](const Rows<1>& rows, int c) {
+    [[maybe_unused]] const floatx4 x[1] = {edge_in<F>(rows.v[0], fm, sc, scv, shv)};
     floatx4 z[NT], gz[NT];
     if constexpr (!TM) {
 #pragma unroll
@@ -657,6 +658,7 @@
       }
       accF[tt] += gz[tt];
     }
+    if constexpr (NW) return;
     Fr sgz[NT];
 #pragma unroll
     for (int tt = 0; tt < NT; ++tt) sgz[tt] = split(gz[tt]);
@@ -684,13 +686,14 @@
         if (h >= 0) GzT[(size_t)ks * C * NS + (size_t)h * NS + n] = accF[tt][r];
       }
   }
-  block_partial(accW, scratch, C * F, [&](int a, int s, int jj) {
-    const int h = GM<C>::mrow(a, s), k = GM<F>::mrow(0, jj);
-    return (h >= 0 && k >= 0) ? h * F + k : -1;
-  }, partW + (size_t)bx * C * F);
-}
-
-template <int F, int PREC, bool TM, bool MSG = false>
+  if constexpr (!NW)
+    block_partial(accW, scratch, C * F, [&](int a, int s, int jj) {
+      const int h = GM<C>::mrow(a, s), k = GM<F>::mrow(0, jj);
+      return (h >= 0 && k >= 0) ? h * F + k : -1;
+    }, partW + (size_t)bx * C * F);
+}
+
+template <int F, int PREC, bool TM, bool MSG = false, bool TW = false>
 __global__ __launch_bounds__(256, 2) void km_source_bwd(
     EdgeGeo geo, const float* __restrict__ msg, const float* __restrict__ y, const float* __restrict__ sc,
     const float* __restrict__ sh, const float* __restrict__ QtS, const float* __restrict__ Ws1,
@@ -699,10 +702,12 @@
     const float* __restrict__ ghS, const float* __restrict__ g_next,
     const float* __restrict__ mu1, const float* __restrict__ inv1, float* __restrict__ g_tot,
     float* __restrict__ partW2, float* __restrict__ partW1, float* __restrict__ partCol,
-    float* __restrict__ partBN, const uint8_t* __restrict__ tmask) {
+    float* __restrict__ partBN, const uint8_t* __restrict__ tmask,
+    float* __restrict__ partWt) {
+  static_assert(!TW || TM, "the folded TModel weight gradient reads the mask");
   constexpr int C = 2 * F, NT = GM<C>::NT;
   constexpr bool PACK = MF_SB_PACK && NT == 2 && GM<C>::nreg(1) == 1 && GM<F>::NT == 1 && GM<F>::RPG == 3;
-  constexpr int NIMG = PACK ? 5 : 3 * NT + 1;
+  constexpr int NIMG = (PACK ? 5 : 3 * NT + 1) + (TW ? (PACK ? 1 : NT) : 0);
   constexpr int SCR = C * (C + 1) > C * F ? C * (C + 1) : C * F;
   using WI = WgImg<PREC>;
   MF_GEO
@@ -723,7 +728,9 @@
   short* im_r3 = img + 2 * WI::U;
   short* im_c1 = img + 3 * WI::U;
   short* im_c2 = img + 4 * WI::U;
-  (void)im_r1; (void)im_r2; (void)im_r3; (void)im_c1; (void)im_c2;
+  short* im_r4 = img + 5 * WI::U;
+  short* im_zt = im_x + WI::U;
+  (void)im_r1; (void)im_r2; (void)im_r3; (void)im_c1; (void)im_c2; (void)im_r4; (void)im_zt;
   const long long CNS = (long long)C * NS;
   const bool tpart = Rs != nullptr;
 
@@ -770,7 +777,9 @@
   [[maybe_unused]] const RowOff<C> roC(eo0, RB, g4);
 
   floatx4 accW2[NT * NT], accW1[NT], accB[NT];
-  floatx4 accP[5];
+  constexpr int NP = TW ? 7 : 5, NPI = TW ? 6 : 5;
+  floatx4 accP[NP];
+  [[maybe_unused]] floatx4 accWt[NT];
 #pragma unroll
   for (int tt = 0; tt < NT; ++tt) {
     accW1[tt] = zero4();
@@ -779,7 +788,9 @@
     for (int nb = 0; nb < NT; ++nb) accW2[tt * NT + nb] = zero4();
   }
 #pragma unroll
-  for (int i = 0; i < 5; ++i) accP[i] = zero4();
+  for (int i = 0; i < NP; ++i) accP[i] = zero4();
+#pragma unroll
+  for (int tt = 0; tt < NT; ++tt) accWt[tt] = zero4();
   floatx4 sg = zero4(), sgx = zero4();
   const s16x8 ones = ones_reg();
   __syncthreads();
@@ -840,12 +851,30 @@
       for (int r = 0; r < GM<C>::nreg(tt); ++r) gz[tt][r] *= dlrelu(zs[tt][r]);
       sgz[tt] = split(gz[tt]);
     }
+    [[maybe_unused]] floatx4 ztw[NT];
+    [[maybe_unused]] Fr sztw[NT];
+    if constexpr (TW) {
+#pragma unroll
+      for (int tt = 0; tt < NT; ++tt) {
+        const floatx4 gh = ClassRows<C>::get(ghl, c - c0, tt, g4);
+#pragma unroll
+        for (int r = 0; r < 4; ++r)
+          ztw[tt][r] = (fvalid && r < GM<C>::nreg(tt)) ? gh[r] * mask_slope(rows.m, 4 * tt + r) : 0.f;
+        sztw[tt] = split(ztw[tt]);
+      }
+    }
     lds_order();
     [[maybe_unused]] floatx4 r3v, c2v;
     if constexpr (PACK) {
       r3v = floatx4{gm[1][0], gz[1][0], 0.f, 0.f};
       c2v = floatx4{as[1][0], x[0][0], x[0][1], x[0][2]};
-      const Fr sr3 = {s16x4{sgm[1].h[0], sgz[1].h[0], 0, 0}, s16x4{sgm[1].l[0], sgz[1].l[0], 0, 0}};
+      Fr sr3 = {s16x4{sgm[1].h[0], sgz[1].h[0], 0, 0}, s16x4{sgm[1].l[0], sgz[1].l[0], 0, 0}};
+      if constexpr (TW) {
+        r3v[2] = ztw[1][0];
+        sr3.h[2] = sztw[1].h[0];
+        sr3.l[2] = sztw[1].l[0];
+        WI::put(im_r4, lane, ztw[0], sztw[0]);
+      }
       WI::put(im_r1, lane, gm[0], sgm[0]);
       WI::put(im_r2, lane, gz[0], sgz[0]);
       WI::put(im_r3, lane, r3v, sr3);
@@ -859,13 +888,18 @@
         WI::put(im_gz + tt * WI::U, lane, gz[tt], sgz[tt]);
       }
       WI::put(im_x, lane, x[0], split(x[0]));
+      if constexpr (TW) {
+#pragma unroll
+        for (int tt = 0; tt < NT; ++tt) WI::put(im_zt + tt * WI::U, lane, ztw[tt], sztw[tt]);
+      }
     }
     lds_order();
 #if MF_WG_EARLY_READS
-    typename WI::R rx, ra[NT], rgm[NT], rgz[NT], rp[5], rq[2];
+    typename WI::R rx, ra[NT], rgm[NT], rgz[NT], rp[NPI], rq[2];
+    [[maybe_unused]] typename WI::R rzt[NT];
     if constexpr (PACK) {
 #pragma unroll
-      for (int i = 0; i < 5; ++i) rp[i] = WI::rd(img + i * WI::U, lane);
+      for (int i = 0; i < NPI; ++i) rp[i] = WI::rd(img + i * WI::U, lane);
 #if MF_WG4
       lds_order();
       rq[0] = WI::rd(im_c1, lane);
@@ -878,13 +912,16 @@
         ra[tt] = WI::rd(im_a + tt * WI::U, lane);
         rgm[tt] = WI::rd(im_gm + tt * WI::U, lane);
         rgz[tt] = WI::rd(im_gz + tt * WI::U, lane);
+        if constexpr (TW) rzt[tt] = WI::rd(im_zt + tt * WI::U, lane);
       }
     }
     lds_order();
 #endif
     floatx4 g[1] = {zero4()};
     if constexpr (PREC >= 1) L1sT.apply(sgz, g); else L1sT.apply(gz, g);
-    if (tpart) {
+    if constexpr (TW) {
+      if constexpr (PREC >= 1) L1tT.apply(sztw, g); else L1tT.apply(ztw, g);
+    } else if (tpart) {
       floatx4 zt[NT];
       if constexpr (!TM) {
 #pragma unroll
@@ -933,6 +970,11 @@
       accP[2] = WI::mma4(t2, tc2, accP[2]);
       accP[3] = WI::mma4(t3, tc1, accP[3]);
       accP[4] = WI::mma4(t3, tc2, accP[4]);
+      if constexpr (TW) {
+        const typename WI::TB tx3 = WI::B(rp[4]);
+        accP[5] = WI::mma(WI::A(rp[5]), tx3, accP[5]);
+        accP[6] = WI::mma(t3, tx3, accP[6]);
+      }
 #else
       const typename WI::TB tc1 = WI::B(rp[3]), tc2 = WI::B(rp[4]);
       accP[0] = WI::mma(t1, tc1, accP[0]);
@@ -940,6 +982,10 @@
       accP[2] = WI::mma(t2, tc2, accP[2]);
       accP[3] = WI::mma(t3, tc1, accP[3]);
       accP[4] = WI::mma(t3, tc2, accP[4]);
+      if constexpr (TW) {
+        accP[5] = WI::mma(WI::A(rp[5]), tc2, accP[5]);
+        accP[6] = WI::mma(t3, tc2, accP[6]);
+      }
 #endif
       const floatx4 cs2 = WI::colsum(t2, gz[0], ones), cs3 = WI::colsum(t3, r3v, ones);
       if (j16 == WI::CS_LANE) {
@@ -977,6 +1023,13 @@
       const typename WI::TA tgz = WI::A(im_gz + tt * WI::U, lane);
 #endif
       accW1[tt] = WI::mma(tgz, tx, accW1[tt]);
+      if constexpr (TW) {
+#if MF_WG_EARLY_READS
+        accWt[tt] = WI::mma(WI::A(rzt[tt]), tx, accWt[tt]);
+#else
+        accWt[tt] = WI::mma(WI::A(im_zt + tt * WI::U, lane), tx, accWt[tt]);
+#endif
+      }
       const floatx4 cs = WI::colsum(tgz, gz[tt]);
       if (j16 == WI::CS_LANE) {
 #pragma unroll
@@ -1037,6 +1090,22 @@
       const int h = GM<C>::mrow(a, s), k = GM<F>::mrow(0, jj);
       return (h >= 0 && k >= 0) ? h * F + k : -1;
     }, partW1 + (size_t)bx * C * F);
+  }
+  if constexpr (TW) {
+    if constexpr (PACK) {
+      block_partial(accP, scratch, C * F, [&](int a, int s, int jj) {
+        int h = -1, k = -1;
+        if ((jj & 3) != 0) k = GM<F>::row(jj >> 2, (jj & 3) - 1);
+        if (a == 5) h = GM<C>::mrow(0, s);
+        if (a == 6 && (s & 3) == 2) h = GM<C>::row(s >> 2, 4);
+        return (h >= 0 && k >= 0) ? h * F + k : -1;
+      }, partWt + (size_t)bx * C * F);
+    } else {
+      block_partial(accWt, scratch, C * F, [&](int a, int s, int jj) {
+        const int h = GM<C>::mrow(a, s), k = GM<F>::mrow(0, jj);
+        return (h >= 0 && k >= 0) ? h * F + k : -1;
+      }, partWt + (size_t)bx * C * F);
+    }
   }
   if (mu1) {
     __syncthreads();
@@ -1364,12 +1433,35 @@
 int target_bwd(const EdgeGeo& geo, int F, const float* y, const float* sc, const float* sh,
                const float* Rs, const float* Wt1, const float* ghS, float* gz, float* gxe,
                float* part, const uint8_t* tmask, int prec, hipStream_t st) {
-  if (tmask) {
+  if (!part) {
+    if (!tmask || gxe || !source_bwd_folds(F, prec))
+      return pf::fail("pfsgnn mfma", "target_bwd: no mask-only form for this call");
+#define MF_CASE_NW(FF, PP)                                                                      \
+  case FF * 8 + PP:                                                                             \
+    hipLaunchKernelGGL((km_target_bwd<FF, PP, true, true>), dim3(edge_grid(geo)), dim3(256), 0, \
+                       st, geo, y, sc, sh, Rs, Wt1, ghS, gz, gxe, part, tmask);                 \
+    break;
+    switch (F * 8 + prec) {
+      MF_CASE_NW(8, 0) MF_CASE_NW(8, 1) MF_CASE_NW(10, 0) MF_CASE_NW(10, 1) MF_CASE_NW(10, 2)
+      MF_CASE_NW(10, 3) MF_CASE_NW(10, 4)
+      default: return pf::fail("pfsgnn mfma", "unsupported Fdim for this edge path");
+    }
+#undef MF_CASE_NW
+  } else if (tmask) {
     MF_LAUNCH3(F, prec, true, km_target_bwd, y, sc, sh, Rs, Wt1, ghS, gz, gxe, part, tmask)
   } else {
     MF_LAUNCH3(F, prec, false, km_target_bwd, y, sc, sh, Rs, Wt1, ghS, gz, gxe, part, tmask)
   }
   return 0;
+}
+
+bool source_bwd_folds(int F, int prec) {
+  switch (F * 8 + prec) {
+    case 8 * 8 + 0: case 8 * 8 + 1: case 10 * 8 + 0: case 10 * 8 + 1: case 10 * 8 + 2:
+    case 10 * 8 + 3: case 10 * 8 + 4:
+      return true;
+  }
+  return false;
 }
 
 int source_bwd(const EdgeGeo& geo, int F, const float* msg, const float* y, const float* sc,
@@ -1377,14 +1469,41 @@
                const float* bs2, const float* mean, const float* coef, const float* Rs,
                const float* Wt1, const float* ghS, const float* g_next, const float* mu1,
                const float* inv1, float* g_tot, float* pW2, float* pW1, float* pCol, float* pBN,
-               const uint8_t* tmask, int prec, hipStream_t st) {
+               const uint8_t* tmask, int prec, hipStream_t st, float* pWt) {
+  if (pWt) {
+    if (!(tmask && Rs) || !source_bwd_folds(F, prec))
+      return pf::fail("pfsgnn mfma", "source_bwd: no folded form for this call");
+    if (msg && prec != 0 && prec != 1) return pf::fail("pfsgnn mfma", "message cache: mfma paths only");
+#define MF_CASE_TW(FF, PP, MM)                                                                   \
+  case FF * 8 + PP:                                                                             \
+    hipLaunchKernelGGL((km_source_bwd<FF, PP, true, MM, true>), dim3(edge_grid(geo)), dim3(256), 0, \
+                       st, geo, msg, y, sc, sh, QtS, Ws1, Ws2, bs2, mean, coef, Rs, Wt1, ghS,     \
+                       g_next, mu1, inv1, g_tot, pW2, pW1, pCol, pBN, tmask, pWt);              \
+    break;
+    if (msg) {
+      switch (F * 8 + prec) {
+        MF_CASE_TW(8, 0, true) MF_CASE_TW(8, 1, true) MF_CASE_TW(10, 0, true)
+        MF_CASE_TW(10, 1, true)
+        default: return pf::fail("pfsgnn mfma", "unsupported Fdim for this edge path");
+      }
+    } else {
+      switch (F * 8 + prec) {
+        MF_CASE_TW(8, 0, false) MF_CASE_TW(8, 1, false) MF_CASE_TW(10, 0, false)
+        MF_CASE_TW(10, 1, false) MF_CASE_TW(10, 2, false) MF_CASE_TW(10, 3, false)
+        MF_CASE_TW(10, 4, false)
+        default: return pf::fail("pfsgnn mfma", "unsupported Fdim for this edge path");
+      }
+    }
+#undef MF_CASE_TW
+    return 0;
+  }
   if (msg) {
     if (prec != 0 && prec != 1) return pf::fail("pfsgnn mfma", "message cache: mfma paths only");
 #define MF_CASE_MSG(FF, PP, TT)                                                                  \
   case FF * 8 + PP:                                                                             \
     hipLaunchKernelGGL((km_source_bwd<FF, PP, TT, true>), dim3(edge_grid(geo)), dim3(256), 0, st, \
                        geo, msg, y, sc, sh, QtS, Ws1, Ws2, bs2, mean, coef, Rs, Wt1, ghS, g_next, \
-                       mu1, inv1, g_tot, pW2, pW1, pCol, pBN, tmask);                           \
+                       mu1, inv1, g_tot, pW2, pW1, pCol, pBN, tmask, nullptr);                  \
     break;
     if (tmask && Rs) {
       switch (F * 8 + prec) {
@@ -1404,10 +1523,10 @@
   }
   if (tmask && Rs) {
     MF_LAUNCH3(F, prec, true, km_source_bwd, nullptr, y, sc, sh, QtS, Ws1, Ws2, bs2, mean, coef, Rs, Wt1,
-               ghS, g_next, mu1, inv1, g_tot, pW2, pW1, pCol, pBN, tmask)
+               ghS, g_next, mu1, inv1, g_tot, pW2, pW1, pCol, pBN, tmask, nullptr)
   } else {
     MF_LAUNCH3(F, prec, false, km_source_bwd, nullptr, y, sc, sh, QtS, Ws1, Ws2, bs2, mean, coef, Rs, Wt1,
-               ghS, g_next, mu1, inv1, g_tot, pW2, pW1, pCol, pBN, tmask)
+               ghS, g_next, mu1, inv1, g_tot, pW2, pW1, pCol, pBN, tmask, nullptr)
   }
   return 0;
 }
diff --git a/pfs-neural-net_amd/pfsgnn/engine.py b/pfs-neural-net_amd/pfsgnn/engine.py
--- a/pfs-neural-net_amd/pfsgnn/engine.py
+++ b/pfs-neural-net_amd/pfsgnn/engine.py
@@ -339,7 +339,7 @@
         return be.moment_coef(st["mom"], gst, d.NC if d.sp is None else d.sp.fib_ptr)
 
     def source_edge_bwd(self, P, Gr, d, pre, st, coef, tpart, g_next, bnstat, g_xt, se=None,
-                        epre=None, tmask=None):
+                        epre=None, tmask=None, dWt1=None):
         be, F = self.be, self.F
         Ws1, Ws2 = P[pre + "node_mlp_1.0.weight"], P[pre + "node_mlp_1.2.weight"]
         y, sc, sh = st["xe3"]
@@ -353,7 +353,8 @@
             tpart, g_next, bnstat, Gr[pre + "node_mlp_1.0.weight"], Gr[pre + "node_mlp_1.2.weight"],
             Gr[pre + "node_mlp_1.2.bias"], bn2=bn2, g_xt=g_xt,
             **({"tmask": tmask} if tmask is not None and tpart is not None else {}),
-            **({"msg": st["msg"]} if st.get("msg") is not None else {}))
+            **({"msg": st["msg"]} if st.get("msg") is not None else {}),
+            **({"dWt1": dWt1} if dWt1 is not None else {}))
         g_tot, GzS = out[0], out[1]
         be.wgrad(GzS, st["xt"], Gr[pre + "node_mlp_1.0.weight"], col0=0,
                  db=Gr[pre + "node_mlp_1.0.bias"])
@@ -482,6 +483,11 @@
         Wt1 = P[pre + "node_mlp_1.0.weight"]
         y, sc, sh = st["xe3"]
         kw = {"tmask": st["tmask"]} if st.get("tmask") is not None else {}
+        st["tfold"] = bool(kw and not want_gxe and d.sp is None and hasattr(be, "tbwd_fold")
+                           and os.environ.get("PFSGNN_TBWD_FOLD", "1") != "0"
+                           and be.tbwd_fold(d))
+        if st["tfold"]:
+            kw["fold"] = True
         if bn_sums is not None:
             kw["bn_sums"] = bn_sums
         out = be.target_bwd(d, y, sc, sh, st["Rs"], Wt1, g_hsum,
@@ -639,7 +645,9 @@
                                                    g_xe, bnstat, g_xt_in,
                                                    se=None if ev else se,
                                                    epre=p + "edge_model.",
-                                                   tmask=stt.get("tmask") if live_t else None)
+                                                   tmask=stt.get("tmask") if live_t else None,
+                                                   dWt1=Gr[p + "t_model.node_mlp_1.0.weight"]
+                                                   if live_t and stt.get("tfold") else None)
                 if not self.normed:
                     bnc = None
                 elif ev:
diff --git a/pfs-neural-net_amd/pfsgnn/native.py b/pfs-neural-net_amd/pfsgnn/native.py
--- a/pfs-neural-net_amd/pfsgnn/native.py
+++ b/pfs-neural-net_amd/pfsgnn/native.py
@@ -195,6 +195,9 @@
     "pfsgnn_tmask_bytes": ([I, I, I, I], SZ),
     "pfsgnn_target_bwd": ([I, I, I, I, P, P, P, P, P, P, P, P, P, P, P, P, SZ, P], I),
     "pfsgnn_target_bwd_bn": ([I, I, I, I] + [P] * 14 + [FL, P, P, SZ, P], I),
+    "pfsgnn_tbwd_fold": ([I], I),
+    "pfsgnn_target_bwd_fold": ([I, I, I, I] + [P] * 14 + [FL, P, P, SZ, P], I),
+    "pfsgnn_source_bwd_fold": ([I, I, I, I] + [P] * 17 + [LL, FL] + [P] * 16 + [P, SZ, P], I),
     "pfsgnn_source_bwd": ([I, I, I, I] + [P] * 24 + [P, SZ, P], I),
     "pfsgnn_source_bwd_bn": ([I, I, I, I] + [P] * 17 + [LL, FL] + [P] * 12 + [P, SZ, P], I),
     "pfsgnn_msg_bytes": ([I, I, I, I], SZ),
@@ -1051,8 +1054,29 @@
               float(bscale), _ptr(A), _ptr(tmask), ws, wsb, _stream())
         return hsum if agg is None else (hsum, A)
 
+    def tbwd_fold(self, d):
+        return d.sp is None and not self._composed(d) and bool(lib().pfsgnn_tbwd_fold(d.F))
+
     def target_bwd(self, d, y, sc, sh, Rs, Wt1, g_hsum, dWt1, want_gxe=False, g_xs=None,
-                   tmask=None, bn_sums=None):
+                   tmask=None, bn_sums=None, fold=False):
+        if fold:
+            assert tmask is not None and not want_gxe and d.sp is None
+            self._chk(g_xs)
+            GzT = self.empty(2 * d.F, d.NS)
+            g_hsum = g_hsum.contiguous()
+            Yp = mu = var = part = None
+            eps = 0.0
+            if bn_sums is not None:
+                assert g_xs is not None
+                Yp, mu, var, eps = bn_sums
+                self._chk(Yp, mu, var)
+                part = self.empty((d.NS + 63) // 64, 32)
+            ws, wsb = self._wsargs(d)
+            _call("pfsgnn_target_bwd_fold", d.G, d.NF, d.NC, d.F, y.data_ptr(), _ptr(sc),
+                  _ptr(sh), Rs.data_ptr(), Wt1.data_ptr(), g_hsum.data_ptr(), GzT.data_ptr(),
+                  dWt1.data_ptr(), None, _ptr(g_xs), tmask.data_ptr(), _ptr(Yp), _ptr(mu),
+                  _ptr(var), float(eps), _ptr(part), ws, wsb, _stream())
+            return (GzT, None) if bn_sums is None else (GzT, None, part)
         if bn_sums is not None:
             assert g_xs is not None and not self._composed(d) and d.sp is None
             Yp, mu, var, eps = bn_sums
@@ -1083,7 +1107,8 @@
         return GzT, gxe
 
     def source_bwd(self, d, y, sc, sh, Qt, Ws1, Ws2, bs2, mean, coef, tpart, g_next, bnstat,
-                   dWs1, dWs2, dbs2, bn2=None, g_xt=None, tmask=None, msg=None):
+                   dWs1, dWs2, dbs2, bn2=None, g_xt=None, tmask=None, msg=None, dWt1=None):
+        assert dWt1 is None or (tpart is not None and tmask is not None and d.sp is None)
         if self._composed(d):
             out = self._sp.source_bwd(d, y, sc, sh, Qt, Ws1, Ws2, bs2, mean, coef, tpart, g_next,
                                       bnstat, dWs1, dWs2, dbs2)
@@ -1112,6 +1137,21 @@
         head = (d.G, d.NF, d.NC, d.F, y.data_ptr(), _ptr(sc), _ptr(sh), Qt.data_ptr(),
                 Ws1.data_ptr(), Ws2.data_ptr(), bs2.data_ptr(), mean.data_ptr(), coef.data_ptr(),
                 _ptr(Rs), _ptr(Wt1), _ptr(g_hsum), _ptr(g_next), _ptr(mu1), _ptr(inv1))
+        if dWt1 is not None:
+            var1 = gamma = a = g0 = g1 = dg = db = None
+            n, eps = 0, 0.0
+            if bn2 is not None:
+                assert bnstat is not None
+                gamma, var1, n, eps, dg, db = bn2
+                a, g0, g1 = self.empty(d.F), self.empty(d.F), self.empty(d.F)
+            _call("pfsgnn_source_bwd_fold", *head, _ptr(var1), _ptr(gamma), int(n), float(eps),
+                  g_tot.data_ptr(), GzS.data_ptr(), dWs1.data_ptr(), dWs2.data_ptr(),
+                  dbs2.data_ptr(), _ptr(Sg), _ptr(Sgx), _ptr(a), _ptr(g0), _ptr(g1), _ptr(dg),
+                  _ptr(db), _ptr(g_xt), tmask.data_ptr(), _ptr(msg), dWt1.data_ptr(), ws, wsb,
+                  _stream())
+            if bn2 is not None:
+                return g_tot, GzS, None, None, (a, g0, g1)
+            return g_tot, GzS, Sg, Sgx
         if bn2 is not None:
             assert bnstat is not None
             gamma, var1, n, eps, dg, db = bn2
```

Result: faster. 517.6 million edges/s, median of 6 (+1.6%).
